# markchil/gptools

Measured on AMD Instinct MI355X. Metric: K-build+Cholesky GFLOP/s (% fp64 MFMA peak) and LML evals/sec, N=8192, higher is better.
Workload: dtype f64

## Files before the change

gptools_amd/_lib.py:

```python
import ctypes as C
import os
import subprocess
import threading

import numpy as np

_HERE = os.path.dirname(os.path.abspath(__file__))
LIB_PATH = os.path.join(_HERE, "libgpt_hip.so")

GPT_OK = 0
GPT_E_ARG, GPT_E_VALUE, GPT_E_NOTIMPL, GPT_E_HIP, GPT_E_NOMEM, GPT_E_STATE = -1, -2, -3, -4, -5, -6
KERNEL_SE, KERNEL_M52, KERNEL_DIAGNOISE, KERNEL_ZERO, KERNEL_RQ, KERNEL_MATERN, KERNEL_PRODUCT = 0, 1, 2, 3, 4, 5, 6
KERNEL_GIBBS_TANH, KERNEL_GIBBS_DTANH = 7, 8
MAX_DIM = 16
WARP_LINEAR, WARP_BETA, WARP_MAX_LAYERS = 1, 2, 4

_dp = C.POINTER(C.c_double)
_ip = C.POINTER(C.c_int32)
_vp = C.c_void_p
_i64 = C.c_int64

SIGNATURES = {
    "gpt_version": (C.c_int, []),
    "gpt_last_error": (C.c_char_p, []),
    "gpt_ctx_create": (C.c_int, [C.c_int, _vp, C.POINTER(_vp)]),
    "gpt_ctx_destroy": (C.c_int, [_vp]),
    "gpt_ctx_set_option": (C.c_int, [_vp, C.c_char_p, _i64]),
    "gpt_ctx_synchronize": (C.c_int, [_vp]),
    "gpt_ctx_stream": (_vp, [_vp]),
    "gpt_ctx_edge_count": (C.c_int64, [_vp]),
    "gpt_concurrency_hint": (C.c_int, [C.c_int]),
    "gpt_kpairs": (C.c_int, [_vp, C.c_int, _dp, C.c_int, _dp, _dp, _ip, _ip, _i64, C.c_int, C.c_int, C.c_int, _ip, _dp]),
    "gpt_kbuild": (C.c_int, [_vp, C.c_int, _dp, C.c_int, _dp, _ip, _i64, _dp, _ip, _i64, C.c_int, C.c_int, _ip, _dp]),
    "gpt_kpairs2": (C.c_int, [_vp, C.c_int, _dp, C.c_int, C.c_int, _dp, C.c_int, _dp, _dp, _ip, _ip, _i64, C.c_int, _dp]),
    "gpt_kbuild2": (C.c_int, [_vp, C.c_int, _dp, C.c_int, C.c_int, _dp, C.c_int, _dp, _ip, _i64, _dp, _ip, _i64, C.c_int, _dp]),
    "gpt_fit_terms": (C.c_int, [_vp, C.c_int, _ip, _ip, _dp, _ip, _ip, C.c_double, _dp, _dp, C.c_double, _dp, _dp]),
    "gpt_set_data": (C.c_int, [_vp, _dp, _ip, _i64, C.c_int]),
    "gpt_set_T": (C.c_int, [_vp, _dp, _i64]),
    "gpt_set_warp": (C.c_int, [_vp, C.c_int, _ip, _dp]),
    "gpt_set_warp_batch": (C.c_int, [_vp, C.c_int, C.c_int, _ip, _dp]),
    "gpt_fit": (C.c_int, [_vp, C.c_int, _dp, C.c_int, C.c_double, _dp, _dp, C.c_double, _dp, _dp]),
    "gpt_fit_sum": (C.c_int, [_vp, C.c_int, _ip, _dp, _ip, C.c_double, _dp, _dp, C.c_double, _dp, _dp]),
    "gpt_fit_batch": (C.c_int, [_vp, C.c_int, C.c_int, _dp, C.c_int, _dp, _dp, _dp, C.c_double, _dp, _dp, _ip]),
    "gpt_fit_batch_sum": (C.c_int, [_vp, C.c_int, C.c_int, _ip, _dp, _ip, _dp, _dp, _dp, C.c_double, _dp, _dp, _ip]),
    "gpt_mem_info": (C.c_int, [_vp, C.POINTER(_i64), C.POINTER(_i64)]),
    "gpt_release_batch_scratch": (C.c_int, [_vp]),
    "gpt_fit_batch_terms": (C.c_int, [_vp, C.c_int, C.c_int, _ip, _ip, _dp, _ip, _ip, _dp, _dp, _dp, C.c_double, _dp, _dp, _ip]),
    "gpt_predict_batch": (C.c_int, [_vp, _dp, _ip, _i64, _ip, _ip, _dp, _dp, _dp, _dp]),
    "gpt_fit_matrix": (C.c_int, [_vp, _dp, _i64, _dp, _dp, _dp]),
    "gpt_get_L": (C.c_int, [_vp, _dp]),
    "gpt_get_alpha": (C.c_int, [_vp, _dp]),
    "gpt_ll_grad": (C.c_int, [_vp, C.c_int, _ip, _ip, _dp]),
    "gpt_predict": (C.c_int, [_vp, _dp, _ip, _i64, C.c_int, _dp, _ip, _dp, _dp, _dp]),
    "gpt_host_alloc": (C.c_int, [_i64, C.POINTER(_vp)]),
    "gpt_host_free": (C.c_int, [_vp]),
    "gpt_cov_sample": (C.c_int, [_vp, _i64, C.c_double, _dp, _i64, _dp]),
    "gpt_solve_L": (C.c_int, [_vp, _dp, _i64]),
    "gpt_cho_solve": (C.c_int, [_vp, _dp, _i64]),
    "gpt_last_timings": (C.c_int, [_vp, _dp, C.c_int]),
    "gpt_gemm_profile_read": (C.c_int, [_vp, _dp]),
    "gpt_gemm_profile_read4": (C.c_int, [_vp, _dp]),
    "gpt_plan_unique_id": (C.c_int, [_vp]),
    "gpt_plan_create": (C.c_int, [C.c_int, C.POINTER(_vp), C.POINTER(_i64), _i64, C.c_int, _vp, _vp, C.c_int, _vp, C.POINTER(_vp)]),
    "gpt_plan_set_comm": (C.c_int, [_vp, C.c_int, C.c_int, _vp]),
    "gpt_plan_set_channel": (C.c_int, [_vp, C.c_int, C.c_int, C.c_int, _vp]),
    "gpt_plan_run": (C.c_int, [_vp, C.c_int, _dp, C.c_int, C.c_double, C.c_double]),
    "gpt_plan_last_enqueue_ms": (C.c_double, [_vp]),
    "gpt_plan_destroy": (C.c_int, [_vp]),
    "gpt_potrf_host": (C.c_int, [_vp, _dp, _i64]),
    "gpt_gemm_nt_host": (C.c_int, [_vp, _i64, _i64, _i64, C.c_double, _dp, _dp, C.c_double, _dp]),
    "gpt_dev_kbuild": (C.c_int, [_vp, C.c_int, _dp, C.c_int, _vp, _vp, _i64, _vp, _vp, _i64, C.c_int, C.c_int, C.c_int,
                                 _ip, C.c_int, _i64, _i64, _vp, C.c_double, C.c_double, _vp, _i64]),
    "gpt_dev_gemm_nt": (C.c_int, [_vp, _i64, _i64, _i64, C.c_double, _vp, _i64, _vp, _i64, C.c_double, _vp, _i64, C.c_int]),
    "gpt_dev_gemm_nt_stair": (C.c_int, [_vp, _i64, _i64, _i64, _i64, C.c_double, _vp, _i64, _vp, _i64, _i64, _i64, C.c_double, _vp, _i64]),
    "gpt_dev_gemm_nt_gridstair": (C.c_int, [_vp, _i64, _i64, _i64, _i64, C.c_double, _vp, _i64, _vp, _i64, _i64, _i64, _i64, _i64,
                                           C.c_double, _vp, _i64]),
    "gpt_dev_row_sumsq": (C.c_int, [_vp, _vp, _i64, _vp]),
    "gpt_dev_potrf_panel": (C.c_int, [_vp, _i64, _i64, _vp, _i64, _vp, _vp, _i64]),
    "gpt_dev_potrf": (C.c_int, [_vp, _i64, _vp, _i64, _vp, _vp]),
    "gpt_dev_trsm_rlt": (C.c_int, [_vp, _i64, _i64, _vp, _i64, _vp, _vp, _i64]),
    "gpt_dev_trinv": (C.c_int, [_vp, _i64, _vp, _i64, _vp, _vp, _i64]),
    "gpt_dev_copy2d": (C.c_int, [_vp, _i64, _i64, _vp, _i64, _vp, _i64]),
    "gpt_dev_copy2d_on": (C.c_int, [_vp, _vp, _i64, _i64, _vp, _i64, _vp, _i64]),
    "gpt_dev_pad_block": (C.c_int, [_vp, _vp, _i64, _i64, _i64, _i64, _i64, _vp, C.c_double]),
    "gpt_dev_panel_scalars": (C.c_int, [_vp, _vp, _i64, _i64, _i64, _vp]),
}

_lib = None
_lock = threading.Lock()


class GPTBackendError(RuntimeError):
    """The HIP backend is missing or failed; there is deliberately no CPU fallback."""


def build(verbose=False):
    cmd = ["make", "-C", os.path.join(_HERE, "csrc"), "-j4"]
    res = subprocess.run(cmd, stdout=subprocess.PIPE, stderr=subprocess.STDOUT, text=True)
    if verbose or res.returncode != 0:
        print(res.stdout)
    if res.returncode != 0:
        raise GPTBackendError("building libgpt_hip.so failed")
    return LIB_PATH


def load():
    global _lib
    with _lock:
        if _lib is None:
            if not os.path.exists(LIB_PATH):
                raise GPTBackendError(
                    "%s not found: run `python -c 'import __graft_entry__ as g; g.build()'` "
                    "(gptools_amd has no CPU fallback)" % LIB_PATH)
            try:
                import torch
            except ImportError:
                pass
            lib = C.CDLL(LIB_PATH)
            for name, (res, args) in SIGNATURES.items():
                fn = getattr(lib, name)
                fn.restype = res
                fn.argtypes = args
            _lib = lib
    return _lib


def last_error():
    return load().gpt_last_error().decode("utf-8", "replace")


def check(rc):
    if rc == GPT_OK:
        return
    msg = last_error()
    if rc > 0:
        raise np.linalg.LinAlgError(msg or "%d-th leading minor of the array is not positive definite" % rc)
    if rc in (GPT_E_ARG, GPT_E_VALUE):
        raise ValueError(msg)
    if rc == GPT_E_NOTIMPL:
        raise NotImplementedError(msg)
    if rc == GPT_E_NOMEM:
        raise MemoryError(msg)
    raise GPTBackendError("libgpt_hip: %s (code %d)" % (msg, rc))


def f64(a):
    return np.ascontiguousarray(a, dtype=np.float64)


def i32(a):
    return np.ascontiguousarray(a, dtype=np.int32)


def dptr(a):
    return None if a is None else a.ctypes.data_as(_dp)


def iptr(a):
    return None if a is None else a.ctypes.data_as(_ip)


class _PinnedOwner(object):

    def __init__(self, lib, ptr, nbytes):
        self._lib, self._ptr, self._nbytes = lib, ptr, nbytes

    def __del__(self):
        try:
            if self._ptr:
                _pinned_release(self._lib, self._ptr, self._nbytes)
                self._ptr = None
        except Exception:
            pass


PINNED_POOL_BYTES = 2 << 30
_pinned_free = {}
_pinned_held = [0]


def _pinned_release(lib, ptr, nbytes):
    with _lock:
        if _pinned_held[0] + nbytes <= PINNED_POOL_BYTES:
            _pinned_free.setdefault(nbytes, []).append(ptr)
            _pinned_held[0] += nbytes
            return
    lib.gpt_host_free(ptr)


def pinned_empty(shape, min_bytes=1 << 20):
    n = int(np.prod(shape))
    if n * 8 < min_bytes:
        return np.empty(shape, dtype=np.float64)
    lib = load()
    p = None
    with _lock:
        blocks = _pinned_free.get(n * 8)
        if blocks:
            p = blocks.pop()
            _pinned_held[0] -= n * 8
    if p is None:
        p = _vp()
        check(lib.gpt_host_alloc(n * 8, C.byref(p)))
    buf = (C.c_double * n).from_address(p.value)
    buf._owner = _PinnedOwner(lib, p, n * 8)
    return np.ctypeslib.as_array(buf).reshape(shape)


class concurrent_evaluations(object):

    def __enter__(self):
        load().gpt_concurrency_hint(1)
        return self

    def __exit__(self, *exc):
        load().gpt_concurrency_hint(-1)
        return False


class Context(object):

    def __init__(self, device=0, stream=None):
        lib = load()
        h = _vp()
        check(lib.gpt_ctx_create(int(device), _vp(stream) if stream else None, C.byref(h)))
        self._h = h
        self._lib = lib
        self.device = int(device)
        self._warp_key = None

    def close(self):
        if getattr(self, "_h", None):
            self._lib.gpt_ctx_destroy(self._h)
            self._h = None

    def __del__(self):
        try:
            self.close()
        except Exception:
            pass

    @property
    def handle(self):
        if not self._h:
            raise GPTBackendError("context already destroyed")
        return self._h

    def set_option(self, key, value):
        check(self._lib.gpt_ctx_set_option(self.handle, key.encode(), int(value)))

    def synchronize(self):
        check(self._lib.gpt_ctx_synchronize(self.handle))

    @property
    def stream(self):
        return self._lib.gpt_ctx_stream(self.handle)

    @property
    def edge_count(self):
        return int(self._lib.gpt_ctx_edge_count(self.handle))

    @staticmethod
    def _pair_args(Xi, Xj, ni, nj):
        Xi, Xj, ni, nj = f64(Xi), f64(Xj), i32(ni), i32(nj)
        if Xi.ndim != 2 or Xi.shape != Xj.shape or ni.shape != Xi.shape or nj.shape != Xi.shape:
            raise ValueError("Lengths/widths of Xi, Xj, ni, nj don't match")
        M, D = Xi.shape
        return (dptr(Xi), dptr(Xj), iptr(ni), iptr(nj), M), D, np.empty(M, dtype=np.float64), (Xi, Xj, ni, nj)

    @staticmethod
    def _block_args(Xi, ni, Xj, nj):
        Xi, ni = f64(Xi), i32(ni)
        M, D = Xi.shape
        if Xj is None:
            Xj_, nj_, P = None, None, M
        else:
            Xj_, nj_ = f64(Xj), i32(nj)
            P = Xj_.shape[0]
        return (dptr(Xi), iptr(ni), M, dptr(Xj_), iptr(nj_), P), D, np.empty((M, P), dtype=np.float64), (Xi, ni, Xj_, nj_)

    def kpairs(self, kernel_id, params, Xi, Xj, ni, nj, hyper_deriv=None, symmetric=False, noise_n=None):
        params = f64(params)
        pts, D, out, keep = self._pair_args(Xi, Xj, ni, nj)
        nn = None if noise_n is None else i32(noise_n)
        check(self._lib.gpt_kpairs(self.handle, kernel_id, dptr(params), len(params), *pts, D,
                                   -1 if hyper_deriv is None else int(hyper_deriv), int(bool(symmetric)), iptr(nn), dptr(out)))
        return out

    def kbuild(self, kernel_id, params, Xi, ni, Xj=None, nj=None, hyper_deriv=None, noise_n=None):
        params = f64(params)
        pts, D, out, keep = self._block_args(Xi, ni, Xj, nj)
        nn = None if noise_n is None else i32(noise_n)
        check(self._lib.gpt_kbuild(self.handle, kernel_id, dptr(params), len(params), *pts, D,
                                   -1 if hyper_deriv is None else int(hyper_deriv), iptr(nn), dptr(out)))
        return out

    def kpairs2(self, kid1, params1, kid2, params2, Xi, Xj, ni, nj):
        p1, p2 = f64(params1), f64(params2)
        pts, D, out, keep = self._pair_args(Xi, Xj, ni, nj)
        check(self._lib.gpt_kpairs2(self.handle, kid1, dptr(p1), len(p1), kid2, dptr(p2), len(p2), *pts, D, dptr(out)))
        return out

    def kbuild2(self, kid1, params1, kid2, params2, Xi, ni, Xj=None, nj=None):
        p1, p2 = f64(params1), f64(params2)
        pts, D, out, keep = self._block_args(Xi, ni, Xj, nj)
        check(self._lib.gpt_kbuild2(self.handle, kid1, dptr(p1), len(p1), kid2, dptr(p2), len(p2), *pts, D, dptr(out)))
        return out

    @staticmethod
    def _flat_params(terms):
        return np.concatenate([np.asarray(p, dtype=float) for t in terms for p in t[1::2]])

    @staticmethod
    def _pack_terms(terms):
        ids = i32(np.asarray([t[0] for t in terms]))
        ids2 = i32(np.asarray([t[2] if len(t) == 4 else -1 for t in terms]))
        npar1 = i32(np.asarray([len(t[1]) for t in terms]))
        npar = i32(np.asarray([len(t[1]) + (len(t[3]) if len(t) == 4 else 0) for t in terms]))
        return ids, ids2, npar, npar1, f64(Context._flat_params(terms))

    def fit_terms(self, terms, noise_var, y, err_y, diag_add):
        ids, ids2, npar, npar1, flat = self._pack_terms(terms)
        y, err_y = f64(y), f64(err_y)
        ll = C.c_double()
        ld = C.c_double()
        check(self._lib.gpt_fit_terms(self.handle, len(ids), iptr(ids), iptr(ids2), dptr(flat), iptr(npar), iptr(npar1),
                                      float(noise_var), dptr(y), dptr(err_y), float(diag_add), C.byref(ll), C.byref(ld)))
        return ll.value, ld.value

    def set_data(self, X, n):
        X, n = f64(X), i32(n)
        self._warp_key = None
        self._num_dim = X.shape[1]
        check(self._lib.gpt_set_data(self.handle, dptr(X), iptr(n), X.shape[0], X.shape[1]))

    def set_warp(self, layers):
        layers = [(int(t), f64(p).ravel()) for t, p in (layers or [])]
        key = tuple((t, p.tobytes()) for t, p in layers) or None
        if key == self._warp_key:
            return
        self._warp_key = None
        if not layers:
            check(self._lib.gpt_set_warp(self.handle, 0, None, None))
            return
        types = i32(np.asarray([t for t, _ in layers]))
        flat = f64(np.concatenate([p for _, p in layers]))
        if any(p.size != 2 * getattr(self, "_num_dim", -1) for _, p in layers):
            raise ValueError("set_warp needs set_data first, and every layer takes 2 * num_dim parameters")
        check(self._lib.gpt_set_warp(self.handle, len(layers), iptr(types), dptr(flat)))
        self._warp_key = key

    def set_warp_batch(self, layers_list):
        types = [int(t) for t, _ in layers_list[0]]
        D = getattr(self, "_num_dim", -1)
        rows = []
        for layers in layers_list:
            if [int(t) for t, _ in layers] != types:
                raise ValueError("set_warp_batch: every element takes the same layer types")
            ps = [f64(p).ravel() for _, p in layers]
            if any(p.size != 2 * D for p in ps):
                raise ValueError("set_warp_batch needs set_data first, and every layer takes 2 * num_dim parameters")
            rows.append(np.concatenate(ps) if ps else np.zeros(0))
        flat = f64(np.array(rows))
        check(self._lib.gpt_set_warp_batch(self.handle, len(layers_list), len(types), iptr(i32(np.asarray(types))), dptr(flat)))

    def set_T(self, T):
        if T is None:
            check(self._lib.gpt_set_T(self.handle, None, 0))
            return
        T = f64(T)
        if T.ndim != 2:
            raise ValueError("T must be 2-dimensional")
        check(self._lib.gpt_set_T(self.handle, dptr(T), T.shape[0]))

    def fit(self, kernel_id, params, noise_var, y, err_y, diag_add):
        params, y, err_y = f64(params), f64(y), f64(err_y)
        ll = C.c_double()
        ld = C.c_double()
        check(self._lib.gpt_fit(self.handle, kernel_id, dptr(params), len(params), float(noise_var), dptr(y),
                                dptr(err_y), float(diag_add), C.byref(ll), C.byref(ld)))
        return ll.value, ld.value

    def fit_sum(self, kernel_ids, params_list, noise_var, y, err_y, diag_add):
        ids = i32(np.asarray(kernel_ids))
        npar = i32(np.asarray([len(p) for p in params_list]))
        flat = f64(np.concatenate([np.asarray(p, dtype=float) for p in params_list]))
        y, err_y = f64(y), f64(err_y)
        ll = C.c_double()
        ld = C.c_double()
        check(self._lib.gpt_fit_sum(self.handle, len(ids), iptr(ids), dptr(flat), iptr(npar), float(noise_var), dptr(y),
                                    dptr(err_y), float(diag_add), C.byref(ll), C.byref(ld)))
        return ll.value, ld.value

    def fit_batch(self, kernel_id, params, noise_var, y, err_y, diag_add):
        params, noise_var, y, err_y = f64(np.atleast_2d(params)), f64(noise_var), f64(np.atleast_2d(y)), f64(err_y)
        B = params.shape[0]
        if noise_var.shape != (B,) or y.shape[0] != B or y.shape[1] != err_y.shape[0]:
            raise ValueError("fit_batch: params (B, p), noise_var (B,), y (B, N), err_y (N,) expected")
        ll, ld, info = np.empty(B), np.empty(B), np.zeros(B, dtype=np.int32)
        check(self._lib.gpt_fit_batch(self.handle, B, kernel_id, dptr(params), params.shape[1], dptr(noise_var), dptr(y),
                                      dptr(err_y), float(diag_add), dptr(ll), dptr(ld), iptr(info)))
        return ll, ld, info

    def fit_batch_sum(self, kernel_ids, params, nparams, noise_var, y, err_y, diag_add):
        ids, npar = i32(kernel_ids), i32(nparams)
        params, noise_var, y, err_y = f64(np.atleast_2d(params)), f64(noise_var), f64(np.atleast_2d(y)), f64(err_y)
        B = params.shape[0]
        if (noise_var.shape != (B,) or y.shape[0] != B or y.shape[1] != err_y.shape[0] or len(ids) != len(npar)
                or params.shape[1] != int(npar.sum())):
            raise ValueError("fit_batch_sum: params (B, sum(nparams)), noise_var (B,), y (B, N), err_y (N,) expected")
        ll, ld, info = np.empty(B), np.empty(B), np.zeros(B, dtype=np.int32)
        check(self._lib.gpt_fit_batch_sum(self.handle, B, len(ids), iptr(ids), dptr(params), iptr(npar), dptr(noise_var),
                                          dptr(y), dptr(err_y), float(diag_add), dptr(ll), dptr(ld), iptr(info)))
        return ll, ld, info

    def fit_batch_terms(self, terms_list, noise_var, y, err_y, diag_add):
        ids, ids2, npar, npar1, _ = self._pack_terms(terms_list[0])
        params = f64(np.array([self._flat_params(terms) for terms in terms_list]))
        noise_var, y, err_y = f64(noise_var), f64(np.atleast_2d(y)), f64(err_y)
        B = params.shape[0]
        if noise_var.shape != (B,) or y.shape[0] != B or y.shape[1] != err_y.shape[0] or params.shape[1] != int(npar.sum()):
            raise ValueError("fit_batch_terms: one parameter set per element, noise_var (B,), y (B, N), err_y (N,) expected")
        ll, ld, info = np.empty(B), np.empty(B), np.zeros(B, dtype=np.int32)
        check(self._lib.gpt_fit_batch_terms(self.handle, B, len(ids), iptr(ids), iptr(ids2), dptr(params), iptr(npar), iptr(npar1),
                                            dptr(noise_var), dptr(y), dptr(err_y), float(diag_add), dptr(ll), dptr(ld), iptr(info)))
        return ll, ld, info

    def predict_batch(self, Xstar, nstar, keep, noise_n=None, want_var=True, want_cov=False, want_cov_sum=False):
        Xstar, nstar, keep = f64(Xstar), i32(nstar), i32(np.asarray(keep) != 0)
        B, M = keep.shape[0], Xstar.shape[0]
        mean = np.full((B, M), np.nan)
        var = np.full((B, M), np.nan) if want_var else None
        cov = np.full((B, M, M), np.nan) if want_cov else None
        cov_sum = np.empty((M, M)) if want_cov_sum else None
        nn = None if noise_n is None else i32(np.asarray(noise_n).reshape(-1))
        check(self._lib.gpt_predict_batch(self.handle, dptr(Xstar), iptr(nstar), M, iptr(nn), iptr(keep), dptr(mean), dptr(var),
                                          dptr(cov), dptr(cov_sum)))
        return mean, var, cov, cov_sum

    def mem_info(self):
        f, t = _i64(), _i64()
        check(self._lib.gpt_mem_info(self.handle, C.byref(f), C.byref(t)))
        return int(f.value), int(t.value)

    def release_batch_scratch(self):
        check(self._lib.gpt_release_batch_scratch(self.handle))

    def ll_grad(self, term_idx, local_idx):
        ti, li = i32(np.asarray(term_idx)), i32(np.asarray(local_idx))
        out = np.empty(len(ti) + 1)
        check(self._lib.gpt_ll_grad(self.handle, len(ti), iptr(ti), iptr(li), dptr(out)))
        return out

    def fit_matrix(self, K_tot, y):
        K_tot, y = f64(K_tot), f64(y)
        ll = C.c_double()
        ld = C.c_double()
        check(self._lib.gpt_fit_matrix(self.handle, dptr(K_tot), K_tot.shape[0], dptr(y), C.byref(ll), C.byref(ld)))
        return ll.value, ld.value

    def get_L(self, N):
        L = np.empty((N, N), dtype=np.float64)
        check(self._lib.gpt_get_L(self.handle, dptr(L)))
        return L

    def get_alpha(self, N):
        a = np.empty(N, dtype=np.float64)
        check(self._lib.gpt_get_alpha(self.handle, dptr(a)))
        return a

    def predict(self, Xstar, nstar, want, noise_params=None, noise_n=None, device_cov=False):
        Xstar, nstar = f64(Xstar), i32(nstar)
        M = Xstar.shape[0]
        mean = np.empty(M)
        std = np.empty(M) if want >= 1 else None
        cov = pinned_empty((M, M)) if (want == 2 and not device_cov) else None
        npar = None if noise_params is None else f64(noise_params)
        nn = None if noise_n is None else i32(noise_n)
        check(self._lib.gpt_predict(self.handle, dptr(Xstar), iptr(nstar), M, int(want), dptr(npar), iptr(nn),
                                    dptr(mean), dptr(std), dptr(cov)))
        return mean, std, cov

    def cov_sample(self, diag_add, rand_vars):
        R = f64(np.atleast_2d(rand_vars))
        out = np.empty(R.shape)
        check(self._lib.gpt_cov_sample(self.handle, R.shape[0], float(diag_add), dptr(R), R.shape[1], dptr(out)))
        return out

    def solve_L(self, B):
        B2 = np.array(B, dtype=np.float64, order="C")
        shp = B2.shape
        B2 = np.ascontiguousarray(B2.reshape(shp[0], -1))
        check(self._lib.gpt_solve_L(self.handle, dptr(B2), B2.shape[1]))
        return B2.reshape(shp)

    def cho_solve(self, B):
        B2 = np.array(B, dtype=np.float64, order="C")
        shp = B2.shape
        B2 = np.ascontiguousarray(B2.reshape(shp[0], -1))
        check(self._lib.gpt_cho_solve(self.handle, dptr(B2), B2.shape[1]))
        return B2.reshape(shp)

    def last_timings(self):
        out = np.zeros(5)
        self._lib.gpt_last_timings(self.handle, dptr(out), 5)
        return dict(upload=out[0], kbuild=out[1], potrf=out[2], tail=out[3], total=out[4])

    def gemm_profile_read(self, with_bytes=False):
        out = np.zeros(4)
        check(self._lib.gpt_gemm_profile_read4(self.handle, dptr(out)))
        if with_bytes:
            return float(out[0]), float(out[1]), int(out[2]), float(out[3])
        return float(out[0]), float(out[1]), int(out[2])

    def potrf_host(self, A):
        L = np.array(A, dtype=np.float64, order="C")
        check(self._lib.gpt_potrf_host(self.handle, dptr(L), L.shape[0]))
        return L

    def gemm_nt_host(self, alpha, A, B, beta, Cm):
        A, B = f64(A), f64(B)
        Cm = np.array(Cm, dtype=np.float64, order="C")
        check(self._lib.gpt_gemm_nt_host(self.handle, A.shape[0], B.shape[0], A.shape[1], float(alpha), dptr(A),
                                         dptr(B), float(beta), dptr(Cm)))
        return Cm


_default_ctx = {}


def default_context(device=0):
    key = (os.getpid(), int(device))
    ctx = _default_ctx.get(key)
    if ctx is None:
        ctx = Context(device)
        _default_ctx[key] = ctx
    return ctx
```

gptools_amd/csrc/api.hip:

```cpp
#include <math.h>
#include <stdarg.h>
#include <stdlib.h>
#include <string.h>
#include <new>
#include <chrono>
#include <mutex>
#include <vector>
#include "common.hpp"
#include "warp.hpp"

static thread_local char g_err[512] = "";

void gpt_set_error(const char *fmt, ...)
{
    va_list ap;
    va_start(ap, fmt);
    vsnprintf(g_err, sizeof(g_err), fmt, ap);
    va_end(ap);
}

extern "C" const char *gpt_last_error(void) { return g_err; }
extern "C" int gpt_version(void) { return 100; }

#define GPT_TRY(expr)          \
    do {                       \
        int rc_ = (expr);      \
        if (rc_ != GPT_OK) return rc_; \
    } while (0)

static inline int64_t round_up(int64_t x, int64_t m) { return (x + m - 1) / m * m; }

#include "api_kparams.inc"

struct DevBuf {
    void *p = nullptr;
    size_t cap = 0;
};

enum { SLOT_XI = 0, SLOT_XJ, SLOT_NI, SLOT_NJ, SLOT_OUT, SLOT_KST, SLOT_KSS, SLOT_XS, SLOT_NS, SLOT_VEC, SLOT_VEC2,
       SLOT_RHS, SLOT_LOW, SLOT_KFULL, SLOT_TK, SLOT_ZERO, SLOT_UINV, SLOT_WINV, SLOT_GPART, SLOT_BINV, SLOT_BTMP,
       SLOT_BINV2, SLOT_BINV3, SLOT_BINV3U, SLOT_BINVU, SLOT_BATCH_A, SLOT_BATCH_WS, SLOT_BATCH_MISC, SLOT_SPLITK,
       SLOT_PB_V, SLOT_PB_COV, SLOT_PB_MISC, SLOT_XSW, SLOT_SS, SLOT_SI, SLOT_SJ, SLOT_WB_X, SLOT_WB_S, SLOT_WB_P, SLOT_COUNT };

struct gpt_ctx {
    int device = 0;
    hipStream_t stream = nullptr;
    bool own_stream = false;
    hipStream_t panel_stream = nullptr;
    hipStream_t helper_stream = nullptr;
    int64_t nb_early = 0, nb_switch_rows = 4608;
    unsigned *d_edge = nullptr;
    unsigned edge_seq = 0;
    int64_t tail_wait = 1;
    int64_t merge_urgent = 1;
    int64_t edge_flags = 1;
    bool flags_now = false;
    int reserve_cus = 0;
    int64_t gemm_prio = -1;
    int64_t purg_rows = 6144;
    int64_t defer_rows = 0;
    int helper_cus = 0;
    std::vector<hipEvent_t> events;
    hipEvent_t tev[5] = {nullptr, nullptr, nullptr, nullptr, nullptr};
    int64_t nb_outer = 0;
    int lookahead = 1;
    int use_graph = 0;
    long n_maxsum = 0;
    long n_maxord = 0;
    int timing = 0;
    int tile = 0;
    int gemm_pad = 1024;
    int64_t fuse_trsm = 8192;
    unsigned *d_flag = nullptr;
    unsigned flag_epoch = 0;
    int64_t binv_launches = 0;
    int64_t splitk = 512;
    int64_t fuse_rows32 = 2048, fuse_rows16 = 0;
    int64_t fuse_rows64 = 2048;
    int64_t helper_min_n = 12288;
    int helper_tf = 45;
    int ramp = 0;
    int inner = 0;
    int64_t N = 0;
    int64_t Nx = 0;
    int D = 0;
    double *dT = nullptr;
    int64_t Ny = 0, NxP = 0;
    double *dX = nullptr;
    int32_t *dn = nullptr;
    WarpLayers warp = WarpLayers();
    double *dXw = nullptr, *dS = nullptr;
    int warpb_nbatch = 0;
    bool rb_warped = false;
    int64_t NP = 0;
    double *dA = nullptr;
    double *d_invd = nullptr;
    int32_t *d_info = nullptr;
    double *d_y = nullptr, *d_erry = nullptr, *d_scal = nullptr, *d_alpha = nullptr;
    double *h_scal = nullptr;
    double *h_yerr = nullptr;
    double *h_alpha = nullptr;
    bool h_alpha_valid = false;
    int32_t *h_info = nullptr;
    bool factored = false, alpha_valid = false, have_kernel = false;
    bool binv_valid = false;
    bool binv2_valid = false;
    bool binv3_valid = false;
    int64_t dev_gemm_pad = 0;
    int64_t eager_alpha = 0;
    int64_t binv_early = 0;
    hipEvent_t e_binv_early = nullptr;
    int64_t defer_pad = 1;
    unsigned alpha_counter = 0;
    int64_t debug_poison = 0;
    int64_t edge_test_stall = 0;
    double *h_stage = nullptr;
    hipStream_t copy_stream = nullptr;
    hipEvent_t cev[4] = {nullptr, nullptr, nullptr, nullptr};
    double *h_batch = nullptr;
    size_t h_batch_cap = 0;
    uint64_t batch_gen = 1, rb_gen = 0;
    int rb_nbatch = 0;
    int64_t rb_N = 0;
    ModelKernel rb_model;
    std::vector<KParams> rb_kp, rb_kp2;
    std::vector<double> rb_nv;
    int64_t cov_M = 0;
    ModelKernel model;
    double timings[5] = {0, 0, 0, 0, 0};
    int prof_gemm = 0;
    struct GemmProf { hipEvent_t e0, e1, stop; double flops, bytes; };
    std::vector<GemmProf> gprof;
    size_t gprof_used = 0;
    double prof_flops = 0, prof_ms = 0, prof_count = 0, prof_bytes = 0;
    hipGraphExec_t gexec = nullptr;
    int64_t g_n = 0, g_nb = 0;
    int g_la = 0;
    double *g_A = nullptr;
    DevBuf slots[SLOT_COUNT];
};

static int strip_rows_code(const gpt_ctx *c, int64_t m) { return m <= c->fuse_rows16 ? 3 : m <= c->fuse_rows32 ? 2 : m <= c->fuse_rows64 ? 1 : 0; }

static int ensure(gpt_ctx *c, int slot, size_t bytes, void **out)
{
    DevBuf &b = c->slots[slot];
    if (b.cap < bytes) {
        if (b.p) GPT_HIP_CHECK(hipFree(b.p));
        b.p = nullptr;
        b.cap = 0;
        const size_t want = bytes + bytes / 8 + 256;
        GPT_HIP_CHECK(hipMalloc(&b.p, want));
        b.cap = want;
    }
    *out = b.p;
    return GPT_OK;
}

static hipEvent_t get_event(gpt_ctx *c, size_t idx)
{
    while (c->events.size() <= idx) {
        hipEvent_t e = nullptr;
        if (hipEventCreate(&e) != hipSuccess) return nullptr;
        c->events.push_back(e);
    }
    return c->events[idx];
}

static void invalidate_factor(gpt_ctx *c)
{
    c->factored = false;
    c->h_alpha_valid = c->alpha_valid = c->binv_valid = c->binv2_valid = c->binv3_valid = false;
}

static int stream_follows(gpt_ctx *c, hipStream_t from, hipStream_t to, size_t idx)
{
    hipEvent_t e = get_event(c, idx);
    if (!e) return GPT_E_HIP;
    GPT_HIP_CHECK(hipEventRecord(e, from));
    GPT_HIP_CHECK(hipStreamWaitEvent(to, e, 0));
    return GPT_OK;
}

#include "api_schedule.inc"
#include "api_context.inc"
#include "api_kernels.inc"
#include "api_fit.inc"
#include "api_batch.inc"
#include "api_grad.inc"
#include "api_solve.inc"
#include "api_predict.inc"
#include "api_dev.inc"
#include "api_plan.inc"
```

gptools_amd/csrc/api_batch.inc:

```
#define GPT_BATCH_MAX_N 8192
static int fit_batch_impl(gpt_ctx *c, int nbatch, int nterms, const int *kernel_ids, const int *kernel_ids2, const double *params,
                          const int *nparams_t, const int *nparams1_t, const double *noise_var, const double *y, const double *err_y,
                          double diag_add, double *ll_data_out, double *logdet_half_out, int32_t *info_out);

extern "C" int gpt_fit_batch(gpt_ctx *c, int nbatch, int kernel_id, const double *params, int nparams,
                             const double *noise_var, const double *y, const double *err_y, double diag_add,
                             double *ll_data_out, double *logdet_half_out, int32_t *info_out)
{
    return fit_batch_impl(c, nbatch, 1, &kernel_id, nullptr, params, &nparams, nullptr, noise_var, y, err_y, diag_add, ll_data_out,
                          logdet_half_out, info_out);
}

extern "C" int gpt_fit_batch_sum(gpt_ctx *c, int nbatch, int nterms, const int *kernel_ids, const double *params,
                                 const int *nparams_t, const double *noise_var, const double *y, const double *err_y,
                                 double diag_add, double *ll_data_out, double *logdet_half_out, int32_t *info_out)
{
    return fit_batch_impl(c, nbatch, nterms, kernel_ids, nullptr, params, nparams_t, nullptr, noise_var, y, err_y, diag_add, ll_data_out,
                          logdet_half_out, info_out);
}

extern "C" int gpt_fit_batch_terms(gpt_ctx *c, int nbatch, int nterms, const int *kernel_ids, const int *kernel_ids2,
                                   const double *params, const int *nparams_t, const int *nparams1_t, const double *noise_var,
                                   const double *y, const double *err_y, double diag_add, double *ll_data_out,
                                   double *logdet_half_out, int32_t *info_out)
// ... 34 lines not shown
    const size_t off_err = (size_t)nbatch * N, off_nv = off_err + (size_t)N, off_kp = off_nv + (size_t)nbatch, off_res = off_kp + nkp;
    const size_t need = (off_res + 4 * (size_t)nbatch) * sizeof(double);
    if (c->h_batch_cap < need) {
        if (c->h_batch) GPT_HIP_CHECK(hipHostFree(c->h_batch));
        c->h_batch = nullptr;
        c->h_batch_cap = 0;
        GPT_HIP_CHECK(hipHostMalloc((void **)&c->h_batch, need + need / 4, hipHostMallocDefault));
        c->h_batch_cap = need + need / 4;
    }
    double *h = c->h_batch;
    memcpy(h, y, (size_t)nbatch * N * sizeof(double));
    memcpy(h + off_err, err_y, (size_t)N * sizeof(double));
    memcpy(h + off_nv, noise_var, (size_t)nbatch * sizeof(double));
    char *hkp = reinterpret_cast<char *>(h + off_kp), *hkp2 = hkp + (size_t)nterms * nbatch * kp_doubles * 8;
    for (int b = 0; b < nbatch; b++) {
        if (b > 0) GPT_TRY(parse_model(c->D, c->n_maxsum, nterms, kernel_ids, kernel_ids2, params + (size_t)b * m0.nparams, nparams_t, nparams1_t, &mb));
        const ModelKernel &m = b > 0 ? mb : m0;
        for (int t = 0; t < nterms; t++) {
            memcpy(hkp + ((size_t)t * nbatch + (size_t)b) * kp_doubles * 8, &m.f1[t], sizeof(KParams));
            if (any_prod) memcpy(hkp2 + ((size_t)t * nbatch + (size_t)b) * kp_doubles * 8, &m.f2[t], sizeof(KParams));
        }
    }
    c->batch_gen++;
    const int64_t NxP = c->dT ? c->NxP : 0, NyP = c->dT ? round_up(N, 64) : 0;
    const size_t kfull = (size_t)NxP * NxP, tk = (size_t)NyP * NxP;
    double *dA, *dws, *dmisc;
    GPT_TRY(ensure(c, SLOT_BATCH_A, ((size_t)nbatch * bs + (size_t)nbatch * (kfull + tk)) * sizeof(double), (void **)&dA));
    double *dKf = dA + (size_t)nbatch * bs, *dTK = dKf + (size_t)nbatch * kfull;
    GPT_TRY(ensure(c, SLOT_BATCH_WS, (size_t)nbatch * bws * sizeof(double), (void **)&dws));
    const size_t d_off_nv = (size_t)N, d_off_kp = d_off_nv + (size_t)nbatch, d_off_info = d_off_kp + nkp,
                 d_off_zero = d_off_info + (size_t)nbatch;
    GPT_TRY(ensure(c, SLOT_BATCH_MISC, (d_off_zero + (size_t)(c->dT ? Nx : 0)) * sizeof(double), (void **)&dmisc));
    int32_t *dinfo = reinterpret_cast<int32_t *>(dmisc + d_off_info);
    const KParams *dkp = reinterpret_cast<const KParams *>(dmisc + d_off_kp);
    const KParams *dkp2 = any_prod ? dkp + (size_t)nterms * nbatch : nullptr;
    const double *bX = c->dX, *bS = nullptr;
    int64_t xstr = 0, sstr = 0;
    if (wb) {
        bX = (const double *)c->slots[SLOT_WB_X].p;
        bS = (const double *)c->slots[SLOT_WB_S].p;
        xstr = Nx * c->D;
        sstr = Nx;
    }
    EvalScope scope(c, true);
    hipStream_t st = c->panel_stream;
    GPT_TRY(stream_follows(c, c->stream, st, 0));
    GPT_HIP_CHECK(hipMemcpyAsync(dmisc, h + off_err, ((size_t)N + (size_t)nbatch + nkp) * sizeof(double), hipMemcpyHostToDevice, st));
    auto term_kp2 = [&](int t) -> const KParams * { return m0.second(t) ? dkp2 + (size_t)t * nbatch : nullptr; };
    if (c->dT) {
        double *dzero = dmisc + d_off_zero;
        GPT_HIP_CHECK(hipMemsetAsync(dzero, 0, (size_t)Nx * sizeof(double), st));
        if (NxP > Nx) GPT_HIP_CHECK(hipMemsetAsync(dKf, 0, (size_t)nbatch * kfull * sizeof(double), st));
        for (int t = 0; t < nterms; t++)
            GPT_TRY(launch_kbuild_batch(st, m0.f1[t].kernel_id, c->D, dkp + (size_t)t * nbatch, dmisc + d_off_nv, nbatch, bX, c->dn, Nx,
                                        t + 1 == nterms ? dzero : nullptr, 0.0, dKf, NxP, (int64_t)kfull, t > 0 ? 1 : 0, 1, term_kp2(t),
                                        xstr, bS, sstr));
        GPT_TRY(launch_gemm_nt(st, NyP, NxP, NxP, 1.0, c->dT, NxP, dKf, NxP, 0.0, dTK, NxP, 0, 0, 0, nullptr, nullptr, 0, EdgeSig(),
                               EdgeSig(), 0, nbatch, 0, EdgeSig(), (int64_t)kfull, (int64_t)tk));
        GPT_TRY(launch_gemm_nt(st, NyP, NyP, NxP, 1.0, dTK, NxP, c->dT, NxP, 0.0, dA, NP, 1, 0, 0, nullptr, nullptr, 0, EdgeSig(),
                               EdgeSig(), 0, nbatch, (int64_t)tk, EdgeSig(), 0, bs));
        GPT_TRY(launch_add_diag(st, dA, NP, N, dmisc, diag_add, nbatch, bs));
        GPT_TRY(launch_batch_pad(st, h, nbatch, dA, NP, bs, N, NP, 1e300, dinfo));
    } else {
        GPT_TRY(launch_batch_pad(st, h, nbatch, dA, NP, bs, N, NP, 1e300, dinfo));
        for (int t = 0; t < nterms; t++)
            GPT_TRY(launch_kbuild_batch(st, m0.f1[t].kernel_id, c->D, dkp + (size_t)t * nbatch, dmisc + d_off_nv, nbatch,
                                        bX, c->dn, N, t + 1 == nterms ? dmisc : nullptr, diag_add, dA, NP, bs,
                                        t > 0 ? 1 : 0, 0, term_kp2(t), xstr, bS, sstr));
    }
    static const bool force_right = getenv("GPT_BATCH_RIGHT") != nullptr;
    const bool right_looking = force_right || NP <= 512;
    for (int64_t lc = 0; lc < NP; lc += 128) {
        if (!right_looking && lc > 0)
            GPT_TRY(launch_gemm_nt(st, NP - lc, 128, lc, -1.0, dA + lc * NP, NP, dA + lc * NP, NP, 1.0, dA + lc * NP + lc, NP, 1, 0, 0,
                                   nullptr, nullptr, 0, EdgeSig(), EdgeSig(), 0, nbatch, bs));
        GPT_TRY(launch_potf2_diag(st, dA + lc * NP + lc, NP, dws + (lc / 128) * GPT_WS_BLOCK, dinfo, lc, EdgeSig(), nbatch, bs, bws));
        const int64_t r1 = lc + 128, m = NP - r1;
        if (m <= 0) break;
        GPT_TRY(launch_trsm_panel(st, m, dA + lc * NP + lc, NP, dws + (lc / 128) * GPT_WS_BLOCK, dA + r1 * NP + lc, NP, nullptr,
                                  EdgeSig(), nbatch, bs, bws));
        if (right_looking)
            GPT_TRY(launch_gemm_nt(st, m, m, 128, -1.0, dA + r1 * NP + lc, NP, dA + r1 * NP + lc, NP, 1.0, dA + r1 * NP + r1, NP, 1, 0, 0,
                                   nullptr, nullptr, 0, EdgeSig(), EdgeSig(), 0, nbatch, bs));
    }
    GPT_TRY(launch_batch_logdet_dot(st, dA, NP, bs, N, nbatch, dinfo, h + off_res));
    GPT_HIP_CHECK(hipStreamSynchronize(st));
    for (int b = 0; b < nbatch; b++) {
        const double logdet_half = h[off_res + 4 * b], zz = h[off_res + 4 * b + 1];
        int32_t info = (int32_t)h[off_res + 4 * b + 2];
        if (info > N) info = (int32_t)N;
        const double ll = -0.5 * zz - logdet_half - 0.5 * (double)N * log(2.0 * M_PI);
        if (info == 0 && !(ll == ll)) info = (int32_t)N;
        info_out[b] = info;
        ll_data_out[b] = ll;
        if (logdet_half_out) logdet_half_out[b] = logdet_half;
    }
    const KParams *hk = reinterpret_cast<const KParams *>(hkp);
    c->rb_kp.assign(hk, hk + (size_t)nterms * nbatch);
    if (any_prod) c->rb_kp2.assign(hk + (size_t)nterms * nbatch, hk + 2 * (size_t)nterms * nbatch);
    else c->rb_kp2.clear();
    c->rb_nv.assign(noise_var, noise_var + nbatch);
    c->rb_nbatch = nbatch;
    c->rb_model = m0;
    c->rb_N = N;
    c->rb_gen = c->batch_gen;
    c->rb_warped = wb != 0;
    return GPT_OK;
}

static int gemm_nt_few(gpt_ctx *c, hipStream_t st, int64_t m, int64_t n, int64_t k, double alpha, const double *A, int64_t lda,
                       const double *B, int64_t ldb, double beta, double *C, int64_t ldc, int tri);
extern "C" int gpt_predict_batch(gpt_ctx *c, const double *Xstar, const int32_t *nstar, int64_t M, const int32_t *noise_n,
                                 const int32_t *keep, double *mean_out, double *var_out, double *cov_out, double *cov_sum_out)
{
    CTX_ENTER(c);
    GPT_TRY(refuse_warp(c, "gpt_predict_batch"));
    if (c->rb_warped && c->rb_nbatch > 0 && c->rb_gen == c->batch_gen) {
        gpt_set_error("gpt_predict_batch is not available for a batch that was fitted with warps (gpt_set_warp_batch)");
        return GPT_E_NOTIMPL;
    }
    if (c->rb_nbatch <= 0 || c->rb_gen != c->batch_gen) {
        gpt_set_error("gpt_predict_batch: no batch resident (call gpt_fit_batch* first; gpt_set_data, gpt_set_T, gpt_cov_sample and "
                      "gpt_release_batch_scratch end its residency)");
        return GPT_E_STATE;
    }
    if (c->dT) {
        gpt_set_error("gpt_predict_batch: not implemented with a linear transform (gpt_set_T)");
        return GPT_E_NOTIMPL;
    }
    if (M <= 0 || M > 65535 * 32 || !Xstar || !nstar || !keep || !mean_out) {
        gpt_set_error("gpt_predict_batch: bad arguments");
        return GPT_E_ARG;
    }
    const ModelKernel &model = c->rb_model;
    const int D = c->D, nbatch = c->rb_nbatch, nterms = model.nterms;
    const int64_t N = c->rb_N, NP = round_up(N + 1, 128), nleaf = NP / 128, bs = NP * NP, bws = nleaf * GPT_WS_BLOCK;
    const int64_t MP = round_up(M, 64), ldv = (int64_t)nbatch * NP;
    GPT_TRY(check_test_orders(model, c->n_maxsum, false, nstar, M, D));
    double noise_sum = 0.0;
    for (int b = 0; b < nbatch; b++)
        if (keep[b]) noise_sum += c->rb_nv[b];
    std::vector<int32_t> hit((size_t)M, 0);
    if (noise_n)
        for (int64_t a = 0; a < M; a++) {
            bool h = true;
            for (int d = 0; d < D; d++) h = h && nstar[a * D + d] == noise_n[d];
            hit[a] = h ? 1 : 0;
        }
    const size_t nkp = (size_t)nterms * nbatch * (model.any_prod ? 2 : 1);
    const size_t b_kp = nkp * sizeof(KParams) + (size_t)nbatch * 8, b_keep = round_up(nbatch, 2) * 4, b_hit = round_up(M, 2) * 4,
                 b_xs = (size_t)M * D * 8, b_ns = round_up(M * D, 2) * 4;
    const size_t o_keep = b_kp, o_hit = o_keep + b_keep, o_xs = o_hit + b_hit, o_ns = o_xs + b_xs, o_mv = o_ns + b_ns;
    const size_t b_mv = 2 * (size_t)nbatch * MP * 8;
    char *dmisc;
    GPT_TRY(ensure(c, SLOT_PB_MISC, o_mv + b_mv, (void **)&dmisc));
    std::vector<char> hin(o_mv);
    memcpy(hin.data(), c->rb_kp.data(), (size_t)nterms * nbatch * sizeof(KParams));
    if (model.any_prod) memcpy(hin.data() + (size_t)nterms * nbatch * sizeof(KParams), c->rb_kp2.data(), (size_t)nterms * nbatch * sizeof(KParams));
    memcpy(hin.data() + nkp * sizeof(KParams), c->rb_nv.data(), (size_t)nbatch * 8);
    memcpy(hin.data() + o_keep, keep, (size_t)nbatch * 4);
    memcpy(hin.data() + o_hit, hit.data(), (size_t)M * 4);
    memcpy(hin.data() + o_xs, Xstar, b_xs);
    memcpy(hin.data() + o_ns, nstar, (size_t)M * D * 4);
    const KParams *dkp = reinterpret_cast<const KParams *>(dmisc);
    const KParams *dkp2 = model.any_prod ? dkp + (size_t)nterms * nbatch : nullptr;
    const double *dnv = reinterpret_cast<const double *>(dmisc + nkp * sizeof(KParams));
    const int32_t *dkeep = reinterpret_cast<const int32_t *>(dmisc + o_keep), *dhit = reinterpret_cast<const int32_t *>(dmisc + o_hit);
    const double *dXs = reinterpret_cast<const double *>(dmisc + o_xs);
    const int32_t *dns = reinterpret_cast<const int32_t *>(dmisc + o_ns);
    double *dmean = reinterpret_cast<double *>(dmisc + o_mv), *dvar = dmean + (size_t)nbatch * MP;
    double *dV, *dC = nullptr;
    GPT_TRY(ensure(c, SLOT_PB_V, (size_t)MP * ldv * sizeof(double), (void **)&dV));
    const bool want_cov = cov_out != nullptr, want_sum = cov_sum_out != nullptr;
    if (want_cov || want_sum)
        GPT_TRY(ensure(c, SLOT_PB_COV, (want_cov ? (size_t)nbatch : 1) * MP * MP * sizeof(double), (void **)&dC));
    const double *dA = (const double *)c->slots[SLOT_BATCH_A].p, *dws = (const double *)c->slots[SLOT_BATCH_WS].p;
    EvalScope scope(c, true);
    hipStream_t st = c->panel_stream;
    GPT_TRY(stream_follows(c, c->stream, st, 0));
    GPT_HIP_CHECK(hipMemcpyAsync(dmisc, hin.data(), o_mv, hipMemcpyHostToDevice, st));
    auto term_kp2 = [&](int t) -> const KParams * { return model.second(t) ? dkp2 + (size_t)t * nbatch : nullptr; };
    GPT_TRY(launch_zero2d(st, MP, ldv, dV, ldv));
    for (int t = 0; t < nterms; t++)
        GPT_TRY(launch_kbuild_batch_cross(st, model.f1[t].kernel_id, D, dkp + (size_t)t * nbatch, dnv, nbatch, dXs, dns,
                                          M, c->dX, c->dn, N, dV, ldv, NP, t > 0 ? 1 : 0, term_kp2(t)));
    for (int64_t lc = 0; lc < NP; lc += 128) {
        if (lc > 0)
            GPT_TRY(launch_gemm_nt(st, MP, 128, lc, -1.0, dV, ldv, dA + lc * NP, NP, 1.0, dV + lc, ldv, 0, 0, 0, nullptr, nullptr, 0,
                                   EdgeSig(), EdgeSig(), 0, nbatch, NP, EdgeSig(), bs, NP));
        GPT_TRY(launch_trsm_panel(st, MP, nullptr, 0, dws + (lc / 128) * GPT_WS_BLOCK, dV + lc, ldv, nullptr, EdgeSig(), nbatch, NP, bws));
    }
    GPT_TRY(launch_kdiag_batch(st, D, nterms, dkp, dkp2, nbatch, dXs, dns, M, dvar, MP));
    GPT_TRY(launch_batch_meanvar(st, M, MP, N, NP, nbatch, dV, ldv, dA, bs, dkeep, dmean, dvar, MP));
    std::vector<double> hmv(2 * (size_t)nbatch * MP);
    GPT_HIP_CHECK(hipMemcpyAsync(hmv.data(), dmean, hmv.size() * sizeof(double), hipMemcpyDeviceToHost, st));
    if (want_sum) {
        GPT_TRY(launch_zero2d(st, MP, MP, dC, MP));
        GPT_TRY(launch_kss_sum(st, D, nterms, dkp, dkp2, nbatch, dkeep, dXs, dns, M, MP, noise_n ? dhit : nullptr, noise_sum, dC, MP));
        GPT_TRY(gemm_nt_few(c, st, MP, MP, ldv, -1.0, dV, ldv, dV, ldv, 1.0, dC, MP, 1));
        GPT_TRY(launch_mirror_rows(st, dC, MP, 0, MP, MP));
        GPT_HIP_CHECK(hipMemcpy2DAsync(cov_sum_out, (size_t)M * sizeof(double), dC, (size_t)MP * sizeof(double), (size_t)M * sizeof(double),
                                       (size_t)M, hipMemcpyDeviceToHost, st));
    }
    GPT_HIP_CHECK(hipStreamSynchronize(st));
    if (want_cov) {
        const int64_t cs = MP * MP;
        GPT_TRY(launch_zero2d(st, (int64_t)nbatch * MP, MP, dC, MP));
        for (int t = 0; t < nterms; t++)
            GPT_TRY(launch_kbuild_batch_cross(st, model.f1[t].kernel_id, D, dkp + (size_t)t * nbatch, dnv, nbatch, dXs,
                                              dns, M, dXs, dns, M, dC, MP, cs, t > 0 ? 1 : 0, term_kp2(t)));
        GPT_TRY(launch_gemm_nt(st, MP, MP, NP, -1.0, dV, ldv, dV, ldv, 1.0, dC, MP, 0, 0, 0, nullptr, nullptr, 0, EdgeSig(), EdgeSig(), 0,
                               nbatch, NP, EdgeSig(), NP, cs));
        for (int b = 0; b < nbatch; b++)
            if (keep[b])
                GPT_HIP_CHECK(hipMemcpy2DAsync(cov_out + (size_t)b * M * M, (size_t)M * sizeof(double), dC + (size_t)b * cs,
                                               (size_t)MP * sizeof(double), (size_t)M * sizeof(double), (size_t)M, hipMemcpyDeviceToHost, st));
        GPT_HIP_CHECK(hipStreamSynchronize(st));
    }
    for (int b = 0; b < nbatch; b++) {
        if (!keep[b]) continue;
        const double *hm = hmv.data() + (size_t)b * MP, *hv = hm + (size_t)nbatch * MP;
        memcpy(mean_out + (size_t)b * M, hm, (size_t)M * sizeof(double));
        const double nv = c->rb_nv[b];
        if (var_out)
            for (int64_t a = 0; a < M; a++) var_out[(size_t)b * M + a] = hv[a] + (hit[a] ? nv : 0.0);
        if (cov_out && noise_n)
            for (int64_t a = 0; a < M; a++)
                if (hit[a]) cov_out[(size_t)b * M * M + (size_t)a * M + a] += nv;
    }
    return GPT_OK;
}

extern "C" int gpt_last_timings(gpt_ctx *c, double *out_ms, int n)
{
    if (!c || !out_ms) return GPT_E_ARG;
    const int cnt = n < 5 ? n : 5;
    for (int i = 0; i < cnt; i++) out_ms[i] = c->timings[i];
    return cnt;
}

static int harvest_gemm_profile(gpt_ctx *c)
{
    for (size_t i = 0; i < c->gprof_used; i++) {
        float t = 0;
        GPT_HIP_CHECK(hipEventElapsedTime(&t, c->gprof[i].e0, c->gprof[i].stop));
        c->prof_ms += t;
        c->prof_flops += c->gprof[i].flops;
        c->prof_bytes += c->gprof[i].bytes;
    }
    c->prof_count += (double)c->gprof_used;
    c->gprof_used = 0;
    return GPT_OK;
}

static int gemm_profile_read(gpt_ctx *c, double *out, int n)
{
    if (!out || n < 3) return GPT_E_ARG;
    GPT_HIP_CHECK(hipStreamSynchronize(c->stream));
    GPT_HIP_CHECK(hipStreamSynchronize(c->panel_stream));
    GPT_TRY(harvest_gemm_profile(c));
    out[0] = c->prof_flops;
    out[1] = c->prof_ms;
    out[2] = c->prof_count;
    if (n > 3) out[3] = c->prof_bytes;
    c->prof_flops = c->prof_ms = c->prof_count = c->prof_bytes = 0.0;
    return GPT_OK;
}

extern "C" int gpt_gemm_profile_read(gpt_ctx *c, double *out3)
{
    CTX_ENTER(c);
    return gemm_profile_read(c, out3, 3);
}

extern "C" int gpt_gemm_profile_read4(gpt_ctx *c, double *out4)
{
    CTX_ENTER(c);
    return gemm_profile_read(c, out4, 4);
}

#define NEED_FACTOR(c)                                                        \
    do {                                                                      \
        if (!(c)->factored) {                                                 \
            gpt_set_error("no valid factorisation resident (call gpt_fit)");  \
            return GPT_E_STATE;                                               \
        }                                                                     \
    } while (0)

extern "C" int gpt_get_L(gpt_ctx *c, double *L_out)
{
    CTX_ENTER(c);
    NEED_FACTOR(c);
    if (!L_out) return GPT_E_ARG;
    const int64_t N = c->N;
    double *dlow;
    GPT_TRY(ensure(c, SLOT_LOW, (size_t)N * N * sizeof(double), (void **)&dlow));
    GPT_TRY(launch_extract_lower(c->stream, c->dA, c->NP, N, dlow, N));
    GPT_HIP_CHECK(hipMemcpyAsync(L_out, dlow, (size_t)N * N * sizeof(double), hipMemcpyDeviceToHost, c->stream));
    GPT_HIP_CHECK(hipStreamSynchronize(c->stream));
    return GPT_OK;
}

static int ensure_block_inverses(gpt_ctx *c, int64_t nb, int64_t nfull, double **out, double **out_u = nullptr, hipStream_t on = nullptr);
static int ensure_alpha(gpt_ctx *c, hipStream_t on = nullptr)
{
    if (c->alpha_valid) return GPT_OK;
    const int64_t N = c->N, NP = c->NP, n128 = round_up(N, 128);
    hipStream_t st = on ? on : c->stream;
    static const bool narrow = getenv("GPT_ALPHA_NARROW") != nullptr;
    const int64_t nwide = (n128 / 512) * 512;
    double *w = c->d_alpha + NP;
    const double *z = c->dA + N * NP;
    if (!narrow && nwide == N && nwide >= 1024) {
        double *W = nullptr, *U = nullptr;
        GPT_TRY(ensure_block_inverses(c, 512, nwide, &W, &U, st));
        GPT_TRY(launch_trsv_lt_wide(st, nwide, c->dA, NP, U, w, c->d_alpha, z));
        c->alpha_valid = true;
        return GPT_OK;
    }
    GPT_TRY(launch_alpha_init(st, N, NP, z, w, c->d_alpha));
    if (narrow || nwide < 1024) {
        GPT_HIP_CHECK(hipMemcpyAsync(c->d_alpha, w, (size_t)N * sizeof(double), hipMemcpyDeviceToDevice, st));
        GPT_TRY(launch_trsv_lt(st, n128, c->dA, NP, c->d_invd, c->d_alpha));
        c->alpha_valid = true;
        return GPT_OK;
    }
    double *W = nullptr, *U = nullptr;
    GPT_TRY(ensure_block_inverses(c, 512, nwide, &W, &U, st));
    if (n128 > nwide) {
        GPT_TRY(launch_trsv_lt(st, n128, c->dA, NP, c->d_invd, w, nwide / 128));
        GPT_HIP_CHECK(hipMemcpyAsync(c->d_alpha + nwide, w + nwide, (size_t)(n128 - nwide) * sizeof(double), hipMemcpyDeviceToDevice, st));
    }
    GPT_TRY(launch_trsv_lt_wide(st, nwide, c->dA, NP, U, w, c->d_alpha));
    c->alpha_valid = true;
    return GPT_OK;
}

static int alpha_to_host(gpt_ctx *c, hipStream_t on)
{
    hipStream_t st = on ? on : c->stream;
    GPT_TRY(ensure_alpha(c, st));
    if (c->h_alpha_valid) return GPT_OK;
    GPT_HIP_CHECK(hipMemcpyAsync(c->h_alpha, c->d_alpha, (size_t)c->N * sizeof(double), hipMemcpyDeviceToHost, st));
    c->h_alpha_valid = true;
    return GPT_OK;
}

extern "C" int gpt_get_alpha(gpt_ctx *c, double *alpha_out)
{
    CTX_ENTER(c);
    NEED_FACTOR(c);
    if (!alpha_out) return GPT_E_ARG;
    const bool landed = c->alpha_valid && c->h_alpha_valid;
    if (!landed) {
        GPT_TRY(alpha_to_host(c));
        GPT_HIP_CHECK(hipStreamSynchronize(c->stream));
    }
    memcpy(alpha_out, c->h_alpha, (size_t)c->N * sizeof(double));
    return GPT_OK;
}
```

gptools_amd/csrc/api_context.inc:

```
extern "C" int gpt_ctx_create(int device_id, void *stream, gpt_ctx **out)
{
    if (!out) return GPT_E_ARG;
    int ndev = 0;
    GPT_HIP_CHECK(hipGetDeviceCount(&ndev));
    if (ndev <= 0 || device_id < 0 || device_id >= ndev) {
        gpt_set_error("no such HIP device %d (count %d)", device_id, ndev);
        return GPT_E_HIP;
    }
    GPT_HIP_CHECK(hipSetDevice(device_id));
    gpt_ctx *c = new (std::nothrow) gpt_ctx();
    if (!c) return GPT_E_NOMEM;
    c->device = device_id;
    int lo = 0, hi = 0;
    GPT_HIP_CHECK(hipDeviceGetStreamPriorityRange(&lo, &hi));
    if (stream) {
        c->stream = (hipStream_t)stream;
    } else {
        int reserve = 32;
        if (const char *e = getenv("GPT_RESERVE_CUS")) reserve = atoi(e);
        hipDeviceProp_t prop;
        GPT_HIP_CHECK(hipGetDeviceProperties(&prop, device_id));
        const int ncu = prop.multiProcessorCount;
        bool masked = false;
        if (reserve > 0 && reserve < ncu) {
            std::vector<uint32_t> mask((ncu + 31) / 32, 0u);
            for (int i = reserve; i < ncu; i++) mask[i / 32] |= (1u << (i % 32));
            masked = hipExtStreamCreateWithCUMask(&c->stream, (uint32_t)mask.size(), mask.data()) == hipSuccess;
            if (!masked) (void)hipGetLastError();
            else c->reserve_cus = reserve;
            if (masked && reserve >= 16) {
                std::vector<uint32_t> hm((ncu + 31) / 32, 0u);
                for (int i = 8; i < reserve; i++) hm[i / 32] |= (1u << (i % 32));
                if (hipExtStreamCreateWithCUMask(&c->helper_stream, (uint32_t)hm.size(), hm.data()) != hipSuccess) {
                    (void)hipGetLastError();
                    c->helper_stream = nullptr;
                }
                c->helper_cus = reserve - 8;
            }
        }
        if (!masked) GPT_HIP_CHECK(hipStreamCreateWithFlags(&c->stream, hipStreamNonBlocking));
        c->own_stream = true;
    }
    GPT_HIP_CHECK(hipStreamCreateWithPriority(&c->panel_stream, hipStreamNonBlocking, hi));
    for (int i = 0; i < 5; i++) GPT_HIP_CHECK(hipEventCreate(&c->tev[i]));
    GPT_HIP_CHECK(hipMalloc(&c->d_info, sizeof(int32_t)));
    GPT_HIP_CHECK(hipMalloc((void **)&c->d_flag, 256));
    GPT_HIP_CHECK(hipMalloc((void **)&c->d_edge, 256));
    GPT_HIP_CHECK(hipMemsetAsync(c->d_flag, 0, 256, c->stream));
    GPT_HIP_CHECK(hipMemsetAsync(c->d_edge, 0, 256, c->stream));
    GPT_HIP_CHECK(hipMalloc(&c->d_scal, 80 * sizeof(double)));
    GPT_HIP_CHECK(hipMemsetAsync(c->d_scal, 0, 80 * sizeof(double), c->stream));
    GPT_HIP_CHECK(hipHostMalloc((void **)&c->h_scal, 4 * sizeof(double), hipHostMallocDefault));
    GPT_HIP_CHECK(hipHostMalloc((void **)&c->h_info, sizeof(int32_t), hipHostMallocDefault));
    *out = c;
    return GPT_OK;
}

static void free_factor(gpt_ctx *c)
{
    if (c->gexec) { hipGraphExecDestroy(c->gexec); c->gexec = nullptr; }
    if (c->dA) hipFree(c->dA);
    if (c->d_invd) hipFree(c->d_invd);
    if (c->d_y) hipFree(c->d_y);
    if (c->h_yerr) hipHostFree(c->h_yerr);
    c->h_yerr = nullptr;
    if (c->h_alpha) hipHostFree(c->h_alpha);
    c->h_alpha = nullptr;
    c->h_alpha_valid = false;
    if (c->d_alpha) hipFree(c->d_alpha);
    c->dA = c->d_invd = c->d_y = c->d_erry = c->d_alpha = nullptr;
    c->NP = 0;
    invalidate_factor(c);
}

extern "C" int gpt_ctx_destroy(gpt_ctx *c)
{
    if (!c) return GPT_OK;
    hipSetDevice(c->device);
    hipStreamSynchronize(c->stream);
    hipStreamSynchronize(c->panel_stream);
    free_factor(c);
    if (c->dX) hipFree(c->dX);
    if (c->dn) hipFree(c->dn);
    if (c->dXw) hipFree(c->dXw);
    if (c->dS) hipFree(c->dS);
    if (c->dT) hipFree(c->dT);
    for (auto &b : c->slots)
        if (b.p) hipFree(b.p);
    for (auto e : c->events) hipEventDestroy(e);
    for (auto &g : c->gprof) { hipEventDestroy(g.e0); hipEventDestroy(g.e1); }
    for (int i = 0; i < 5; i++)
        if (c->tev[i]) hipEventDestroy(c->tev[i]);
    if (c->d_info) hipFree(c->d_info);
    if (c->d_flag) hipFree(c->d_flag);
    if (c->d_edge) hipFree(c->d_edge);
    if (c->d_scal) hipFree(c->d_scal);
    if (c->h_scal) hipHostFree(c->h_scal);
    if (c->h_stage) hipHostFree(c->h_stage);
    if (c->h_batch) hipHostFree(c->h_batch);
    if (c->copy_stream) hipStreamDestroy(c->copy_stream);
    for (auto &e : c->cev)
        if (e) hipEventDestroy(e);
    if (c->h_info) hipHostFree(c->h_info);
    hipStreamDestroy(c->panel_stream);
    if (c->e_binv_early) hipEventDestroy(c->e_binv_early);
    if (c->helper_stream) hipStreamDestroy(c->helper_stream);
    if (c->own_stream) hipStreamDestroy(c->stream);
    delete c;
    return GPT_OK;
}

extern "C" int gpt_ctx_set_option(gpt_ctx *c, const char *key, int64_t value)
{
    if (!c || !key) return GPT_E_ARG;
    if (!strcmp(key, "nb_outer")) {
        if (value < 0 || value % 128) {
            gpt_set_error("nb_outer must be 0 (chosen by size) or a positive multiple of 128");
            return GPT_E_ARG;
        }
        c->nb_outer = value;
    } else if (!strcmp(key, "lookahead")) c->lookahead = value ? 1 : 0;
    else if (!strcmp(key, "graph")) c->use_graph = value ? 1 : 0;
    else if (!strcmp(key, "timing")) c->timing = value ? 1 : 0;
    else if (!strcmp(key, "profile_gemm")) c->prof_gemm = value ? 1 : 0;
    else if (!strcmp(key, "gemm_pad")) c->gemm_pad = (int)value;
    else if (!strcmp(key, "dev_gemm_pad")) c->dev_gemm_pad = value;
    else if (!strcmp(key, "ramp")) c->ramp = value ? 1 : 0;
    else if (!strcmp(key, "defer_rows")) c->defer_rows = value;
    else if (!strcmp(key, "purg_rows")) c->purg_rows = value;
    else if (!strcmp(key, "edge_flags")) c->edge_flags = value;
    else if (!strcmp(key, "merge_urgent")) c->merge_urgent = value;
    else if (!strcmp(key, "tail_wait")) c->tail_wait = value;
    else if (!strcmp(key, "gemm_prio")) c->gemm_prio = value;
    else if (!strcmp(key, "nb_early")) c->nb_early = value;
    else if (!strcmp(key, "nb_switch_rows")) c->nb_switch_rows = value;
    else if (!strcmp(key, "inner")) c->inner = (int)value;
    else if (!strcmp(key, "helper_tf")) c->helper_tf = (int)value;
    else if (!strcmp(key, "helper_min_n")) c->helper_min_n = value;
    else if (!strcmp(key, "fuse_trsm")) c->fuse_trsm = value;
    else if (!strcmp(key, "fuse_rows64")) c->fuse_rows64 = value;
    else if (!strcmp(key, "fuse_rows32")) c->fuse_rows32 = value;
    else if (!strcmp(key, "fuse_rows16")) c->fuse_rows16 = value;
    else if (!strcmp(key, "splitk")) c->splitk = value;
    else if (!strcmp(key, "eager_alpha")) c->eager_alpha = value;
    else if (!strcmp(key, "defer_pad")) c->defer_pad = value;
    else if (!strcmp(key, "binv_launches")) { c->binv_launches = value; c->binv_valid = c->binv2_valid = c->binv3_valid = false; c->h_alpha_valid = c->alpha_valid = false; }
    else if (!strcmp(key, "debug_poison")) c->debug_poison = value;
    else if (!strcmp(key, "alpha_invalidate")) c->h_alpha_valid = c->alpha_valid = false;
    else if (!strcmp(key, "edge_test_stall")) c->edge_test_stall = value;
    else if (!strcmp(key, "tile")) {
        if (value != 0 && value != 32 && value != 64) {
            gpt_set_error("tile must be 0 (by launch size), 32 or 64");
            return GPT_E_ARG;
        }
        c->tile = (int)value;
    } else {
        gpt_set_error("unknown option '%s'", key);
        return GPT_E_ARG;
    }
    return GPT_OK;
}

extern "C" int gpt_ctx_synchronize(gpt_ctx *c)
{
    if (!c) return GPT_E_ARG;
    GPT_HIP_CHECK(hipStreamSynchronize(c->stream));
    return GPT_OK;
}

extern "C" void *gpt_ctx_stream(gpt_ctx *c) { return c ? (void *)c->stream : nullptr; }
extern "C" int64_t gpt_ctx_edge_count(gpt_ctx *c) { return c ? (int64_t)c->edge_seq : -1; }

#define CTX_ENTER(c)                          \
    do {                                      \
        if (!(c)) {                           \
            gpt_set_error("null context");    \
            return GPT_E_ARG;                 \
        }                                     \
        GPT_HIP_CHECK(hipSetDevice((c)->device)); \
    } while (0)
```

gptools_amd/csrc/api_fit.inc:

```
extern "C" int gpt_set_data(gpt_ctx *c, const double *X, const int32_t *n, int64_t N, int D)
{
    CTX_ENTER(c);
    if (N <= 0 || !X || !n || D < 1 || D > GPT_MAX_DIM) {
        gpt_set_error("set_data: bad arguments (N=%lld, D=%d)", (long long)N, D);
        return GPT_E_ARG;
    }
    GPT_HIP_CHECK(hipStreamSynchronize(c->stream));
    if (c->dX) hipFree(c->dX);
    if (c->dn) hipFree(c->dn);
    c->dX = nullptr;
    c->dn = nullptr;
    if (c->dXw) hipFree(c->dXw);
    if (c->dS) hipFree(c->dS);
    c->dXw = c->dS = nullptr;
    c->warp.nlayers = 0;
    c->warpb_nbatch = 0;
    GPT_HIP_CHECK(hipMalloc(&c->dX, (size_t)N * D * sizeof(double)));
    GPT_HIP_CHECK(hipMalloc(&c->dn, (size_t)N * D * sizeof(int32_t)));
    GPT_HIP_CHECK(hipMemcpyAsync(c->dX, X, (size_t)N * D * sizeof(double), hipMemcpyHostToDevice, c->stream));
    GPT_HIP_CHECK(hipMemcpyAsync(c->dn, n, (size_t)N * D * sizeof(int32_t), hipMemcpyHostToDevice, c->stream));
    GPT_HIP_CHECK(hipStreamSynchronize(c->stream));
    c->N = N;
    c->Nx = N;
    c->D = D;
    c->n_maxsum = c->n_maxord = 0;
    for (int64_t i = 0; i < N; i++) {
        long sn = 0;
        for (int d = 0; d < D; d++) {
            sn += n[i * D + d];
            if (n[i * D + d] > c->n_maxord) c->n_maxord = n[i * D + d];
        }
        if (sn > c->n_maxsum) c->n_maxsum = sn;
    }
    invalidate_factor(c);
    c->have_kernel = false;
    c->batch_gen++;
    if (c->dT) hipFree(c->dT);
    c->dT = nullptr;
    c->Ny = 0;
    return GPT_OK;
}

extern "C" int gpt_set_T(gpt_ctx *c, const double *T, int64_t Ny)
{
    CTX_ENTER(c);
    if (!c->dX) {
        gpt_set_error("gpt_set_T: call gpt_set_data first");
        return GPT_E_STATE;
    }
    GPT_HIP_CHECK(hipStreamSynchronize(c->stream));
    if (c->dT) hipFree(c->dT);
    c->dT = nullptr;
    c->Ny = 0;
    invalidate_factor(c);
    c->have_kernel = false;
    c->batch_gen++;
    if (!T || Ny <= 0) return GPT_OK;
    const int64_t NyP = round_up(Ny, 64), NxP = round_up(c->Nx, 16);
    GPT_HIP_CHECK(hipMalloc(&c->dT, (size_t)NyP * NxP * sizeof(double)));
    GPT_HIP_CHECK(hipMemsetAsync(c->dT, 0, (size_t)NyP * NxP * sizeof(double), c->stream));
    GPT_HIP_CHECK(hipMemcpy2DAsync(c->dT, (size_t)NxP * sizeof(double), T, (size_t)c->Nx * sizeof(double),
                                   (size_t)c->Nx * sizeof(double), (size_t)Ny, hipMemcpyHostToDevice, c->stream));
    GPT_HIP_CHECK(hipStreamSynchronize(c->stream));
    c->Ny = Ny;
    c->NxP = NxP;
    return GPT_OK;
}

extern "C" int gpt_set_warp(gpt_ctx *c, int nlayers, const int *types, const double *params)
{
    CTX_ENTER(c);
    if (nlayers == 0 && c->warp.nlayers == 0) return GPT_OK;
    invalidate_factor(c);
    c->have_kernel = false;
    c->cov_M = 0;
    if (nlayers == 0) {
        c->warp.nlayers = 0;
        return GPT_OK;
    }
    if (!c->dX) {
        gpt_set_error("gpt_set_warp: call gpt_set_data first");
        return GPT_E_STATE;
    }
    if (nlayers < 0 || nlayers > GPT_WARP_MAX_LAYERS || !types || !params) {
        gpt_set_error("gpt_set_warp: %d layers (at most %d)", nlayers, GPT_WARP_MAX_LAYERS);
        return GPT_E_ARG;
    }
    WarpLayers wl = WarpLayers();
    wl.nlayers = nlayers;
    wl.D = c->D;
    for (int l = 0; l < nlayers; l++) {
        if (types[l] != GPT_WARP_LINEAR && types[l] != GPT_WARP_BETA) {
            gpt_set_error("gpt_set_warp: unknown warp type %d", types[l]);
            return GPT_E_ARG;
        }
        wl.type[l] = types[l];
        memcpy(wl.p[l], params + (size_t)l * 2 * c->D, (size_t)2 * c->D * sizeof(double));
    }
    c->warp.nlayers = 0;
    if (c->n_maxord > 1) {
        gpt_set_error("%s", WARP_ORDER_MSG);
        return GPT_E_VALUE;
    }
    if (!c->dXw) GPT_HIP_CHECK(hipMalloc(&c->dXw, (size_t)c->Nx * c->D * sizeof(double)));
    if (!c->dS) GPT_HIP_CHECK(hipMalloc(&c->dS, (size_t)c->Nx * sizeof(double)));
    if (c->debug_poison) {
        GPT_HIP_CHECK(hipMemsetAsync(c->dXw, 0xff, (size_t)c->Nx * c->D * sizeof(double), c->stream));
        GPT_HIP_CHECK(hipMemsetAsync(c->dS, 0xff, (size_t)c->Nx * sizeof(double), c->stream));
    }
    GPT_TRY(launch_warp_points(c->stream, wl, c->dX, c->dn, c->Nx, c->dXw, c->dS));
    c->warp = wl;
    return GPT_OK;
}

extern "C" int gpt_set_warp_batch(gpt_ctx *c, int nbatch, int nlayers, const int *types, const double *params)
{
    CTX_ENTER(c);
    c->warpb_nbatch = 0;
    if (nlayers == 0 || nbatch == 0) return GPT_OK;
    if (!c->dX) {
        gpt_set_error("gpt_set_warp_batch: call gpt_set_data first");
        return GPT_E_STATE;
    }
    if (nbatch < 0 || nbatch > 65535 || nlayers < 0 || nlayers > GPT_WARP_MAX_LAYERS || !types || !params) {
        gpt_set_error("gpt_set_warp_batch: %d elements, %d layers (at most %d)", nbatch, nlayers, GPT_WARP_MAX_LAYERS);
        return GPT_E_ARG;
    }
    WarpLayers wl = WarpLayers();
    wl.nlayers = nlayers;
    wl.D = c->D;
    for (int l = 0; l < nlayers; l++) {
        if (types[l] != GPT_WARP_LINEAR && types[l] != GPT_WARP_BETA) {
            gpt_set_error("gpt_set_warp_batch: unknown warp type %d", types[l]);
            return GPT_E_ARG;
        }
        wl.type[l] = types[l];
    }
    if (c->n_maxord > 1) {
        gpt_set_error("%s", WARP_ORDER_MSG);
        return GPT_E_VALUE;
    }
    const size_t np = (size_t)nbatch * nlayers * 2 * c->D, nx = (size_t)nbatch * c->Nx * c->D, ns = (size_t)nbatch * c->Nx;
    double *dP, *dXb, *dSb;
    GPT_TRY(ensure(c, SLOT_WB_P, np * sizeof(double), (void **)&dP));
    GPT_TRY(ensure(c, SLOT_WB_X, nx * sizeof(double), (void **)&dXb));
    GPT_TRY(ensure(c, SLOT_WB_S, ns * sizeof(double), (void **)&dSb));
    hipStream_t st = c->stream;
    GPT_HIP_CHECK(hipMemcpyAsync(dP, params, np * sizeof(double), hipMemcpyHostToDevice, st));
    if (c->debug_poison) {
        GPT_HIP_CHECK(hipMemsetAsync(dXb, 0xff, nx * sizeof(double), st));
        GPT_HIP_CHECK(hipMemsetAsync(dSb, 0xff, ns * sizeof(double), st));
    }
    GPT_TRY(launch_warp_points_batch(st, wl, dP, nbatch, c->dX, c->dn, c->Nx, dXb, dSb));
    GPT_HIP_CHECK(hipStreamSynchronize(st));
    c->warpb_nbatch = nbatch;
    return GPT_OK;
}

static inline const double *model_X(const gpt_ctx *c) { return c->warp.nlayers > 0 ? c->dXw : c->dX; }
static inline const double *model_S(const gpt_ctx *c) { return c->warp.nlayers > 0 ? c->dS : nullptr; }

static int refuse_warp(const gpt_ctx *c, const char *what)
{
    if (c->warp.nlayers > 0) {
        gpt_set_error("%s is not available while warp layers are set (gpt_set_warp)", what);
        return GPT_E_NOTIMPL;
    }
    return GPT_OK;
}

static int ensure_factor_storage(gpt_ctx *c, int64_t N)
{
    const int64_t NP = round_up(N + 1, 128);
    if (c->NP == NP && c->dA) return GPT_OK;
    GPT_HIP_CHECK(hipStreamSynchronize(c->stream));
    free_factor(c);
    GPT_HIP_CHECK(hipMalloc(&c->dA, (size_t)NP * NP * sizeof(double)));
    GPT_HIP_CHECK(hipMalloc(&c->d_invd, (size_t)(NP / 128) * GPT_WS_BLOCK * sizeof(double)));
    GPT_HIP_CHECK(hipMalloc(&c->d_y, (size_t)2 * NP * sizeof(double)));
    c->d_erry = c->d_y + NP;
    GPT_HIP_CHECK(hipHostMalloc((void **)&c->h_yerr, (size_t)2 * NP * sizeof(double), hipHostMallocDefault));
    GPT_HIP_CHECK(hipHostMalloc((void **)&c->h_alpha, (size_t)NP * sizeof(double), hipHostMallocDefault));
    GPT_HIP_CHECK(hipMalloc(&c->d_alpha, (size_t)2 * NP * sizeof(double)));
    c->NP = NP;
    return GPT_OK;
}

static int harvest_gemm_profile(gpt_ctx *c);
static int alpha_to_host(gpt_ctx *c, hipStream_t on = nullptr);

static int factor_and_ll(gpt_ctx *c, int64_t N, double *ll_data_out, double *logdet_half_out, bool padded = false,
                         PotrfRequest req = PotrfRequest())
{
    hipStream_t st = c->stream;
    const int64_t NP = c->NP;
    if (!padded) {
        GPT_HIP_CHECK(hipMemsetAsync(c->d_info, 0, sizeof(int32_t), st));
        GPT_TRY(launch_fill_pad(st, c->dA, NP, N, NP, c->d_y, 1e300));
    }
    if (c->timing) GPT_HIP_CHECK(hipEventRecord(c->tev[2], st));
    req.defer_join = true;
    c->binv_early = 0;
    req.want_early_binv = c->eager_alpha != 0 && !c->use_graph;
    req.defer_pad_leaf = req.want_early_binv && c->defer_pad && N % 512 == 0 && N >= 1024 && NP == N + 128;
    PotrfResult fac;
    GPT_TRY(potrf_run(c, NP, c->dA, NP, c->d_invd, c->d_info, req, &fac));
    const bool pad_on_main = fac.pad_leaf_deferred;
    hipStream_t tl = fac.tail_stream ? fac.tail_stream : st;
    bool joined = false;
    hipStream_t red_st = tl;
    if (pad_on_main && tl != st) {
        red_st = st;
        joined = true;
    } else if (c->eager_alpha && tl != st) {
        GPT_TRY(stream_follows(c, tl, st, 1));
        red_st = st;
        joined = true;
    }
    GPT_TRY(launch_logdet_dot(red_st, c->dA, NP, N, c->d_info, c->d_scal, c->h_scal, nullptr, c->timing ? c->tev[4] : nullptr,
                              c->flags_now ? c->d_edge + 60 : nullptr));
    invalidate_factor(c);
    int rc_alpha = c->eager_alpha ? alpha_to_host(c, tl) : GPT_OK;
    c->binv_early = 0;
    if (tl != st && !joined) GPT_TRY(stream_follows(c, tl, st, 1));
    if (rc_alpha != GPT_OK) {
        invalidate_factor(c);
        if (tl != st) (void)hipStreamSynchronize(tl);
        (void)hipStreamSynchronize(st);
        return rc_alpha;
    }
    if (tl != st) GPT_HIP_CHECK(hipStreamSynchronize(tl));
    GPT_HIP_CHECK(hipStreamSynchronize(st));
    if (c->gprof_used) GPT_TRY(harvest_gemm_profile(c));
    if (c->timing) {
        float ms = 0;
        for (int i = 0; i < 2; i++) {
            hipEventElapsedTime(&ms, c->tev[i], c->tev[i + 1]);
            c->timings[i] = ms;
        }
        hipEventElapsedTime(&ms, c->tev[2], c->tev[4]);
        c->timings[2] = ms;
        c->timings[3] = 0.0;
        hipEventElapsedTime(&ms, c->tev[0], c->tev[4]);
        c->timings[4] = ms;
    }
    if (c->flags_now && c->h_scal[3] != 0.0) {
        invalidate_factor(c);
        return GPT_I_EDGE_TIMEOUT;
    }
    const int32_t info = (int32_t)c->h_scal[2];
    if (info != 0) {
        invalidate_factor(c);
        if (info > N) {
            gpt_set_error("factorisation failed in the augmented row (non-finite data?)");
            return (int)N;
        }
        gpt_set_error("%d-th leading minor of the array is not positive definite", (int)info);
        return (int)info;
    }
    c->factored = true;
    const double logdet_half = c->h_scal[0], zz = c->h_scal[1];
    if (logdet_half_out) *logdet_half_out = logdet_half;
    if (ll_data_out) *ll_data_out = -0.5 * zz - logdet_half - 0.5 * (double)N * log(2.0 * M_PI);
    return GPT_OK;
}

static int kbuild_terms(hipStream_t st, const ModelKernel &m, int symmetric, const double *dXi, const int32_t *dni, int64_t M,
                        const double *dXj, const int32_t *dnj, int64_t P, int lower_only, int64_t i0, int64_t j0,
                        const double *d_err, double noise_var, double diag_add, double *dK, int64_t ldk,
                        const double *dSi = nullptr, const double *dSj = nullptr)
{
    for (int t = 0; t < m.nterms; t++) {
        KParams kp = m.f1[t];
        kp.symmetric = symmetric;
        kp.hyper_deriv = -1;
        const bool last = t + 1 == m.nterms;
        GPT_TRY(launch_kbuild(st, kp, dXi, dni, M, dXj, dnj, P, lower_only, i0, j0, last ? d_err : nullptr, noise_var,
                              diag_add, dK, ldk, t > 0 ? 1 : 0, m.second(t), dSi, dSj));
    }
    return GPT_OK;
}

static int fit_terms(gpt_ctx *c, const ModelKernel &model, double noise_var, const double *y, const double *err_y,
                     double diag_add, double *ll_data_out, double *logdet_half_out);

extern "C" int gpt_fit(gpt_ctx *c, int kernel_id, const double *params, int nparams, double noise_var,
                       const double *y, const double *err_y, double diag_add, double *ll_data_out,
                       double *logdet_half_out)
{
    return gpt_fit_sum(c, 1, &kernel_id, params, &nparams, noise_var, y, err_y, diag_add, ll_data_out, logdet_half_out);
}

static int fit_model(gpt_ctx *c, int nterms, const int *kernel_ids, const int *kernel_ids2, bool need_ids2, const double *params,
                     const int *nparams, const int *nparams1, double noise_var, const double *y, const double *err_y, double diag_add,
                     double *ll_data_out, double *logdet_half_out)
{
    if (!c->dX) {
        gpt_set_error("gpt_fit: call gpt_set_data first");
        return GPT_E_STATE;
    }
    if (!y || !err_y || (need_ids2 && (!kernel_ids2 || !nparams1))) return GPT_E_ARG;
    ModelKernel model;
    GPT_TRY(parse_model(c->D, c->n_maxsum, nterms, kernel_ids, kernel_ids2, params, nparams, nparams1, &model));
    return fit_terms(c, model, noise_var, y, err_y, diag_add, ll_data_out, logdet_half_out);
}

extern "C" int gpt_fit_sum(gpt_ctx *c, int nterms, const int *kernel_ids, const double *params, const int *nparams,
                           double noise_var, const double *y, const double *err_y, double diag_add,
                           double *ll_data_out, double *logdet_half_out)
{
    CTX_ENTER(c);
    return fit_model(c, nterms, kernel_ids, nullptr, false, params, nparams, nullptr, noise_var, y, err_y, diag_add, ll_data_out,
                     logdet_half_out);
}

extern "C" int gpt_fit_terms(gpt_ctx *c, int nterms, const int *kernel_ids, const int *kernel_ids2, const double *params,
                             const int *nparams, const int *nparams1, double noise_var, const double *y, const double *err_y,
                             double diag_add, double *ll_data_out, double *logdet_half_out)
{
    CTX_ENTER(c);
    return fit_model(c, nterms, kernel_ids, kernel_ids2, true, params, nparams, nparams1, noise_var, y, err_y, diag_add, ll_data_out,
                     logdet_half_out);
}

static int fit_terms_once(gpt_ctx *c, const ModelKernel &model, double noise_var, const double *y,
                          const double *err_y, double diag_add, double *ll_data_out, double *logdet_half_out);

static int edge_timeout_fallback(gpt_ctx *c)
{
    g_flags_tripped.store(true);
    hipStreamSynchronize(c->stream);
    hipStreamSynchronize(c->panel_stream);
    static bool told = false;
    if (!told) {
        told = true;
        fprintf(stderr, "libgpt_hip: a flag-edge wait timed out (GPU shared with other work, or kernels serialised by a tool); "
                        "this process uses event edges from now on (GPT_EDGE_FLAGS=0 avoids the attempt)\n");
    }
    return GPT_OK;
}

static int fit_terms(gpt_ctx *c, const ModelKernel &model, double noise_var, const double *y, const double *err_y,
                     double diag_add, double *ll_data_out, double *logdet_half_out)
{
    int rc;
    {
        EvalScope scope(c);
        rc = fit_terms_once(c, model, noise_var, y, err_y, diag_add, ll_data_out, logdet_half_out);
    }
    if (rc == GPT_I_EDGE_TIMEOUT) {
        edge_timeout_fallback(c);
        EvalScope scope(c);
        rc = fit_terms_once(c, model, noise_var, y, err_y, diag_add, ll_data_out, logdet_half_out);
    }
    return rc;
}

static int fit_terms_once(gpt_ctx *c, const ModelKernel &model, double noise_var, const double *y,
                          const double *err_y, double diag_add, double *ll_data_out, double *logdet_half_out)
{
    const int64_t Nx = c->Nx;
    const int64_t N = c->dT ? c->Ny : Nx;
    const double *mX = model_X(c), *mS = model_S(c);
    c->N = N;
    GPT_TRY(ensure_factor_storage(c, N));
    hipStream_t st = c->stream;
    c->factored = false;
    if (c->timing) GPT_HIP_CHECK(hipEventRecord(c->tev[0], st));
    memcpy(c->h_yerr, y, (size_t)N * sizeof(double));
    memcpy(c->h_yerr + c->NP, err_y, (size_t)N * sizeof(double));
    const int64_t NP = c->NP;
    const bool one_launch = (c->dT == nullptr) && NP > N;
    if (!one_launch) {
        GPT_HIP_CHECK(hipMemcpyAsync(c->d_y, c->h_yerr, (size_t)(c->NP + N) * sizeof(double), hipMemcpyHostToDevice, st));
        if (c->timing) GPT_HIP_CHECK(hipEventRecord(c->tev[1], st));
        GPT_HIP_CHECK(hipMemsetAsync(c->d_info, 0, sizeof(int32_t), st));
    }
    c->model = model;
    if (c->dT) {
        const int64_t NxP = c->NxP, NyP = round_up(N, 64);
        double *dK, *dTK, *dzero;
        GPT_TRY(ensure(c, SLOT_KFULL, (size_t)NxP * NxP * sizeof(double), (void **)&dK));
        GPT_TRY(ensure(c, SLOT_TK, (size_t)NyP * NxP * sizeof(double), (void **)&dTK));
        GPT_TRY(ensure(c, SLOT_ZERO, (size_t)Nx * sizeof(double), (void **)&dzero));
        GPT_HIP_CHECK(hipMemsetAsync(dzero, 0, (size_t)Nx * sizeof(double), st));
        if (NxP > Nx) GPT_HIP_CHECK(hipMemsetAsync(dK, 0, (size_t)NxP * NxP * sizeof(double), st));
        GPT_TRY(kbuild_terms(st, c->model, 1, mX, c->dn, Nx, mX, c->dn, Nx, 0, 0, 0, dzero, noise_var, 0.0, dK, NxP, mS, mS));
        GPT_TRY(gemm_nt(c, st, NyP, NxP, NxP, 1.0, c->dT, NxP, dK, NxP, 0.0, dTK, NxP, 0));
        GPT_TRY(gemm_nt(c, st, NyP, NyP, NxP, 1.0, dTK, NxP, c->dT, NxP, 0.0, c->dA, NP, 1));
        GPT_TRY(launch_add_diag(st, c->dA, NP, N, c->d_erry, diag_add));
        GPT_TRY(launch_fill_pad(st, c->dA, NP, N, NP, c->d_y, 1e300));
        c->have_kernel = true;
        return factor_and_ll(c, N, ll_data_out, logdet_half_out, true);
    }
    if (one_launch) {
        GPT_TRY(launch_upload_pad(st, c->h_yerr, c->d_y, NP + N, c->d_info, c->dA, NP, N, NP, 1e300));
        if (c->timing) GPT_HIP_CHECK(hipEventRecord(c->tev[1], st));
    } else {
        GPT_TRY(launch_fill_pad(st, c->dA, NP, N, NP, c->d_y, 1e300));
    }
    const int64_t w0 = (c->nb_early > outer_width(c, NP)) ? c->nb_early : outer_width(c, NP);
    int64_t head = round_up((c->ramp ? 128 : w0) + GPT_PANEL_EXT, 256);
    PotrfRequest req;
    hipEvent_t e_head = nullptr;
    const bool head_flag = c->flags_now && c->edge_seq < 0xf0000000u;
    if (c->lookahead && !c->use_graph && head < N && (head_flag || (e_head = get_event(c, 0)) != nullptr)) {
        GPT_TRY(kbuild_terms(st, c->model, 1, mX, c->dn, N, mX, c->dn, head, 1, 0, 0, c->d_erry, noise_var, diag_add,
                             c->dA, NP, mS, mS));
        if (head_flag) {
            req.head_wait = new_edge(c, 48);
            if (c->edge_test_stall) c->edge_test_stall = 0;
            else GPT_TRY(launch_set_flag(st, req.head_wait.word, req.head_wait.value));
        } else {
            GPT_HIP_CHECK(hipEventRecord(e_head, st));
        }
        GPT_TRY(kbuild_terms(st, c->model, 1, mX + head * c->D, c->dn + head * c->D, N - head, mX + head * c->D,
                             c->dn + head * c->D, N - head, 1, head, head, c->d_erry, noise_var, diag_add,
                             c->dA + head * NP + head, NP, mS ? mS + head : nullptr, mS ? mS + head : nullptr));
    } else {
        GPT_TRY(kbuild_terms(st, c->model, 1, mX, c->dn, N, mX, c->dn, N, 1, 0, 0, c->d_erry, noise_var, diag_add,
                             c->dA, NP, mS, mS));
    }
    c->have_kernel = true;
    req.head_event = e_head;
    return factor_and_ll(c, N, ll_data_out, logdet_half_out, true, req);
}

static int fit_matrix_once(gpt_ctx *c, const double *K_tot, int64_t N, const double *y, double *ll_data_out,
                           double *logdet_half_out);

extern "C" int gpt_fit_matrix(gpt_ctx *c, const double *K_tot, int64_t N, const double *y, double *ll_data_out,
                              double *logdet_half_out)
{
    CTX_ENTER(c);
    if (!K_tot || !y || N <= 0) return GPT_E_ARG;
    int rc;
    {
        EvalScope scope(c);
        rc = fit_matrix_once(c, K_tot, N, y, ll_data_out, logdet_half_out);
    }
    if (rc == GPT_I_EDGE_TIMEOUT) {
        edge_timeout_fallback(c);
        EvalScope scope(c);
        rc = fit_matrix_once(c, K_tot, N, y, ll_data_out, logdet_half_out);
    }
    return rc;
}

static int fit_matrix_once(gpt_ctx *c, const double *K_tot, int64_t N, const double *y, double *ll_data_out,
                           double *logdet_half_out)
{
    GPT_TRY(ensure_factor_storage(c, N));
    hipStream_t st = c->stream;
    c->factored = false;
    c->have_kernel = false;
    c->N = N;
    if (c->timing) {
        GPT_HIP_CHECK(hipEventRecord(c->tev[0], st));
        GPT_HIP_CHECK(hipEventRecord(c->tev[1], st));
    }
    GPT_HIP_CHECK(hipMemcpyAsync(c->d_y, y, (size_t)N * sizeof(double), hipMemcpyHostToDevice, st));
    GPT_HIP_CHECK(hipMemcpy2DAsync(c->dA, (size_t)c->NP * sizeof(double), K_tot, (size_t)N * sizeof(double),
                                   (size_t)N * sizeof(double), (size_t)N, hipMemcpyHostToDevice, st));
    return factor_and_ll(c, N, ll_data_out, logdet_half_out);
}
```

gptools_amd/csrc/api_schedule.inc:

```
#define GPT_PANEL_PRIO 2
static int gemm_nt(gpt_ctx *c, hipStream_t st, int64_t m, int64_t n, int64_t k, double alpha, const double *A,
                   int64_t lda, const double *B, int64_t ldb, double beta, double *C, int64_t ldc, int tri,
                   hipEvent_t done = nullptr, EdgeSig edge = EdgeSig(), EdgeSig wait = EdgeSig(), int64_t edge_cols = 0,
                   EdgeSig tail = EdgeSig())
{
    const double elems = tri ? 0.5 * (double)n * (double)(n + 1) + (double)(m - n) * (double)n : (double)m * (double)n;
    const double flops = 2.0 * (double)k * elems;
    const bool on_main = st == c->stream;
    const bool prof = c->prof_gemm && flops >= 1.0e9 && on_main;
    gpt_ctx::GemmProf *gp = nullptr;
    if (prof) {
        if (c->gprof_used == c->gprof.size()) {
            gpt_ctx::GemmProf g;
            GPT_HIP_CHECK(hipEventCreate(&g.e0));
            GPT_HIP_CHECK(hipEventCreate(&g.e1));
            g.flops = 0;
            g.stop = g.e1;
            c->gprof.push_back(g);
        }
        gp = &c->gprof[c->gprof_used++];
        gp->flops = flops;
        gp->bytes = 16.0 * elems + 8.0 * (double)k * (double)(m > n ? m : n);
    }
    const int lds_pad = on_main ? (c->lookahead ? c->gemm_pad : (int)c->dev_gemm_pad) : 0;
    const bool ext = !c->use_graph && (c->tile == 0 || c->tile == 64);
    hipEvent_t e0 = nullptr, e1 = nullptr;
    if (ext) {
        e0 = prof ? gp->e0 : nullptr;
        e1 = done ? done : (prof ? gp->e1 : nullptr);
        if (prof) gp->stop = e1;
    } else if (prof) {
        gp->stop = gp->e1;
        GPT_HIP_CHECK(hipEventRecord(gp->e0, st));
    }
    {
        static FILE *glog = getenv("GPT_GEMM_LOG") ? fopen(getenv("GPT_GEMM_LOG"), "a") : nullptr;
        if (glog && flops >= 1.0e9 && on_main) {
            const int64_t nt64 = ((m + 63) / 64) * ((n + 63) / 64);
            const int k64 = (c->tile == 64) || !(c->tile == 0 && nt64 < gemm_small_threshold() && !e0 && edge_cols == 0);
            fprintf(glog, "%lld %lld %lld %d %.6e %d\n", (long long)m, (long long)n, (long long)k, tri, flops, k64);
            fflush(glog);
        }
    }
    const int prio = (c->gemm_prio >= 0) ? (int)c->gemm_prio : (!on_main && c->lookahead) ? GPT_PANEL_PRIO : 0;
    int rc = launch_gemm_nt(st, m, n, k, alpha, A, lda, B, ldb, beta, C, ldc, tri, c->tile, lds_pad, e0, e1, prio, edge, wait, edge_cols, 1, 0, tail);
    if (!ext) {
        if (prof) GPT_HIP_CHECK(hipEventRecord(gp->e1, st));
        if (done) GPT_HIP_CHECK(hipEventRecord(done, st));
    }
    return rc;
}

static inline int64_t outer_width(const gpt_ctx *c, int64_t n)
{
    if (c->nb_outer > 0) return c->nb_outer;
    return (n <= 5120) ? 256 : (n <= 12288) ? 384 : 640;
}

#include <atomic>
#include <chrono>
#include <condition_variable>
#include <mutex>
static std::mutex g_eval_mu;
static std::condition_variable g_eval_cv;
static int g_evals = 0;
static int g_flag_evals = 0;
static int g_announced = 0;
static std::atomic<bool> g_flags_tripped{false};
static std::chrono::steady_clock::time_point g_contention_until;
#define GPT_I_EDGE_TIMEOUT (-100)

static bool edge_flags_env_ok()
{
    static int flags_ok = -1;
    if (flags_ok < 0) {
        const char *e = getenv("GPT_EDGE_FLAGS"), *r = getenv("ROCPROF_COUNTER_COLLECTION");
        flags_ok = !((e && atoi(e) == 0) || (r && r[0] && r[0] != '0' && r[0] != 'F' && r[0] != 'f'));
    }
    return flags_ok != 0;
}

struct EvalScope {
    gpt_ctx *c;
    bool flags;
    explicit EvalScope(gpt_ctx *c_, bool never_flags = false) : c(c_), flags(false)
    {
        std::unique_lock<std::mutex> lk(g_eval_mu);
        const auto now = std::chrono::steady_clock::now();
        if (never_flags) {
            if (g_flag_evals != 0) {
                g_contention_until = now + std::chrono::milliseconds(100);
                g_eval_cv.wait(lk, [] { return g_flag_evals == 0; });
            }
            if (g_evals != 0 && g_announced == 0) g_contention_until = now + std::chrono::milliseconds(100);
            g_evals++;
            c->flags_now = false;
            return;
        }
        if (g_flag_evals != 0) {
            g_contention_until = now + std::chrono::milliseconds(100);
            g_eval_cv.wait(lk, [] { return g_flag_evals == 0; });
        }
        flags = edge_flags_env_ok() && !g_flags_tripped.load() && g_evals == 0 && g_announced == 0 && c->edge_flags &&
                c->own_stream && c->d_edge && !c->use_graph && now >= g_contention_until;
        if (g_evals != 0 && g_announced == 0) g_contention_until = now + std::chrono::milliseconds(100);
        g_evals++;
        if (flags) g_flag_evals++;
        c->flags_now = flags;
    }
    ~EvalScope()
    {
        std::lock_guard<std::mutex> lk(g_eval_mu);
        g_evals--;
        if (flags) g_flag_evals--;
        c->flags_now = false;
        g_eval_cv.notify_all();
    }
};

extern "C" int gpt_concurrency_hint(int delta)
{
    std::lock_guard<std::mutex> lk(g_eval_mu);
    g_announced += delta;
    if (g_announced < 0) g_announced = 0;
    return g_announced;
}

static bool gemm_may_wait_in_kernel(const gpt_ctx *c, int64_t m, int64_t n)
{
    if (!(c->tile == 0 || c->tile == 64)) return false;
    const int64_t nt64 = ((m + 63) / 64) * ((n + 63) / 64);
    return nt64 < gemm_small_threshold() && ((m + 31) / 32) * ((n + 31) / 32) <= 1024;
}
static inline EdgeSig new_edge(gpt_ctx *c, int word)
{
    EdgeSig e;
    e.word = c->d_edge + word;
    e.value = ++c->edge_seq;
    e.err = c->d_edge + 60;
    return e;
}

static bool leaf_is_fused(const gpt_ctx *c, int64_t m) { return c->fuse_trsm > 0 && m >= 128 && m <= c->fuse_trsm && !c->use_graph; }
static int64_t leaf_workgroups(const gpt_ctx *c, int64_t m)
{
    if (!leaf_is_fused(c, m)) return 1;
    const int code = strip_rows_code(c, m);
    return code > 0 ? 1 + m / (128 >> code) : 1 + (m + 127) / 128;
}

static int leaf_factor(gpt_ctx *c, hipStream_t st, double *Ad, int64_t lda, double *ws, int32_t *info, int64_t base, int64_t m,
                       hipEvent_t done_ev = nullptr, EdgeSig done_edge = EdgeSig(), EdgeSig wait = EdgeSig())
{
    if (leaf_is_fused(c, m)) {
        if (c->flag_epoch > 0x3fffff00u) {
            GPT_HIP_CHECK(hipMemsetAsync(c->d_flag, 0, 256, st));
            c->flag_epoch = 0;
        }
        c->flag_epoch += 32;
        return launch_potf2_trsm(st, Ad, lda, ws, info, base, m, c->d_flag, c->flag_epoch, done_ev, done_edge, wait, strip_rows_code(c, m));
    }
    GPT_TRY(launch_potf2_diag(st, Ad, lda, ws, info, base, wait));
    GPT_TRY(launch_trsm_panel(st, m, Ad, lda, ws, Ad + 128 * lda, lda, c->use_graph ? nullptr : done_ev, done_edge));
    if (done_ev && c->use_graph) GPT_HIP_CHECK(hipEventRecord(done_ev, st));
    return GPT_OK;
}

static int panel_rec(gpt_ctx *c, hipStream_t st, double *Ap, int64_t lda, int64_t m, int64_t w, double *invd,
                     int32_t *info, int64_t base)
{
    if (w == 128) return leaf_factor(c, st, Ap, lda, invd, info, base, m - 128);
    const int64_t h = (w / 256) * 128 > 0 ? (w / 256) * 128 : 128;
    GPT_TRY(panel_rec(c, st, Ap, lda, m, h, invd, info, base));
    GPT_TRY(gemm_nt(c, st, m - h, w - h, h, -1.0, Ap + h * lda, lda, Ap + h * lda, lda, 1.0, Ap + h * lda + h, lda, 1));
    return panel_rec(c, st, Ap + h * lda + h, lda, m - h, w - h, invd + (h / 128) * GPT_WS_BLOCK, info, base + h);
}

struct PotrfRequest {
    hipEvent_t head_event = nullptr;
    EdgeSig head_wait;
    bool defer_join = false;
    bool want_early_binv = false;
    bool defer_pad_leaf = false;
};
struct PotrfResult {
    hipStream_t tail_stream = nullptr;
    bool pad_leaf_deferred = false;
};
struct PanelShared {
    EdgeSig first_wait;
    bool defer_pad = false;
    bool pad_leaf_deferred = false;
    std::vector<int64_t> pad_upd_lc;
};

#define GPT_PANEL_EXT 128
static int panel_ext_ll(gpt_ctx *c, hipStream_t st, double *A, int64_t lda, int64_t n, int64_t c0, int64_t w,
                        double *invd, int32_t *info, hipEvent_t wait_ev, hipEvent_t done_ev)
{
    bool waited = (wait_ev == nullptr);
    for (int64_t lc = c0; lc < c0 + w; lc += 128) {
        const int64_t kk = lc - c0;
        if (kk > 0) {
            if (!waited) {
                GPT_HIP_CHECK(hipStreamWaitEvent(st, wait_ev, 0));
                waited = true;
            }
            GPT_TRY(gemm_nt(c, st, n - lc, 128, kk, -1.0, A + lc * lda + c0, lda, A + lc * lda + c0, lda, 1.0,
                            A + lc * lda + lc, lda, 1));
        }
        const bool last = (lc + 128 == c0 + w);
        GPT_TRY(leaf_factor(c, st, A + lc * lda + lc, lda, invd + (lc / 128) * GPT_WS_BLOCK, info, lc, n - (lc + 128),
                            last ? done_ev : nullptr));
    }
    const int64_t e0 = c0 + w;
    if (e0 < n) {
        if (!waited) GPT_HIP_CHECK(hipStreamWaitEvent(st, wait_ev, 0));
        const int64_t ew = (n - e0 < GPT_PANEL_EXT) ? n - e0 : GPT_PANEL_EXT;
        GPT_TRY(gemm_nt(c, st, n - e0, ew, w, -1.0, A + e0 * lda + c0, lda, A + e0 * lda + c0, lda, 1.0,
                        A + e0 * lda + e0, lda, 1));
    }
    return GPT_OK;
}

#define GPT_INNER_ROWS 4608
#define GPT_HEAD_WAIT_WGS 33
static int panel_ext(gpt_ctx *c, PanelShared &ps, hipStream_t st, double *A, int64_t lda, int64_t n, int64_t c0, int64_t w,
                     double *invd, int32_t *info, hipEvent_t wait_ev, hipEvent_t done_ev, hipEvent_t first_ev,
                     EdgeSig wait_edge, EdgeSig done_edge)
{
    if (c->inner == 1 || (c->inner == 2 && n - c0 <= GPT_INNER_ROWS))
        return panel_ext_ll(c, st, A, lda, n, c0, w, invd, info, wait_ev, done_ev);
    const int64_t cend = (c0 + w + GPT_PANEL_EXT < n) ? c0 + w + GPT_PANEL_EXT : n;
    for (int64_t lc = c0; lc < c0 + w; lc += 128) {
        const int64_t r1 = lc + 128;
        const bool last = (r1 == c0 + w);
        const int64_t m = n - r1;
        if (ps.defer_pad && m == 0) {
            ps.pad_leaf_deferred = true;
            if (last && done_ev) GPT_HIP_CHECK(hipEventRecord(done_ev, st));
            if (lc == c0 && wait_ev) GPT_HIP_CHECK(hipStreamWaitEvent(st, wait_ev, 0));
            continue;
        }
        EdgeSig fw;
        if (lc == 0 && ps.first_wait.word) {
            fw = ps.first_wait;
            ps.first_wait = EdgeSig();
            if (leaf_workgroups(c, m) > GPT_HEAD_WAIT_WGS) {
                GPT_TRY(launch_wait_flag(st, fw));
                fw = EdgeSig();
            }
        }
        GPT_TRY(leaf_factor(c, st, A + lc * lda + lc, lda, invd + (lc / 128) * GPT_WS_BLOCK, info, lc, m, last ? done_ev : nullptr,
                            last ? done_edge : EdgeSig(), fw));
        if (lc == c0 && wait_ev) GPT_HIP_CHECK(hipStreamWaitEvent(st, wait_ev, 0));
        int64_t cend_p = cend;
        if (ps.defer_pad && cend == n) {
            ps.pad_upd_lc.push_back(lc);
            cend_p = n - 128;
            if (cend_p <= r1 && first_ev) {
                GPT_HIP_CHECK(hipEventRecord(first_ev, st));
                first_ev = nullptr;
            }
        }
        if (cend_p > r1) {
            EdgeSig inwait;
            if (lc == c0 && wait_edge.word) {
                if (gemm_may_wait_in_kernel(c, n - r1, cend_p - r1)) inwait = wait_edge;
                else GPT_TRY(launch_wait_flag(st, wait_edge));
            }
            GPT_TRY(gemm_nt(c, st, n - r1, cend_p - r1, 128, -1.0, A + r1 * lda + lc, lda, A + r1 * lda + lc, lda, 1.0,
                            A + r1 * lda + r1, lda, 1, first_ev, EdgeSig(), inwait));
            first_ev = nullptr;
        }
    }
    return GPT_OK;
}

static int enqueue_early_block_inverses(gpt_ctx *c, hipStream_t S, int64_t cols, int64_t cols_final);
#define GPT_MERGE_MIN_TILES 512
static int potrf_enqueue(gpt_ctx *c, int64_t n, double *A, int64_t lda, double *invd, int32_t *info, const PotrfRequest &req,
                         PotrfResult *res)
{
    if (n % 128) {
        gpt_set_error("potrf: n must be a multiple of 128 (n=%lld)", (long long)n);
        return GPT_E_ARG;
    }
    const int64_t nbo = outer_width(c, n);
    const int64_t nblk = (n + nbo - 1) / nbo;
    const hipStream_t S = c->stream, P = c->panel_stream;
    const bool la = c->lookahead && nblk > 1;
    auto update = [&](hipStream_t st, int64_t pc0, int64_t pw, int64_t a, int64_t b, hipEvent_t done = nullptr, EdgeSig edge = EdgeSig(),
                      EdgeSig wait = EdgeSig(), int64_t edge_cols = 0, EdgeSig tail = EdgeSig()) -> int {
        return gemm_nt(c, st, n - a, b - a, pw, -1.0, A + a * lda + pc0, lda, A + a * lda + pc0, lda, 1.0, A + a * lda + a, lda, 1,
                       done, edge, wait, edge_cols, tail);
    };
    if (!la) {
        for (int64_t k = 0; k < nblk; k++) {
            const int64_t c0 = k * nbo, w = (n - c0 < nbo) ? n - c0 : nbo, m = n - c0;
            GPT_TRY(panel_rec(c, S, A + c0 * lda + c0, lda, m, w, invd + (c0 / 128) * GPT_WS_BLOCK, info, c0));
            if (c0 + w < n) GPT_TRY(update(S, c0, w, c0 + w, n));
        }
        return GPT_OK;
    }
    const bool graph = c->use_graph != 0;
    const bool tile64 = (c->tile == 0 || c->tile == 64);
    const hipStream_t H = (c->helper_stream && !graph && c->helper_tf > 0 && n > c->helper_min_n) ? c->helper_stream : nullptr;
    const double rate_s = 46e12, rate_h = 1e11 * (double)c->helper_tf * (double)c->helper_cus / 24.0;
    const bool use_flags = c->flags_now && !H && c->inner == 0 && c->defer_rows == 0 && tile64;
    const int64_t purg_eff = (H || graph || (use_flags && c->merge_urgent)) ? 0 : c->purg_rows;
    const bool rest_flag = use_flags && c->edge_flags >= 2;
    const bool tail_here = use_flags && c->tail_wait != 0 && !c->prof_gemm;
    const int64_t defer_rows = (!H && !graph) ? c->defer_rows : 0;
    std::vector<int64_t> widths;
    {
        int64_t c0 = 0, w = c->ramp ? 128 : nbo;
        while (c0 < n) {
            const int64_t cap = (c->nb_early > 0 && n - c0 > c->nb_switch_rows) ? c->nb_early : nbo;
            if (w > cap || (!c->ramp)) w = cap;
            if (w > n - c0) w = n - c0;
            widths.push_back(w);
            c0 += w;
            w += 128;
        }
    }
    const size_t np = widths.size();

    PanelShared ps;
    ps.defer_pad = req.defer_pad_leaf && c->inner == 0 && !graph;
    if (req.head_wait.word && c->inner == 0) {
        ps.first_wait = req.head_wait;
    } else {
        hipEvent_t head = req.head_event;
        if (!head) {
            head = get_event(c, 0);
            if (!head) return GPT_E_HIP;
            GPT_HIP_CHECK(hipEventRecord(head, S));
        }
        GPT_HIP_CHECK(hipStreamWaitEvent(P, head, 0));
    }
    if (use_flags && c->edge_seq > 0xf0000000u && !req.head_wait.word) {
        GPT_HIP_CHECK(hipStreamSynchronize(S));
        GPT_HIP_CHECK(hipStreamSynchronize(P));
        GPT_HIP_CHECK(hipMemsetAsync(c->d_edge, 0, 256, S));
        GPT_HIP_CHECK(hipStreamSynchronize(S));
        c->edge_seq = 0;
        c->alpha_counter = 0;
    }
    hipEvent_t e_cu_prev = nullptr, e_help_prev = nullptr, e_rest_prev = nullptr;
    EdgeSig cu_edge_prev, rest_edge_prev;
    EdgeSig next_panel_edge;
    int64_t c0 = 0, s_prev = 0;
    int64_t awaited = 0;
    struct PendingRest { bool on; int64_t c0, w, u1, split; } pend = {false, 0, 0, 0, 0};
    for (size_t k = 0; k < np; c0 += widths[k], k++) {
        const int64_t w = widths[k];
        const int64_t wn = (k + 1 < np) ? widths[k + 1] : 0;
        hipEvent_t e_panel = get_event(c, 2 + 4 * k), e_cu = get_event(c, 3 + 4 * k), e_help = get_event(c, 4 + 4 * k);
        hipEvent_t e_sdone = get_event(c, 5 + 4 * k);
        if (!e_panel || !e_cu || !e_help || !e_sdone) return GPT_E_HIP;
        hipEvent_t e_first = pend.on ? get_event(c, 8 + 4 * np + k) : nullptr;
        if (pend.on && !e_first) return GPT_E_HIP;
        const int64_t u0 = c0 + w + GPT_PANEL_EXT;
        EdgeSig panel_edge;
        bool panel_awaited = false;
        if (use_flags && u0 < n) {
            panel_awaited = next_panel_edge.word != nullptr;
            panel_edge = panel_awaited ? next_panel_edge : new_edge(c, 0);
        }
        next_panel_edge = EdgeSig();
        GPT_TRY(panel_ext(c, ps, P, A, lda, n, c0, w, invd, info, e_cu_prev, use_flags ? nullptr : e_panel, e_first, cu_edge_prev,
                          panel_edge));
        e_cu_prev = nullptr;
        cu_edge_prev = EdgeSig();
        if (pend.on) {
            GPT_HIP_CHECK(hipStreamWaitEvent(S, e_first, 0));
            GPT_TRY(update(S, pend.c0, pend.w, pend.u1, pend.split));
            pend.on = false;
        }
        if (u0 >= n) continue;
        const int64_t u1 = (u0 + wn < n) ? u0 + wn : n;
        int64_t split = n;
        if (H && u1 < n) {
            const double side0 = (double)(n - u1);
            int64_t side = (int64_t)(sqrt(rate_h / (rate_s + rate_h)) * side0) / 64 * 64;
            if (n - side < s_prev) side = n - s_prev;
            if (side >= 1024 && n - side > u1 && (double)w * side0 * side0 >= 1e10) split = n - side;
        }
        if (split < n && !e_help_prev) {
            GPT_HIP_CHECK(hipEventRecord(e_sdone, S));
            GPT_HIP_CHECK(hipStreamWaitEvent(H, e_sdone, 0));
        }
        if (!use_flags) GPT_HIP_CHECK(hipStreamWaitEvent(S, e_panel, 0));
        else if (!panel_awaited) GPT_TRY(launch_wait_flag(S, panel_edge));
        awaited = c0 + w;
        EdgeSig tail;
        if (tail_here && split == n && k + 1 < np && u0 + wn < n) tail = new_edge(c, 0);
        if (split < n) {
            if (use_flags) GPT_TRY(launch_wait_flag(H, panel_edge));
            else GPT_HIP_CHECK(hipStreamWaitEvent(H, e_panel, 0));
            GPT_TRY(update(H, c0, w, split, n, e_help));
        }
        bool help_waited = false;
        if (e_help_prev && u1 > s_prev) {
            GPT_HIP_CHECK(hipStreamWaitEvent(S, e_help_prev, 0));
            help_waited = true;
        }
        auto wait_help_prev = [&]() -> int {
            if (e_help_prev && !help_waited) GPT_HIP_CHECK(hipStreamWaitEvent(S, e_help_prev, 0));
            e_help_prev = nullptr;
            return GPT_OK;
        };
        if (purg_eff > 0 && n - c0 > purg_eff && u1 < n) {
            if (e_rest_prev) GPT_HIP_CHECK(hipStreamWaitEvent(P, e_rest_prev, 0));
            if (!e_rest_prev && !rest_edge_prev.word) {
                hipEvent_t e_k = get_event(c, 9 + 5 * np);
                if (!e_k) return GPT_E_HIP;
                GPT_HIP_CHECK(hipEventRecord(e_k, S));
                GPT_HIP_CHECK(hipStreamWaitEvent(P, e_k, 0));
            }
            EdgeSig rwait;
            if (rest_edge_prev.word) {
                if (gemm_may_wait_in_kernel(c, n - u0, u1 - u0)) rwait = rest_edge_prev;
                else GPT_TRY(launch_wait_flag(P, rest_edge_prev));
            }
            GPT_TRY(update(P, c0, w, u0, u1, nullptr, EdgeSig(), rwait));
            e_rest_prev = nullptr;
            rest_edge_prev = EdgeSig();
            if (rest_flag) {
                rest_edge_prev = new_edge(c, 32);
                GPT_TRY(update(S, c0, w, u1, n, nullptr, rest_edge_prev));
            } else {
                e_rest_prev = get_event(c, 10 + 5 * np + k);
                if (!e_rest_prev) return GPT_E_HIP;
                GPT_TRY(update(S, c0, w, u1, n, e_rest_prev));
            }
            continue;
        }
        e_rest_prev = nullptr;
        rest_edge_prev = EdgeSig();
        if (use_flags) {
            cu_edge_prev = new_edge(c, 16);
            const int64_t mtn = (split - u0 + 63) / 64, mtm = (n - u0 + 63) / 64;
            const int64_t nt64m = mtn * (mtn + 1) / 2 + (mtm - mtn) * mtn;
            if (c->merge_urgent && u1 < split && nt64m >= GPT_MERGE_MIN_TILES && (u1 - u0) % 64 == 0) {
                GPT_TRY(wait_help_prev());
                GPT_TRY(update(S, c0, w, u0, split, nullptr, cu_edge_prev, EdgeSig(), u1 - u0, tail));
                next_panel_edge = tail;
                if (split < n) {
                    s_prev = split;
                    e_help_prev = e_help;
                }
                continue;
            }
            GPT_TRY(update(S, c0, w, u0, u1, nullptr, cu_edge_prev));
        } else {
            GPT_TRY(update(S, c0, w, u0, u1, e_cu));
            e_cu_prev = e_cu;
        }
        if (u1 < n) {
            GPT_TRY(wait_help_prev());
            if (defer_rows > 0 && n - c0 <= defer_rows && k + 1 < np) {
                pend = PendingRest{true, c0, w, u1, split};
            } else {
                GPT_TRY(update(S, c0, w, u1, split, nullptr, EdgeSig(), EdgeSig(), 0, tail));
                next_panel_edge = tail;
            }
            if (split < n) {
                s_prev = split;
                e_help_prev = e_help;
            }
        }
    }
    if (pend.on) GPT_TRY(update(S, pend.c0, pend.w, pend.u1, pend.split));
    if (req.want_early_binv && A == c->dA && invd == c->d_invd && np >= 2)
        GPT_TRY(enqueue_early_block_inverses(c, S, n - widths.back(), awaited));
    if (ps.pad_leaf_deferred) {
        hipEvent_t e_real = get_event(c, 12 + 6 * np);
        if (!e_real) return GPT_E_HIP;
        GPT_HIP_CHECK(hipEventRecord(e_real, P));
        GPT_HIP_CHECK(hipStreamWaitEvent(S, e_real, 0));
        const int64_t pc = n - 128;
        for (const int64_t lc : ps.pad_upd_lc)
            GPT_TRY(gemm_nt(c, S, 128, 128, 128, -1.0, A + pc * lda + lc, lda, A + pc * lda + lc, lda, 1.0, A + pc * lda + pc, lda, 1));
        GPT_TRY(launch_potf2_diag(S, A + pc * lda + pc, lda, invd + (pc / 128) * GPT_WS_BLOCK, info, pc));
        res->pad_leaf_deferred = true;
    }
    if (e_help_prev) GPT_HIP_CHECK(hipStreamWaitEvent(S, e_help_prev, 0));
    if (req.defer_join && !graph) {
        res->tail_stream = P;
        return GPT_OK;
    }
    hipEvent_t e_end = get_event(c, 1);
    if (!e_end) return GPT_E_HIP;
    GPT_HIP_CHECK(hipEventRecord(e_end, P));
    GPT_HIP_CHECK(hipStreamWaitEvent(S, e_end, 0));
    return GPT_OK;
}

static int potrf_run(gpt_ctx *c, int64_t n, double *A, int64_t lda, double *invd, int32_t *info,
                     const PotrfRequest &req = PotrfRequest(), PotrfResult *res = nullptr)
{
    PotrfResult unused;
    if (!res) res = &unused;
    *res = PotrfResult();
    if (!c->use_graph) return potrf_enqueue(c, n, A, lda, invd, info, req, res);
    if (c->gexec && (c->g_n != n || c->g_nb != c->nb_outer || c->g_la != c->lookahead || c->g_A != A)) {
        hipGraphExecDestroy(c->gexec);
        c->gexec = nullptr;
    }
    if (!c->gexec) {
        hipGraph_t graph = nullptr;
        GPT_HIP_CHECK(hipStreamBeginCapture(c->stream, hipStreamCaptureModeRelaxed));
        int rc = potrf_enqueue(c, n, A, lda, invd, info, req, res);
        hipError_t e = hipStreamEndCapture(c->stream, &graph);
        if (rc != GPT_OK) {
            if (graph) hipGraphDestroy(graph);
            return rc;
        }
        GPT_HIP_CHECK(e);
        GPT_HIP_CHECK(hipGraphInstantiate(&c->gexec, graph, nullptr, nullptr, 0));
        hipGraphDestroy(graph);
        c->g_n = n;
        c->g_nb = c->nb_outer;
        c->g_la = c->lookahead;
        c->g_A = A;
    }
    GPT_HIP_CHECK(hipGraphLaunch(c->gexec, c->stream));
    return GPT_OK;
}

static int trsm_rlt(gpt_ctx *c, hipStream_t st, int64_t m, int64_t n, const double *L, int64_t ldl, const double *invd,
                    double *B, int64_t ldb)
{
    if (n == 128) return launch_trsm_panel(st, m, L, ldl, invd, B, ldb);
    const int64_t h = (n / 256) * 128 > 0 ? (n / 256) * 128 : 128;
    GPT_TRY(trsm_rlt(c, st, m, h, L, ldl, invd, B, ldb));
    GPT_TRY(gemm_nt(c, st, m, n - h, h, -1.0, B, ldb, L + h * ldl, ldl, 1.0, B + h, ldb, 0));
    return trsm_rlt(c, st, m, n - h, L + h * ldl + h, ldl, invd + (h / 128) * GPT_WS_BLOCK, B + h, ldb);
}
```

gptools_amd/csrc/api_solve.inc:

```
#define GPT_FEW_ROWS 128
__global__ void eye_strip_kernel(double *__restrict__ U, int64_t n, int64_t w)
{
    const int64_t i = (int64_t)blockIdx.x * blockDim.x + threadIdx.x;
    if (i < n) U[i * w + i % w] = 1.0;
}

__global__ __launch_bounds__(256) void transpose_strip_kernel(const double *__restrict__ U, double *__restrict__ W, int64_t w)
{
    __shared__ double t[32][33];
    const int tx = threadIdx.x & 31, ty = threadIdx.x >> 5;
    const int64_t r0 = (int64_t)blockIdx.y * 32, c0 = (int64_t)blockIdx.x * 32, o = (int64_t)blockIdx.z * w * w;
    for (int i = ty; i < 32; i += 8) t[i][tx] = U[o + (r0 + i) * w + c0 + tx];
    __syncthreads();
    for (int i = ty; i < 32; i += 8) W[o + (c0 + i) * w + r0 + tx] = t[tx][i];
}

static int build_block_inverses_512(gpt_ctx *c, hipStream_t st, int64_t nblk, double *U, double *W)
{
    const int64_t nb = 512, bs = nb * nb, NP = c->NP, bsl = nb * (NP + 1), WS = GPT_WS_BLOCK;
    GPT_HIP_CHECK(hipMemsetAsync(U, 0, (size_t)nblk * bs * sizeof(double), st));
    hipLaunchKernelGGL(eye_strip_kernel, dim3((unsigned)((nblk * nb + 255) / 256)), dim3(256), 0, st, U, nblk * nb, nb);
    GPT_LAUNCH_CHECK();
    for (int p = 0; p < 4; p++)
        GPT_TRY(launch_trsm_panel(st, 128, nullptr, 0, c->d_invd + p * WS, U + (int64_t)p * 128 * nb + p * 128, nb, nullptr, EdgeSig(),
                                  nblk, bs, 4 * WS));
    for (int q = 0; q < 4; q += 2) {
        const int64_t lo = q * 128, mid = lo + 128;
        GPT_TRY(launch_gemm_nt(st, 128, 128, 128, -1.0, U + lo * nb + lo, nb, c->dA + mid * NP + lo, NP, 0.0, U + lo * nb + mid, nb, 0,
                               0, 0, nullptr, nullptr, 0, EdgeSig(), EdgeSig(), 0, nblk, bs, EdgeSig(), bsl, bs));
        GPT_TRY(launch_trsm_panel(st, 128, nullptr, 0, c->d_invd + (q + 1) * WS, U + lo * nb + mid, nb, nullptr, EdgeSig(), nblk, bs,
                                  4 * WS));
    }
    GPT_TRY(launch_gemm_nt(st, 256, 256, 256, -1.0, U, nb, c->dA + 256 * NP, NP, 0.0, U + 256, nb, 0, 0, 0, nullptr, nullptr, 0, EdgeSig(),
                           EdgeSig(), 0, nblk, bs, EdgeSig(), bsl, bs));
    GPT_TRY(launch_trsm_panel(st, 256, nullptr, 0, c->d_invd + 2 * WS, U + 256, nb, nullptr, EdgeSig(), nblk, bs, 4 * WS));
    GPT_TRY(launch_gemm_nt(st, 256, 128, 128, -1.0, U + 256, nb, c->dA + 384 * NP + 256, NP, 1.0, U + 384, nb, 0, 0, 0, nullptr, nullptr, 0,
                           EdgeSig(), EdgeSig(), 0, nblk, bs, EdgeSig(), bsl, bs));
    GPT_TRY(launch_trsm_panel(st, 256, nullptr, 0, c->d_invd + 3 * WS, U + 384, nb, nullptr, EdgeSig(), nblk, bs, 4 * WS));
    hipLaunchKernelGGL(transpose_strip_kernel, dim3((unsigned)(nb / 32), (unsigned)(nb / 32), (unsigned)nblk), dim3(256), 0, st, U, W, nb);
    GPT_LAUNCH_CHECK();
    return GPT_OK;
}

static int ensure_block_inverses_wide(gpt_ctx *c, int64_t nb, int64_t nfull, double **out);
static int ensure_block_inverses(gpt_ctx *c, int64_t nb, int64_t nfull, double **out, double **out_u, hipStream_t on)
{
    if (nb == GPT_BINV_NB2) return ensure_block_inverses_wide(c, nb, nfull, out);
    const int64_t nall = (c->NP / nb) * nb;
    if (nfull > nall || nall <= 0) {
        gpt_set_error("block inverses: extent %lld exceeds the padded order %lld", (long long)nfull, (long long)c->NP);
        return GPT_E_ARG;
    }
    double *W, *Us = nullptr;
    GPT_TRY(ensure(c, SLOT_BINV, (size_t)nall * nb * sizeof(double), (void **)&W));
    GPT_TRY(ensure(c, SLOT_BINVU, (size_t)nall * nb * sizeof(double), (void **)&Us));
    *out = W;
    if (out_u) *out_u = Us;
    if (c->binv_valid) return GPT_OK;
    hipStream_t st = on ? on : c->stream;
    if (c->binv_launches) {
        GPT_TRY(build_block_inverses_512(c, st, nall / nb, Us, W));
    } else {
        const int64_t b0 = c->binv_early;
        GPT_TRY(launch_trinv512(st, nall / nb - b0, c->dA + b0 * nb * (c->NP + 1), c->NP, c->d_invd + b0 * (nb / 128) * GPT_WS_BLOCK,
                                Us + b0 * nb * nb, W + b0 * nb * nb));
        if (b0 > 0 && c->e_binv_early && st != c->stream) GPT_HIP_CHECK(hipStreamWaitEvent(st, c->e_binv_early, 0));
        c->binv_early = 0;
    }
    c->binv_valid = true;
    return GPT_OK;
}

static int enqueue_early_block_inverses(gpt_ctx *c, hipStream_t S, int64_t cols, int64_t cols_final)
{
    const int64_t nb = GPT_BINV_NB, nall = (c->NP / nb) * nb;
    int64_t b = cols / nb;
    c->binv_early = 0;
    if (c->binv_launches || nall < 2 * nb || b <= 0 || b >= nall / nb) return GPT_OK;
    if (b * nb > cols_final) b = cols_final / nb;
    if (b <= 0) return GPT_OK;
    double *W, *Us = nullptr;
    GPT_TRY(ensure(c, SLOT_BINV, (size_t)nall * nb * sizeof(double), (void **)&W));
    GPT_TRY(ensure(c, SLOT_BINVU, (size_t)nall * nb * sizeof(double), (void **)&Us));
    GPT_TRY(launch_trinv512(S, b, c->dA, c->NP, c->d_invd, Us, W));
    if (!c->e_binv_early) GPT_HIP_CHECK(hipEventCreateWithFlags(&c->e_binv_early, hipEventDisableTiming));
    GPT_HIP_CHECK(hipEventRecord(c->e_binv_early, S));
    c->binv_early = b;
    return GPT_OK;
}

#define GPT_BINV_NB3 2048
static int ensure_block_inverses_wide(gpt_ctx *c, int64_t nb, int64_t nfull, double **out)
{
    const bool w3 = (nb == GPT_BINV_NB3);
    double *W, *U, *T, *Wb;
    if (nfull > (c->NP / nb) * nb) {
        gpt_set_error("block inverses: extent %lld exceeds the padded order %lld", (long long)nfull, (long long)c->NP);
        return GPT_E_ARG;
    }
    nfull = (c->NP / nb) * nb;
    GPT_TRY(ensure(c, w3 ? SLOT_BINV3 : SLOT_BINV2, (size_t)nfull * nb * sizeof(double), (void **)&W));
    *out = W;
    bool &valid = w3 ? c->binv3_valid : c->binv2_valid;
    if (valid) return GPT_OK;
    GPT_TRY(ensure_block_inverses(c, GPT_BINV_NB, nfull, &Wb));
    GPT_TRY(ensure(c, SLOT_BINV3U, (size_t)2 * nfull * nb * sizeof(double), (void **)&U));
    T = U + nfull * nb;
    hipStream_t st = c->stream;
    GPT_HIP_CHECK(hipMemsetAsync(U, 0, (size_t)nfull * nb * sizeof(double), st));
    const WideBatch wb = {nfull / nb, nb * nb, nb * nb, nb * (c->NP + 1), nb * GPT_BINV_NB};
    GPT_TRY(trtri_u_gemm_b(c, st, 0, nb, Wb, U, nb, T, nb, wb));
    hipLaunchKernelGGL(transpose_rect_kernel, dim3((unsigned)(nb / 32), (unsigned)(nb / 32), (unsigned)wb.n), dim3(256), 0, st, U, nb, W, nb, nb,
                       nb, nb * nb, nb * nb);
    GPT_LAUNCH_CHECK();
    valid = true;
    if (c->slots[SLOT_BINV3U].cap > ((size_t)256 << 20)) {
        GPT_HIP_CHECK(hipStreamSynchronize(st));
        DevBuf &b = c->slots[SLOT_BINV3U];
        GPT_HIP_CHECK(hipFree(b.p));
        b.p = nullptr;
        b.cap = 0;
    }
    return GPT_OK;
}

static int trsm_rlt_binv(gpt_ctx *c, hipStream_t st, int64_t m, int64_t nb, int64_t lo, int64_t hi, const double *W, double *B,
                         int64_t ldb, double *V, int64_t ldv)
{
    const int64_t n = hi - lo;
    if (n == nb) return gemm_nt(c, st, m, nb, nb, 1.0, B + lo, ldb, W + lo * nb, nb, 0.0, V + lo, ldv, 0);
    const int64_t h = (n / (2 * nb)) * nb > 0 ? (n / (2 * nb)) * nb : nb;
    const int64_t mid = lo + h;
    GPT_TRY(trsm_rlt_binv(c, st, m, nb, lo, mid, W, B, ldb, V, ldv));
    GPT_TRY(gemm_nt(c, st, m, hi - mid, h, -1.0, V + lo, ldv, c->dA + mid * c->NP + lo, c->NP, 1.0, B + mid, ldb, 0));
    return trsm_rlt_binv(c, st, m, nb, mid, hi, W, B, ldb, V, ldv);
}

__global__ __launch_bounds__(256) void splitk_reduce_kernel(int64_t m, int64_t n2, int S, const double2 *__restrict__ P, int64_t pstride2,
                                                            double beta, double *__restrict__ C, int64_t ldc)
{
    const int64_t i = (int64_t)blockIdx.x * 256 + threadIdx.x;
    if (i >= m * n2) return;
    const int64_t r = i / n2, q = i - r * n2;
    double2 *cp = reinterpret_cast<double2 *>(C + r * ldc) + q;
    double2 acc = make_double2(0.0, 0.0);
    if (beta != 0.0) {
        acc = *cp;
        acc.x *= beta;
        acc.y *= beta;
    }
    if (S % 8 == 0) {
        for (int s = 0; s < S; s += 8) {
            double2 p[8];
#pragma unroll
            for (int q = 0; q < 8; q++) p[q] = P[(int64_t)(s + q) * pstride2 + i];
#pragma unroll
            for (int q = 0; q < 8; q++) {
                acc.x += p[q].x;
                acc.y += p[q].y;
            }
        }
    } else {
        for (int s = 0; s < S; s += 2) {
            const double2 p0 = P[(int64_t)s * pstride2 + i], p1 = P[(int64_t)(s + 1) * pstride2 + i];
            acc.x = (acc.x + p0.x) + p1.x;
            acc.y = (acc.y + p0.y) + p1.y;
        }
    }
    *cp = acc;
}

static int gemm_nt_few(gpt_ctx *c, hipStream_t st, int64_t m, int64_t n, int64_t k, double alpha, const double *A, int64_t lda,
                       const double *B, int64_t ldb, double beta, double *C, int64_t ldc, int tri = 0)
{
    const int64_t tiles = ((m + 31) / 32) * ((n + 31) / 32);
    int64_t S = 1;
    if (c->splitk && !c->use_graph && c->tile == 0 && k >= 1024 && (n % 2) == 0 && (ldc % 2) == 0)
        while (S < 32 && tiles * S < c->splitk && (k / (2 * S)) >= 256 && (k % (2 * S * 16)) == 0) S *= 2;
    if (S == 1) return gemm_nt(c, st, m, n, k, alpha, A, lda, B, ldb, beta, C, ldc, tri);
    double *P;
    const int64_t pstride = ((m + 31) / 32) * 32 * n;
    GPT_TRY(ensure(c, SLOT_SPLITK, (size_t)S * pstride * sizeof(double), (void **)&P));
    const int64_t kc = k / S;
    GPT_TRY(launch_gemm_nt(st, m, n, kc, alpha, A, lda, B, ldb, 0.0, P, n, 0, 0, 0, nullptr, nullptr, 0, EdgeSig(), EdgeSig(), 0, S, kc,
                           EdgeSig(), kc, pstride));
    const int64_t n2 = n / 2, tot = m * n2;
    hipLaunchKernelGGL(splitk_reduce_kernel, dim3((unsigned)((tot + 255) / 256)), dim3(256), 0, st, m, n2, (int)S,
                       reinterpret_cast<const double2 *>(P), pstride / 2, beta, C, ldc);
    GPT_LAUNCH_CHECK();
    return GPT_OK;
}

static int solve_rows_resident(gpt_ctx *c, hipStream_t st, int64_t m, int64_t n128, double *B, int64_t ldb, double *V, int64_t ldv)
{
    const int64_t nfull = (n128 / GPT_BINV_NB) * GPT_BINV_NB;
    if (nfull < 2 * GPT_BINV_NB) {
        GPT_TRY(launch_copy2d(st, m, n128, B, ldb, V, ldv));
        return trsm_rlt(c, st, m, n128, c->dA, c->NP, c->d_invd, V, ldv);
    }
    double *W;
    GPT_TRY(ensure_block_inverses(c, GPT_BINV_NB, nfull, &W));
    const int64_t rem = n128 - nfull;
    if (m <= 256) {
        double *W3 = nullptr, *W2 = nullptr;
        int64_t n3 = 0, n2 = 0;
        if (m <= GPT_FEW_ROWS && n128 >= 4 * GPT_BINV_NB3) {
            n3 = (n128 / GPT_BINV_NB3) * GPT_BINV_NB3;
            GPT_TRY(ensure_block_inverses_wide(c, GPT_BINV_NB3, n3, &W3));
        } else if (m <= GPT_FEW_ROWS && n128 >= 4 * GPT_BINV_NB2) {
            n2 = (n128 / GPT_BINV_NB2) * GPT_BINV_NB2;
            GPT_TRY(ensure_block_inverses(c, GPT_BINV_NB2, n2, &W2));
        }
        int64_t j = 0;
        while (j < nfull) {
            const int64_t nb = (j + GPT_BINV_NB3 <= n3) ? GPT_BINV_NB3 : (j + GPT_BINV_NB2 <= n2) ? GPT_BINV_NB2 : GPT_BINV_NB;
            const double *Wj = (nb == GPT_BINV_NB3) ? W3 + j * nb : (nb == GPT_BINV_NB2) ? W2 + j * nb : W + j * nb;
            GPT_TRY(gemm_nt_few(c, st, m, nb, nb, 1.0, B + j, ldb, Wj, nb, 0.0, V + j, ldv));
            const int64_t r0 = j + nb;
            if (r0 < n128)
                GPT_TRY(gemm_nt_few(c, st, m, n128 - r0, nb, -1.0, V + j, ldv, c->dA + r0 * c->NP + j, c->NP, 1.0, B + r0, ldb));
            j = r0;
        }
    } else {
        GPT_TRY(trsm_rlt_binv(c, st, m, GPT_BINV_NB, 0, nfull, W, B, ldb, V, ldv));
        if (rem > 0) GPT_TRY(gemm_nt(c, st, m, rem, nfull, -1.0, V, ldv, c->dA + nfull * c->NP, c->NP, 1.0, B + nfull, ldb, 0));
    }
    if (rem > 0) {
        GPT_TRY(launch_copy2d(st, m, rem, B + nfull, ldb, V + nfull, ldv));
        GPT_TRY(trsm_rlt(c, st, m, rem, c->dA + nfull * c->NP + nfull, c->NP, c->d_invd + (nfull / 128) * GPT_WS_BLOCK, V + nfull, ldv));
    }
    return GPT_OK;
}

#define GPT_STAGE_BYTES ((size_t)16 << 20)
struct StagePending { double *dst; int64_t ldd, rows, cols; bool on; };
static thread_local StagePending g_stage_pend[2] = {{nullptr, 0, 0, 0, false}, {nullptr, 0, 0, 0, false}};
static thread_local int g_stage_next = 0;

static bool host_ptr_is_pinned(const void *p)
{
    hipPointerAttribute_t at;
    if (hipPointerGetAttributes(&at, p) != hipSuccess) {
        (void)hipGetLastError();
        return false;
    }
    return at.type == hipMemoryTypeHost;
}

static int stage_drain(gpt_ctx *c, int slot)
{
    StagePending &p = g_stage_pend[slot];
    if (!p.on) return GPT_OK;
    GPT_HIP_CHECK(hipEventSynchronize(c->cev[slot]));
    const double *src = c->h_stage + (size_t)slot * (GPT_STAGE_BYTES / sizeof(double));
    for (int64_t r = 0; r < p.rows; r++) memcpy(p.dst + r * p.ldd, src + r * p.cols, (size_t)p.cols * sizeof(double));
    p.on = false;
    return GPT_OK;
}

static int d2h_rows(gpt_ctx *c, double *dst, int64_t ldd, const double *dsrc, int64_t lds, int64_t rows, int64_t cols)
{
    if (host_ptr_is_pinned(dst)) {
        GPT_HIP_CHECK(hipMemcpy2DAsync(dst, (size_t)ldd * sizeof(double), dsrc, (size_t)lds * sizeof(double),
                                       (size_t)cols * sizeof(double), (size_t)rows, hipMemcpyDeviceToHost, c->copy_stream));
        return GPT_OK;
    }
    if (!c->h_stage) GPT_HIP_CHECK(hipHostMalloc((void **)&c->h_stage, 2 * GPT_STAGE_BYTES, hipHostMallocDefault));
    const int64_t per = (int64_t)(GPT_STAGE_BYTES / sizeof(double)) / cols;
    if (per < 1) {
        gpt_set_error("d2h_rows: a row of %lld doubles exceeds the staging slot", (long long)cols);
        return GPT_E_ARG;
    }
    for (int64_t r0 = 0; r0 < rows; r0 += per) {
        const int64_t nr = (rows - r0 < per) ? rows - r0 : per;
        const int slot = g_stage_next;
        g_stage_next ^= 1;
        GPT_TRY(stage_drain(c, slot));
        double *ring = c->h_stage + (size_t)slot * (GPT_STAGE_BYTES / sizeof(double));
        GPT_HIP_CHECK(hipMemcpy2DAsync(ring, (size_t)cols * sizeof(double), dsrc + r0 * lds, (size_t)lds * sizeof(double),
                                       (size_t)cols * sizeof(double), (size_t)nr, hipMemcpyDeviceToHost, c->copy_stream));
        GPT_HIP_CHECK(hipEventRecord(c->cev[slot], c->copy_stream));
        g_stage_pend[slot] = StagePending{dst + r0 * ldd, ldd, nr, cols, true};
    }
    return GPT_OK;
}

static int d2h_finish(gpt_ctx *c)
{
    GPT_TRY(stage_drain(c, g_stage_next));
    GPT_TRY(stage_drain(c, g_stage_next ^ 1));
    GPT_HIP_CHECK(hipStreamSynchronize(c->copy_stream));
    return GPT_OK;
}

extern "C" int gpt_host_alloc(int64_t bytes, void **out)
{
    if (!out || bytes <= 0) return GPT_E_ARG;
    *out = nullptr;
    GPT_HIP_CHECK(hipHostMalloc(out, (size_t)bytes, hipHostMallocDefault));
    return GPT_OK;
}

extern "C" int gpt_mem_info(gpt_ctx *c, int64_t *free_bytes, int64_t *total_bytes)
{
    CTX_ENTER(c);
    size_t f = 0, t = 0;
    GPT_HIP_CHECK(hipMemGetInfo(&f, &t));
    if (free_bytes) *free_bytes = (int64_t)f;
    if (total_bytes) *total_bytes = (int64_t)t;
    return GPT_OK;
}

extern "C" int gpt_release_batch_scratch(gpt_ctx *c)
{
    CTX_ENTER(c);
    GPT_HIP_CHECK(hipStreamSynchronize(c->stream));
    GPT_HIP_CHECK(hipStreamSynchronize(c->panel_stream));
    c->batch_gen++;
    for (int slot : {SLOT_BATCH_A, SLOT_BATCH_WS, SLOT_BATCH_MISC, SLOT_PB_V, SLOT_PB_COV, SLOT_PB_MISC}) {
        DevBuf &b = c->slots[slot];
        if (b.p) GPT_HIP_CHECK(hipFree(b.p));
        b.p = nullptr;
        b.cap = 0;
    }
    return GPT_OK;
}

extern "C" int gpt_host_free(void *p)
{
    if (p) GPT_HIP_CHECK(hipHostFree(p));
    return GPT_OK;
}
```

gptools_amd/csrc/common.hpp:

```cpp
#pragma once
#include <hip/hip_runtime.h>
#include <hip/hip_ext.h>
#include <stdint.h>
#include <stdio.h>
#include "../../include/gpt_hip.h"

typedef double f64x4 __attribute__((ext_vector_type(4)));
typedef double f64x2 __attribute__((ext_vector_type(2)));

#define GPT_WAVE 64
#define GPT_WS_BLOCK 9216
#define GPT_WS_LOFF 2048

void gpt_set_error(const char *fmt, ...);

#define GPT_HIP_CHECK(expr)                                                              \
    do {                                                                                 \
        hipError_t e_ = (expr);                                                          \
        if (e_ != hipSuccess) {                                                          \
            gpt_set_error("%s failed: %s (%s:%d)", #expr, hipGetErrorString(e_), __FILE__, __LINE__); \
            return (e_ == hipErrorOutOfMemory) ? GPT_E_NOMEM : GPT_E_HIP;                \
        }                                                                                \
    } while (0)

#define GPT_LAUNCH_CHECK()                                                               \
    do {                                                                                 \
        hipError_t e_ = hipGetLastError();                                               \
        if (e_ != hipSuccess) {                                                          \
            gpt_set_error("kernel launch failed: %s (%s:%d)", hipGetErrorString(e_), __FILE__, __LINE__); \
            return GPT_E_HIP;                                                            \
        }                                                                                \
    } while (0)

struct KParams {
    int kernel_id;
    int D;
    int hyper_deriv;
    int symmetric;
    double sigma;
    double alpha;
    double l[GPT_MAX_DIM];
    double inv_l[GPT_MAX_DIM];
    double inv_var[GPT_MAX_DIM];
    int noise_n[GPT_MAX_DIM];
    double m_cnu;
    double m_mu;
    int m_nint;
    int m_isint;
    int zero_l;
    int pad_;
    double m_gampl, m_gammi, m_gam1, m_gam2;
    double m_g[2], m_gm[2], m_nus[2];
    double g_amp[2], g_w[2], g_x0[2], g_c;
    int g_nt, g_pad_;
};

struct EdgeSig {
    unsigned *word = nullptr;
    unsigned value = 0;
    unsigned *err = nullptr;
};
#define GPT_EDGE_TIMEOUT_TICKS 25000000ll
#ifdef __HIPCC__
__device__ __forceinline__ void edge_signal(unsigned *word, unsigned value, unsigned total)
{
    asm volatile("s_waitcnt vmcnt(0)" ::: "memory");
    __syncthreads();
    if (threadIdx.x == 0) {
        const unsigned done = __hip_atomic_fetch_add(word + 1, 1u, __ATOMIC_RELAXED, __HIP_MEMORY_SCOPE_AGENT) + 1u;
        if (done == total) {
            __hip_atomic_store(word + 1, 0u, __ATOMIC_RELAXED, __HIP_MEMORY_SCOPE_AGENT);
            __hip_atomic_store(word, value, __ATOMIC_RELAXED, __HIP_MEMORY_SCOPE_SYSTEM);
        }
    }
}
template <int SLEEP, bool ACQUIRE>
__device__ __forceinline__ void edge_poll(const unsigned *word, unsigned value, unsigned *err)
{
    if ((int)(__hip_atomic_load(word, __ATOMIC_RELAXED, __HIP_MEMORY_SCOPE_SYSTEM) - value) < 0) {
        const long long t0 = wall_clock64();
        while ((int)(__hip_atomic_load(word, __ATOMIC_RELAXED, __HIP_MEMORY_SCOPE_SYSTEM) - value) < 0) {
            __builtin_amdgcn_s_sleep(SLEEP);
            if (err && wall_clock64() - t0 > GPT_EDGE_TIMEOUT_TICKS) {
                __hip_atomic_store(err, 1u, __ATOMIC_RELAXED, __HIP_MEMORY_SCOPE_SYSTEM);
                break;
            }
        }
    }
    if (ACQUIRE) __builtin_amdgcn_fence(__ATOMIC_ACQUIRE, "agent");
}
#endif

int launch_kpairs(hipStream_t st, const KParams &kp, const double *dXi, const double *dXj,
                  const int32_t *dni, const int32_t *dnj, int64_t M, double *dout, int accumulate = 0,
                  const KParams *kp2 = nullptr);
int launch_kbuild(hipStream_t st, const KParams &kp, const double *dXi, const int32_t *dni, int64_t M,
                  const double *dXj, const int32_t *dnj, int64_t P, int lower_only, int64_t i0, int64_t j0,
                  const double *d_err_y, double noise_var, double diag_add, double *dK, int64_t ldk,
                  int accumulate = 0, const KParams *kp2 = nullptr, const double *dSi = nullptr, const double *dSj = nullptr);
int launch_kbuild_prod(hipStream_t st, const KParams &kp1, const KParams &kp2, const double *dXi, const int32_t *dni, int64_t M,
                       const double *dXj, const int32_t *dnj, int64_t P, int lower_only, int64_t i0, int64_t j0,
                       const double *d_err_y, double noise_var, double diag_add, double *dK, int64_t ldk, int accumulate,
                       const double *dSi = nullptr, const double *dSj = nullptr);
int launch_kpairs_prod(hipStream_t st, const KParams &kp1, const KParams &kp2, const double *dXi, const double *dXj,
                       const int32_t *dni, const int32_t *dnj, int64_t M, double *dout, int accumulate);
int launch_check_orders(hipStream_t st, const int32_t *dn, int64_t M, int D, int32_t *d_flag);
int launch_gemm_nt(hipStream_t st, int64_t m, int64_t n, int64_t k, double alpha, const double *A, int64_t lda,
                   const double *B, int64_t ldb, double beta, double *C, int64_t ldc, int tri, int force_tile, int lds_pad,
                   hipEvent_t ev0 = nullptr, hipEvent_t ev1 = nullptr, int prio = 0, EdgeSig edge = EdgeSig(),
                   EdgeSig wait = EdgeSig(), int64_t edge_cols = 0, int64_t nbatch = 1, int64_t bstride = 0,
                   EdgeSig tail = EdgeSig(), int64_t bstride_b = -1, int64_t bstride_c = -1);
int launch_potf2_diag(hipStream_t st, double *A, int64_t lda, double *invd, int32_t *info, int64_t info_base,
                      EdgeSig wait = EdgeSig(), int64_t nbatch = 1, int64_t bstride_a = 0, int64_t bstride_ws = 0);
int launch_gemm_nt_stair(hipStream_t st, int64_t m, int64_t nseg, int64_t seg_cols, int64_t k, double alpha,
                         const double *A, int64_t lda, const double *B, int64_t ldb, int64_t b_stride, int64_t row_step,
                         double beta, double *C, int64_t ldc, int lds_pad, hipEvent_t ev0 = nullptr,
                         hipEvent_t ev1 = nullptr);
int launch_gemm_nt_gridstair(hipStream_t st, int64_t m, int64_t nseg, int64_t seg_cols, int64_t k, double alpha, const double *A,
                             int64_t lda, const double *B, int64_t ldb, int64_t off, int64_t num, int64_t den, int64_t base,
                             double beta, double *C, int64_t ldc, int lds_pad, hipEvent_t ev0 = nullptr, hipEvent_t ev1 = nullptr);
int launch_potf2_trsm(hipStream_t st, double *A, int64_t lda, double *invd, int32_t *info, int64_t info_base, int64_t m,
                      unsigned *flag, unsigned flag_base, hipEvent_t done = nullptr, EdgeSig edge = EdgeSig(),
                      EdgeSig wait = EdgeSig(), int rows64 = 0);
int launch_trsm_panel(hipStream_t st, int64_t m, const double *L, int64_t ldl, const double *invd,
                      double *B, int64_t ldb, hipEvent_t done = nullptr, EdgeSig edge = EdgeSig(), int64_t nbatch = 1,
                      int64_t bstride_b = 0, int64_t bstride_ws = 0);
int launch_kbuild_batch(hipStream_t st, int kernel_id, int D, const KParams *d_kps, const double *d_noise_var, int64_t nbatch,
                        const double *dX, const int32_t *dn, int64_t N, const double *d_err_y, double diag_add, double *dK,
                        int64_t ldk, int64_t bstride, int accumulate = 0, int full = 0, const KParams *d_kps2 = nullptr,
                        int64_t xstride = 0, const double *dS = nullptr, int64_t sstride = 0);
int launch_batch_pad(hipStream_t st, const double *h_y, int64_t nbatch, double *A, int64_t lda, int64_t bstride, int64_t n_valid,
                     int64_t n_pad, double big, int32_t *info);
int launch_kbuild_batch_cross(hipStream_t st, int kernel_id, int D, const KParams *d_kps, const double *d_nv, int64_t nbatch,
                              const double *dXi, const int32_t *dni, int64_t M, const double *dXj, const int32_t *dnj, int64_t P, double *dK,
                              int64_t ldk, int64_t bstride, int accumulate = 0, const KParams *d_kps2 = nullptr);
int launch_kdiag_batch(hipStream_t st, int D, int nterms, const KParams *d_kps, const KParams *d_kps2, int64_t nbatch, const double *dX,
                       const int32_t *dn, int64_t M, double *dout, int64_t ldo);
int launch_kss_sum(hipStream_t st, int D, int nterms, const KParams *d_kps, const KParams *d_kps2, int64_t nbatch, const int32_t *d_keep,
                   const double *dX, const int32_t *dn, int64_t M, int64_t MP, const int32_t *d_hit, double noise_sum, double *dC,
                   int64_t ldc);
int launch_batch_meanvar(hipStream_t st, int64_t M, int64_t MP, int64_t N, int64_t NP, int64_t nbatch, double *V, int64_t ldv,
                         const double *A, int64_t bs, const int32_t *keep, double *mean, double *var, int64_t ld);
int launch_batch_logdet_dot(hipStream_t st, const double *A, int64_t lda, int64_t bstride, int64_t n, int64_t nbatch,
                            const int32_t *d_info, double *out3);
#define GPT_GRAD_MAXH 8
int grad_reduce_blocks(int64_t N);
int launch_grad_reduce(hipStream_t st, const KParams &kp, int nh, const int *hl, const double *dX, const int32_t *dn,
                       int64_t N, const double *dalpha, const double *dW, int64_t ldw, double *dpartial);
int launch_add_diag(hipStream_t st, double *A, int64_t lda, int64_t n, const double *err, double diag_add, int64_t nbatch = 1,
                    int64_t bstride = 0);
void gpt_jitter(hipStream_t st);
int launch_set_flag(hipStream_t st, unsigned *word, unsigned value);
int launch_wait_flag(hipStream_t st, EdgeSig w);
int gemm_small_threshold();
int launch_upload_pad(hipStream_t st, const double *h_src, double *d_dst, int64_t ncopy, int32_t *info, double *A,
                      int64_t lda, int64_t n_valid, int64_t n_pad, double big);
int launch_fill_pad(hipStream_t st, double *A, int64_t lda, int64_t n_valid, int64_t n_pad, const double *dy,
                    double big);
int launch_logdet_dot(hipStream_t st, const double *A, int64_t lda, int64_t n, const int32_t *d_info, double *d_part,
                      double *out4, hipEvent_t ev0 = nullptr, hipEvent_t ev1 = nullptr, unsigned *edge_err = nullptr);
int launch_extract_lower(hipStream_t st, const double *A, int64_t lda, int64_t n, double *out, int64_t ldo);
int launch_trsv_lt(hipStream_t st, int64_t n, const double *L, int64_t ldl, const double *invd, double *x, int64_t b_lo = 0);
int launch_trsv_lt_wide(hipStream_t st, int64_t nwide, const double *L, int64_t ldl, const double *U, double *w, double *x,
                        const double *w0 = nullptr);
int launch_alpha_init(hipStream_t st, int64_t n, int64_t np, const double *z, double *w, double *x);
int launch_gemv_n(hipStream_t st, int64_t m, int64_t n, const double *A, int64_t lda, const double *x, double *y);
int launch_trinv512(hipStream_t st, int64_t nblk, const double *L, int64_t ldl, const double *invd, double *U, double *W);
int launch_rowsumsq_sub(hipStream_t st, int64_t m, int64_t n, const double *V, int64_t ldv, const double *kdiag,
                        double *var_out);
int launch_add_noise_sym(hipStream_t st, const KParams &kp, const double *dX, const int32_t *dn, int64_t M,
                         double *C, int64_t ldc);
int launch_mirror_rows(hipStream_t st, double *A, int64_t lda, int64_t c0, int64_t w, int64_t n);
int launch_alpha_trace(hipStream_t st, const double *alpha, const double *W, int64_t ldw, int64_t n, double *out);
int launch_diag_gather(hipStream_t st, const double *A, int64_t lda, int64_t n, double *out);
int launch_copy2d(hipStream_t st, int64_t rows, int64_t cols, const double *src, int64_t lds, double *dst, int64_t ldd);
int launch_zero2d(hipStream_t st, int64_t rows, int64_t cols, double *dst, int64_t ldd);
int launch_pad_block(hipStream_t st, double *A, int64_t lda, int64_t c0, int64_t nb, int64_t n_valid, int64_t n_pad,
                     const double *dy, double big);
int launch_row_sumsq(hipStream_t st, const double *row, int64_t w, double *acc);
int launch_panel_scalars(hipStream_t st, const double *P, int64_t ldp, int64_t w, int64_t zrow, double *acc);
```

gptools_amd/csrc/solve.hip:

```cpp
#include "common.hpp"
#include <type_traits>
#define GPT_TRY_RC_SOLVE(expr) do { int rc_ = (expr); if (rc_ != GPT_OK) return rc_; } while (0)

__global__ void fill_pad_kernel(double *__restrict__ A, int64_t lda, int64_t n_valid, int64_t n_pad,
                                const double *__restrict__ dy, double big)
{
    const int64_t row = n_valid + blockIdx.y;
    const int64_t col = (int64_t)blockIdx.x * blockDim.x + threadIdx.x;
    if (row >= n_pad || col >= n_pad) return;
    double v = 0.0;
    if (row == n_valid && dy != nullptr) {
        if (col < n_valid) v = dy[col];
        else if (col == row) v = big;
    } else if (col == row) {
        v = 1.0;
    }
    A[row * lda + col] = v;
}

__global__ void set_flag_kernel(unsigned *word, unsigned value)
{
    __hip_atomic_store(word, value, __ATOMIC_RELEASE, __HIP_MEMORY_SCOPE_SYSTEM);
}

// ... 233 lines not shown
        }
        for (int off = 32; off > 0; off >>= 1) {
            a += __shfl_down(a, off);
            b += __shfl_down(b, off);
        }
        if (lane == 0) {
            s0[wave] = a;
            s1[wave] = b;
        }
        __syncthreads();
        if (threadIdx.x == 0) {
            p0[vw] = ((s0[0] + s0[1]) + s0[2]) + s0[3];
            p1[vw] = ((s1[0] + s1[1]) + s1[2]) + s1[3];
        }
        __syncthreads();
    }
    if (threadIdx.x < 64) {
        const unsigned w = threadIdx.x;
        double ta = (w < LD_WGS) ? p0[w] : 0.0, tb = (w < LD_WGS) ? p1[w] : 0.0;
        for (int off = 32; off > 0; off >>= 1) {
            ta += __shfl_down(ta, off);
            tb += __shfl_down(tb, off);
        }
        if (w == 0) {
            double *o = out + 4 * (int64_t)blockIdx.x;
            __hip_atomic_store(o + 0, ta, __ATOMIC_RELAXED, __HIP_MEMORY_SCOPE_SYSTEM);
            __hip_atomic_store(o + 1, tb, __ATOMIC_RELAXED, __HIP_MEMORY_SCOPE_SYSTEM);
            __hip_atomic_store(o + 2, (double)info[blockIdx.x], __ATOMIC_RELAXED, __HIP_MEMORY_SCOPE_SYSTEM);
        }
    }
}

int launch_batch_logdet_dot(hipStream_t st, const double *A, int64_t lda, int64_t bstride, int64_t n, int64_t nbatch,
                            const int32_t *d_info, double *out3)
{
    if (nbatch <= 0) return GPT_OK;
    hipLaunchKernelGGL(batch_logdet_dot_kernel, dim3((unsigned)nbatch), dim3(256), 0, st, A, lda, bstride, n, d_info, out3);
    GPT_LAUNCH_CHECK();
    return GPT_OK;
}

__global__ void extract_lower_kernel(const double *__restrict__ A, int64_t lda, int64_t n,
                                     double *__restrict__ out, int64_t ldo)
{
    const int64_t col = (int64_t)blockIdx.x * blockDim.x + threadIdx.x;
    if (col >= n) return;
    for (int64_t row = blockIdx.y; row < n; row += gridDim.y)
        out[row * ldo + col] = (col <= row) ? A[row * lda + col] : 0.0;
}

int launch_extract_lower(hipStream_t st, const double *A, int64_t lda, int64_t n, double *out, int64_t ldo)
{
    if (n <= 0) return GPT_OK;
    dim3 grid((unsigned)((n + 255) / 256), (unsigned)(n < 16384 ? n : 16384));
    hipLaunchKernelGGL(extract_lower_kernel, grid, dim3(256), 0, st, A, lda, n, out, ldo);
    GPT_LAUNCH_CHECK();
    return GPT_OK;
}

__global__ void copy2d_kernel(int64_t rows, int64_t cols, const double *__restrict__ src, int64_t lds,
                              double *__restrict__ dst, int64_t ldd)
{
    const int64_t col = (int64_t)blockIdx.x * blockDim.x + threadIdx.x;
    if (col >= cols) return;
    for (int64_t row = blockIdx.y; row < rows; row += gridDim.y) dst[row * ldd + col] = src[row * lds + col];
}

int launch_copy2d(hipStream_t st, int64_t rows, int64_t cols, const double *src, int64_t lds, double *dst, int64_t ldd)
{
    if (rows <= 0 || cols <= 0) return GPT_OK;
    dim3 grid((unsigned)((cols + 255) / 256), (unsigned)(rows < 16384 ? rows : 16384));
    hipLaunchKernelGGL(copy2d_kernel, grid, dim3(256), 0, st, rows, cols, src, lds, dst, ldd);
    GPT_LAUNCH_CHECK();
    return GPT_OK;
}

__global__ void zero2d_kernel(int64_t rows, int64_t cols, double *__restrict__ dst, int64_t ldd)
{
    const int64_t col = (int64_t)blockIdx.x * blockDim.x + threadIdx.x;
    if (col >= cols) return;
    for (int64_t row = blockIdx.y; row < rows; row += gridDim.y) dst[row * ldd + col] = 0.0;
}

int launch_zero2d(hipStream_t st, int64_t rows, int64_t cols, double *dst, int64_t ldd)
{
    if (rows <= 0 || cols <= 0) return GPT_OK;
    dim3 grid((unsigned)((cols + 255) / 256), (unsigned)(rows < 16384 ? rows : 16384));
    hipLaunchKernelGGL(zero2d_kernel, grid, dim3(256), 0, st, rows, cols, dst, ldd);
    GPT_LAUNCH_CHECK();
    return GPT_OK;
}

__global__ __launch_bounds__(256) void trsv_lt_diag_kernel(const double *__restrict__ Lbb, int64_t ldl,
                                                           const double *__restrict__ invd, double *__restrict__ x)
{
    (void)Lbb;
    (void)ldl;
    __shared__ double ws[GPT_WS_BLOCK];
    __shared__ double w[128], xb[16];
    const int tid = threadIdx.x;
    for (int i = tid; i < GPT_WS_BLOCK; i += 256) ws[i] = invd[i];
    if (tid < 128) w[tid] = x[tid];
    __syncthreads();
    const int j = tid >> 4, i = tid & 15;
    const int col = (i >> 2) * 64 + 16 * (i & 3);
    for (int b = 7; b >= 0; b--) {
        if (tid < 128 && j == b) {
            const double *inv = ws + b * 256 + col;
            double acc = 0.0;
#pragma unroll
            for (int k = 0; k < 16; k++) acc = fma(inv[k], w[b * 16 + k], acc);
            xb[i] = acc;
        }
        __syncthreads();
        if (tid < 128) {
            if (j == b) w[tid] = xb[i];
            else if (j < b) {
                const double *lb = ws + GPT_WS_LOFF + (b * (b - 1) / 2 + j) * 256 + col;
                double acc = w[tid];
#pragma unroll
                for (int k = 0; k < 16; k++) acc = fma(-lb[k], xb[k], acc);
                w[tid] = acc;
            }
        }
        __syncthreads();
    }
    if (tid < 128) x[tid] = w[tid];
}

__global__ __launch_bounds__(256) void trsv_lt_update_kernel(int64_t ncols, const double *__restrict__ Lrow,
                                                             int64_t ldl, const double *__restrict__ xb,
                                                             double *__restrict__ w)
{
    __shared__ double xs[128];
    if (threadIdx.x < 128) xs[threadIdx.x] = xb[threadIdx.x];
    __syncthreads();
    const int64_t col = (int64_t)blockIdx.x * 256 + threadIdx.x;
    if (col >= ncols) return;
    double acc = 0.0;
#pragma unroll 8
    for (int r = 0; r < 128; r++) acc = fma(Lrow[(int64_t)r * ldl + col], xs[r], acc);
    w[col] -= acc;
}

int launch_trsv_lt(hipStream_t st, int64_t n, const double *L, int64_t ldl, const double *invd, double *x, int64_t b_lo)
{
    if (n % 128) {
        gpt_set_error("trsv_lt: n must be a multiple of 128");
        return GPT_E_ARG;
    }
    for (int64_t b = n / 128 - 1; b >= b_lo; b--) {
        const double *Lbb = L + (b * 128) * ldl + b * 128;
        hipLaunchKernelGGL(trsv_lt_diag_kernel, dim3(1), dim3(256), 0, st, Lbb, ldl, invd + b * GPT_WS_BLOCK, x + b * 128);
        if (b > 0) {
            const int64_t ncols = b * 128;
            hipLaunchKernelGGL(trsv_lt_update_kernel, dim3((unsigned)((ncols + 255) / 256)), dim3(256), 0, st, ncols,
                               L + (b * 128) * ldl, ldl, x + b * 128, x);
        }
    }
    GPT_LAUNCH_CHECK();
    return GPT_OK;
}

#define TI_NB 512
#define TI_XS 513
__global__ __launch_bounds__(512, 2) void trinv512_kernel(int nblk, const double *__restrict__ L, int64_t ldl, const double *__restrict__ invd,
                                                          double *__restrict__ U, double *__restrict__ W)
{
    __shared__ double xs[16 * TI_XS];
    __shared__ double xt[2][256];
    __shared__ double dl[32 * 256];
    const int tid = threadIdx.x, lane = tid & 63, fr = lane & 15, fk = lane >> 4;
    const int w = __builtin_amdgcn_readfirstlane(tid >> 6);
    const int s = 31 - (int)blockIdx.x / nblk, b = (int)blockIdx.x % nblk;
    const double *Lb = L + (int64_t)b * TI_NB * (ldl + 1);
    const double *wsb = invd + (int64_t)b * 4 * GPT_WS_BLOCK;

    f64x4 acc[4];
#pragma unroll
    for (int t = 0; t < 4; t++) {
        acc[t] = f64x4{0.0, 0.0, 0.0, 0.0};
        if (8 * t + w == s) {
#pragma unroll
            for (int q = 0; q < 4; q++) acc[t][q] = (fk + 4 * q == fr) ? 1.0 : 0.0;
        }
    }
    f64x4 la[2][4];
    auto request = [&](f64x4 (&dst)[4], int k, auto nl) {
        const int kc = k > 0 ? k : 0;
#pragma unroll
        for (int t = 0; t < decltype(nl)::value; t++) {
            const double *p = Lb + (int64_t)(16 * kc + fk) * ldl + 16 * (8 * t + w) + fr;
#pragma unroll
            for (int u = 0; u < 4; u++) dst[t][u] = p[(int64_t)(4 * u) * ldl];
        }
    };
    auto solve = [&](const f64x4 &r, int k) {
        const double *dk = dl + k * 256 + 64 * (fr >> 2) + 16 * (fr & 3) + fk;
        f64x4 x = f64x4{0.0, 0.0, 0.0, 0.0};
#pragma unroll
        for (int u = 0; u < 4; u++) x = __builtin_amdgcn_mfma_f64_16x16x4f64(dk[4 * u], r[u], x, 0, 0, 0);
        *reinterpret_cast<f64x4 *>(&xt[k & 1][4 * lane]) = x;
#pragma unroll
        for (int q = 0; q < 4; q++) xs[fr * TI_XS + 16 * k + fk + 4 * q] = x[q];
    };
    auto nlive = [&](int k) { const int n = (k - w + 7) >> 3; return n < 0 ? 0 : (n > 4 ? 4 : n); };

    {
        double v[16];
        const int lim = 256 * (s + 1);
#pragma unroll
        for (int i = 0; i < 16; i++) {
            const int e = tid + 512 * i, ec = e < lim ? e : 0;
            v[i] = wsb[(int64_t)(ec >> 11) * GPT_WS_BLOCK + (ec & 2047)];
        }
#pragma unroll
        for (int i = 0; i < 16; i++) {
            const int e = tid + 512 * i;
            if (e < lim) dl[e] = v[i];
        }
    }
    request(la[0], s, std::integral_constant<int, 4>());
    request(la[1], s - 1, std::integral_constant<int, 4>());
    __syncthreads();
#pragma unroll
    for (int t = 0; t < 4; t++)
        if (8 * t + w == s) solve(acc[t], s);
    __syncthreads();
    auto step = [&](f64x4 (&lk)[4], int k, auto nl) {
        constexpr int NL = decltype(nl)::value;
        f64x4 xb = *reinterpret_cast<const f64x4 *>(&xt[k & 1][4 * lane]);
        xb = -xb;
        const int tn = (k - 1) >> 3;
        const bool next_owner = (w == ((k - 1) & 7));
        if (next_owner) {
#pragma unroll
            for (int t = 0; t < NL; t++)
                if (t == tn) {
#pragma unroll
                    for (int u = 0; u < 4; u++) acc[t] = __builtin_amdgcn_mfma_f64_16x16x4f64(lk[t][u], xb[u], acc[t], 0, 0, 0);
                    solve(acc[t], k - 1);
                }
        }
#pragma unroll
        for (int t = 0; t < NL; t++) {
            if (!(next_owner && t == tn)) {
#pragma unroll
                for (int u = 0; u < 4; u++) acc[t] = __builtin_amdgcn_mfma_f64_16x16x4f64(lk[t][u], xb[u], acc[t], 0, 0, 0);
            }
        }
        request(lk, k - 2, nl);
        __syncthreads();
    };
    int k = s;
    auto phase = [&](auto nl) {
        while (k > 0 && nlive(k) == decltype(nl)::value) {
            step(la[0], k, nl);
            if (k - 1 > 0) step(la[1], k - 1, nl);
            k -= 2;
        }
    };
    phase(std::integral_constant<int, 4>());
    phase(std::integral_constant<int, 3>());
    phase(std::integral_constant<int, 2>());
    phase(std::integral_constant<int, 1>());
    phase(std::integral_constant<int, 0>());

    double *Ub = U + (int64_t)b * TI_NB * TI_NB, *Wb = W + (int64_t)b * TI_NB * TI_NB;
    const int nz = 16 * s + 16;
    {
        double v[16];
#pragma unroll
        for (int i = 0; i < 16; i++) {
            const int e = tid + 512 * i, r = e >> 9, c = e & 511;
            v[i] = (c < nz) ? xs[r * TI_XS + c] : 0.0;
        }
#pragma unroll
        for (int i = 0; i < 16; i++) {
            const int e = tid + 512 * i, r = e >> 9, c = e & 511;
            Wb[(int64_t)(16 * s + r) * TI_NB + c] = v[i];
        }
#pragma unroll
        for (int i = 0; i < 16; i++) {
            const int e = tid + 512 * i, c = e >> 4, r = e & 15;
            v[i] = (c < nz) ? xs[r * TI_XS + c] : 0.0;
        }
#pragma unroll
        for (int i = 0; i < 16; i++) {
            const int e = tid + 512 * i, c = e >> 4, r = e & 15;
            Ub[(int64_t)c * TI_NB + 16 * s + r] = v[i];
        }
    }
}

int launch_trinv512(hipStream_t st, int64_t nblk, const double *L, int64_t ldl, const double *invd, double *U, double *W)
{
    if (nblk <= 0) return GPT_OK;
    hipLaunchKernelGGL(trinv512_kernel, dim3((unsigned)(32 * nblk)), dim3(512), 0, st, (int)nblk, L, ldl, invd, U, W);
    GPT_LAUNCH_CHECK();
    return GPT_OK;
}

#define TW_NB 512
__global__ __launch_bounds__(512) void gemv_t_sub_kernel(int64_t ncols, const double *__restrict__ M, int64_t ldm,
                                                         const double *__restrict__ x, double *__restrict__ w, const double *__restrict__ w_in)
{
    __shared__ double xs[TW_NB];
    __shared__ double part[32][17];
    const int tid = threadIdx.x, lane = tid & 63, g = tid >> 6, c = lane & 15, rs = lane >> 4;
    xs[tid] = x[tid];
    __syncthreads();
    const int64_t col = (int64_t)blockIdx.x * 16 + c;
    double a0 = 0.0, a1 = 0.0, a2 = 0.0, a3 = 0.0;
    if (col < ncols) {
        const int r0 = g * (TW_NB / 8) + rs;
        const double *p = M + (int64_t)r0 * ldm + col;
        double v[16];
#pragma unroll
        for (int i = 0; i < 16; i++) v[i] = p[(int64_t)(4 * i) * ldm];
#pragma unroll
        for (int i = 0; i < 16; i += 4) {
            a0 = fma(v[i + 0], xs[r0 + 4 * (i + 0)], a0);
            a1 = fma(v[i + 1], xs[r0 + 4 * (i + 1)], a1);
            a2 = fma(v[i + 2], xs[r0 + 4 * (i + 2)], a2);
            a3 = fma(v[i + 3], xs[r0 + 4 * (i + 3)], a3);
        }
    }
    part[g * 4 + rs][c] = (a0 + a1) + (a2 + a3);
    __syncthreads();
    if (tid < 16 && col < ncols) {
        double t = 0.0;
#pragma unroll
        for (int q = 0; q < 32; q++) t += part[q][tid];
        w[col] = w_in[col] - t;
    }
}

__global__ __launch_bounds__(256) void alpha_init_kernel(int64_t n, int64_t np, const double *__restrict__ z, double *__restrict__ w,
                                                         double *__restrict__ x)
{
    const int64_t i = (int64_t)blockIdx.x * 256 + threadIdx.x;
    if (i < np) {
        w[i] = i < n ? z[i] : 0.0;
        x[i] = 0.0;
    }
}
int launch_alpha_init(hipStream_t st, int64_t n, int64_t np, const double *z, double *w, double *x)
{
    hipLaunchKernelGGL(alpha_init_kernel, dim3((unsigned)((np + 255) / 256)), dim3(256), 0, st, n, np, z, w, x);
    GPT_LAUNCH_CHECK();
    return GPT_OK;
}

int launch_trsv_lt_wide(hipStream_t st, int64_t nwide, const double *L, int64_t ldl, const double *U, double *w, double *x, const double *w0)
{
    if (nwide % TW_NB) {
        gpt_set_error("trsv_lt_wide: the extent must be a multiple of %d", TW_NB);
        return GPT_E_ARG;
    }
    if (w0 && nwide < 2 * TW_NB) {
        gpt_set_error("trsv_lt_wide: w0 needs at least two blocks");
        return GPT_E_ARG;
    }
    const double *wsrc = w0 ? w0 : w;
    for (int64_t j0 = nwide - TW_NB; j0 >= 0; j0 -= TW_NB) {
        GPT_TRY_RC_SOLVE(launch_gemv_n(st, TW_NB, TW_NB, U + j0 * TW_NB, TW_NB, wsrc + j0, x + j0));
        if (j0 > 0)
            hipLaunchKernelGGL(gemv_t_sub_kernel, dim3((unsigned)(j0 / 16)), dim3(512), 0, st, j0, L + j0 * ldl, ldl, x + j0, w, wsrc);
        wsrc = w;
    }
    GPT_LAUNCH_CHECK();
    return GPT_OK;
}

template <int WAVES, bool SQ>
__global__ __launch_bounds__(256) void rowred_kernel(int64_t m, int64_t n, const double *__restrict__ A, int64_t lda,
                                                     const double *__restrict__ x, double *__restrict__ y)
{
    __shared__ double part[4];
    const int lane = threadIdx.x & 63, wave = threadIdx.x >> 6;
    const int64_t row = (WAVES == 4) ? (int64_t)blockIdx.x : (int64_t)blockIdx.x * 4 + wave;
    const bool live = row < m;
    const int t = (WAVES == 4) ? (int)threadIdx.x : lane, T = WAVES * 64;
    double a0 = 0.0, a1 = 0.0, a2 = 0.0, a3 = 0.0;
    if (live) {
        const double *r = A + row * lda;
        int64_t c = t;
        for (; c + 3 * T < n; c += 4 * T) {
            const double v0 = r[c], v1 = r[c + T], v2 = r[c + 2 * T], v3 = r[c + 3 * T];
            a0 = fma(v0, SQ ? v0 : x[c], a0);
            a1 = fma(v1, SQ ? v1 : x[c + T], a1);
            a2 = fma(v2, SQ ? v2 : x[c + 2 * T], a2);
            a3 = fma(v3, SQ ? v3 : x[c + 3 * T], a3);
        }
        for (; c < n; c += T) {
            const double v0 = r[c];
            a0 = fma(v0, SQ ? v0 : x[c], a0);
        }
    }
    double acc = (a0 + a1) + (a2 + a3);
    for (int off = 32; off > 0; off >>= 1) acc += __shfl_down(acc, off);
    if (WAVES == 4) {
        if (lane == 0) part[wave] = acc;
        __syncthreads();
        if (threadIdx.x == 0 && live) {
            const double tot = (part[0] + part[1]) + (part[2] + part[3]);
            y[row] = SQ ? x[row] - tot : tot;
        }
    } else if (lane == 0 && live) {
        y[row] = SQ ? x[row] - acc : acc;
    }
}

int launch_gemv_n(hipStream_t st, int64_t m, int64_t n, const double *A, int64_t lda, const double *x, double *y)
{
    if (m <= 0) return GPT_OK;
    if (m < 2048) hipLaunchKernelGGL((rowred_kernel<4, false>), dim3((unsigned)m), dim3(256), 0, st, m, n, A, lda, x, y);
    else hipLaunchKernelGGL((rowred_kernel<1, false>), dim3((unsigned)((m + 3) / 4)), dim3(256), 0, st, m, n, A, lda, x, y);
    GPT_LAUNCH_CHECK();
    return GPT_OK;
}

int launch_rowsumsq_sub(hipStream_t st, int64_t m, int64_t n, const double *V, int64_t ldv, const double *kdiag,
                        double *var_out)
{
    if (m <= 0) return GPT_OK;
    if (m < 2048) hipLaunchKernelGGL((rowred_kernel<4, true>), dim3((unsigned)m), dim3(256), 0, st, m, n, V, ldv, kdiag, var_out);
    else hipLaunchKernelGGL((rowred_kernel<1, true>), dim3((unsigned)((m + 3) / 4)), dim3(256), 0, st, m, n, V, ldv, kdiag, var_out);
    GPT_LAUNCH_CHECK();
    return GPT_OK;
}

__global__ __launch_bounds__(256) void mirror_rows_kernel(double *__restrict__ A, int64_t lda, int64_t c0, int64_t w, int64_t n)
{
    __shared__ double t[32][33];
    const int tx = threadIdx.x & 31, ty = threadIdx.x >> 5;
    const int64_t a0 = c0 + (int64_t)blockIdx.y * 32;
    const int64_t b0 = a0 + (int64_t)blockIdx.x * 32;
    if (b0 >= n) return;
    for (int i = ty; i < 32; i += 8)
        if (b0 + i < n && a0 + tx < c0 + w) t[i][tx] = A[(b0 + i) * lda + a0 + tx];
    __syncthreads();
    for (int i = ty; i < 32; i += 8) {
        const int64_t a = a0 + i, b = b0 + tx;
        if (a < c0 + w && b < n && b > a) A[a * lda + b] = t[tx][i];
    }
}

int launch_mirror_rows(hipStream_t st, double *A, int64_t lda, int64_t c0, int64_t w, int64_t n)
{
    if (w <= 0 || c0 >= n) return GPT_OK;
    dim3 grid((unsigned)((n - c0 + 31) / 32), (unsigned)((w + 31) / 32));
    hipLaunchKernelGGL(mirror_rows_kernel, grid, dim3(256), 0, st, A, lda, c0, w, n);
    GPT_LAUNCH_CHECK();
    return GPT_OK;
}

__global__ __launch_bounds__(256) void alpha_trace_kernel(const double *__restrict__ alpha, const double *__restrict__ W,
                                                          int64_t ldw, int64_t n, double *__restrict__ out)
{
    __shared__ double s0[4];
    double a = 0.0;
    for (int64_t i = threadIdx.x; i < n; i += 256) a += alpha[i] * alpha[i] - W[i * ldw + i];
    for (int off = 32; off > 0; off >>= 1) a += __shfl_down(a, off);
    if ((threadIdx.x & 63) == 0) s0[threadIdx.x >> 6] = a;
    __syncthreads();
    if (threadIdx.x == 0) out[0] = ((s0[0] + s0[1]) + s0[2]) + s0[3];
}

int launch_alpha_trace(hipStream_t st, const double *alpha, const double *W, int64_t ldw, int64_t n, double *out)
{
    hipLaunchKernelGGL(alpha_trace_kernel, dim3(1), dim3(256), 0, st, alpha, W, ldw, n, out);
    GPT_LAUNCH_CHECK();
    return GPT_OK;
}

__global__ void diag_gather_kernel(const double *__restrict__ A, int64_t lda, int64_t n, double *__restrict__ out)
{
    const int64_t i = (int64_t)blockIdx.x * blockDim.x + threadIdx.x;
    if (i < n) out[i] = A[i * lda + i];
}

int launch_diag_gather(hipStream_t st, const double *A, int64_t lda, int64_t n, double *out)
{
    if (n <= 0) return GPT_OK;
    hipLaunchKernelGGL(diag_gather_kernel, dim3((unsigned)((n + 255) / 256)), dim3(256), 0, st, A, lda, n, out);
    GPT_LAUNCH_CHECK();
    return GPT_OK;
}

__global__ void pad_block_kernel(double *__restrict__ A, int64_t lda, int64_t c0, int64_t nb, int64_t n_valid,
                                 int64_t n_pad, const double *__restrict__ dy, double big)
{
    const int64_t c = (int64_t)blockIdx.x * blockDim.x + threadIdx.x;
    const int64_t row = n_valid + blockIdx.y;
    if (c >= nb || row >= n_pad) return;
    const int64_t gc = c0 + c;
    double v = 0.0;
    if (row == n_valid && gc < n_valid) v = dy[gc];
    else if (gc == row) v = (row == n_valid) ? big : 1.0;
    A[row * lda + c] = v;
}

int launch_pad_block(hipStream_t st, double *A, int64_t lda, int64_t c0, int64_t nb, int64_t n_valid, int64_t n_pad,
                     const double *dy, double big)
{
    if (n_pad <= n_valid || nb <= 0) return GPT_OK;
    dim3 grid((unsigned)((nb + 255) / 256), (unsigned)(n_pad - n_valid));
    hipLaunchKernelGGL(pad_block_kernel, grid, dim3(256), 0, st, A, lda, c0, nb, n_valid, n_pad, dy, big);
    GPT_LAUNCH_CHECK();
    return GPT_OK;
}

__global__ __launch_bounds__(256) void panel_scalars_kernel(const double *__restrict__ P, int64_t ldp, int64_t w,
                                                            int64_t zrow, double *__restrict__ acc)
{
    __shared__ double s0[4], s1[4];
    double a = 0.0, b = 0.0;
    for (int64_t i = threadIdx.x; i < w; i += 256) {
        a += log(P[i * ldp + i]);
        if (zrow >= 0) {
            const double z = P[zrow * ldp + i];
            b = fma(z, z, b);
        }
    }
    for (int off = 32; off > 0; off >>= 1) {
        a += __shfl_down(a, off);
        b += __shfl_down(b, off);
    }
    const int lane = threadIdx.x & 63, wave = threadIdx.x >> 6;
    if (lane == 0) {
        s0[wave] = a;
        s1[wave] = b;
    }
    __syncthreads();
    if (threadIdx.x == 0) {
        acc[0] += ((s0[0] + s0[1]) + s0[2]) + s0[3];
        if (zrow >= 0) acc[1] += ((s1[0] + s1[1]) + s1[2]) + s1[3];
    }
}

int launch_panel_scalars(hipStream_t st, const double *P, int64_t ldp, int64_t w, int64_t zrow, double *acc)
{
    if (w <= 0) return GPT_OK;
    hipLaunchKernelGGL(panel_scalars_kernel, dim3(1), dim3(256), 0, st, P, ldp, w, zrow, acc);
    GPT_LAUNCH_CHECK();
    return GPT_OK;
}

__global__ __launch_bounds__(256) void row_sumsq_kernel(const double *__restrict__ row, int64_t w, double *__restrict__ acc)
{
    __shared__ double s1[4];
    double b = 0.0;
    for (int64_t i = threadIdx.x; i < w; i += 256) b = fma(row[i], row[i], b);
    for (int off = 32; off > 0; off >>= 1) b += __shfl_down(b, off);
    if ((threadIdx.x & 63) == 0) s1[threadIdx.x >> 6] = b;
    __syncthreads();
    if (threadIdx.x == 0) acc[0] += ((s1[0] + s1[1]) + s1[2]) + s1[3];
}

int launch_row_sumsq(hipStream_t st, const double *row, int64_t w, double *acc)
{
    if (w <= 0) return GPT_OK;
    hipLaunchKernelGGL(row_sumsq_kernel, dim3(1), dim3(256), 0, st, row, w, acc);
    GPT_LAUNCH_CHECK();
    return GPT_OK;
}

__global__ __launch_bounds__(256) void batch_meanvar_kernel(int64_t M, int64_t MP, int64_t N, int64_t NP, double *__restrict__ V,
                                                            int64_t ldv, const double *__restrict__ A, int64_t bs,
                                                            const int32_t *__restrict__ keep, double *__restrict__ mean,
                                                            double *__restrict__ var, int64_t ld)
{
    const int lane = threadIdx.x & 63;
    const int64_t a = (int64_t)blockIdx.x * 4 + (threadIdx.x >> 6), b = blockIdx.y;
    if (a >= MP) return;
    double *row = V + a * ldv + b * NP;
    if (!keep[b]) {
        for (int64_t i = lane; i < NP; i += 64) row[i] = 0.0;
        return;
    }
    const double *z = A + b * bs + N * NP;
    double s = 0.0, q = 0.0;
    for (int64_t i = lane; i < N; i += 64) {
        const double v = row[i];
        s = fma(v, z[i], s);
        q = fma(v, v, q);
    }
    for (int64_t i = N + lane; i < NP; i += 64) row[i] = 0.0;
#pragma unroll
    for (int off = 32; off > 0; off >>= 1) {
        s += __shfl_xor(s, off, 64);
        q += __shfl_xor(q, off, 64);
    }
    if (lane == 0 && a < M) {
        mean[b * ld + a] = s;
        var[b * ld + a] -= q;
    }
}

int launch_batch_meanvar(hipStream_t st, int64_t M, int64_t MP, int64_t N, int64_t NP, int64_t nbatch, double *V, int64_t ldv,
                         const double *A, int64_t bs, const int32_t *keep, double *mean, double *var, int64_t ld)
{
    if (MP <= 0 || nbatch <= 0) return GPT_OK;
    hipLaunchKernelGGL(batch_meanvar_kernel, dim3((unsigned)((MP + 3) / 4), (unsigned)nbatch), dim3(256), 0, st, M, MP, N, NP, V, ldv, A,
                       bs, keep, mean, var, ld);
    GPT_LAUNCH_CHECK();
    return GPT_OK;
}
```

include/gpt_hip.h:

```cpp
#ifndef GPT_HIP_H_
#define GPT_HIP_H_

#include <stdint.h>

#ifdef __cplusplus
extern "C" {
#endif

#define GPT_OK 0
#define GPT_E_ARG (-1)
#define GPT_E_VALUE (-2)
#define GPT_E_NOTIMPL (-3)
#define GPT_E_HIP (-4)
#define GPT_E_NOMEM (-5)
#define GPT_E_STATE (-6)

#define GPT_KERNEL_SE 0
#define GPT_KERNEL_M52 1
#define GPT_KERNEL_DIAGNOISE 2
#define GPT_KERNEL_ZERO 3
#define GPT_KERNEL_RQ 4
#define GPT_RQ_MAXORD 16
#define GPT_KERNEL_MATERN 5

#define GPT_KERNEL_PRODUCT 6
#define GPT_KERNEL_GIBBS_TANH 7
#define GPT_KERNEL_GIBBS_DTANH 8

#define GPT_MAX_DIM 16
#define GPT_WARP_LINEAR 1
#define GPT_WARP_BETA 2
#define GPT_WARP_MAX_LAYERS 4
#define GPT_WS_BLOCK 9216

typedef struct gpt_ctx gpt_ctx;

int gpt_version(void);
const char *gpt_last_error(void);

int gpt_ctx_create(int device_id, void *stream, gpt_ctx **out);
int gpt_ctx_destroy(gpt_ctx *ctx);
int gpt_ctx_set_option(gpt_ctx *ctx, const char *key, int64_t value);
int gpt_ctx_synchronize(gpt_ctx *ctx);
void *gpt_ctx_stream(gpt_ctx *ctx);
int64_t gpt_ctx_edge_count(gpt_ctx *ctx);
int gpt_concurrency_hint(int delta);

int gpt_kpairs(gpt_ctx *ctx, int kernel_id, const double *params, int nparams,
               const double *Xi, const double *Xj, const int32_t *ni, const int32_t *nj,
               int64_t M, int D, int hyper_deriv, int symmetric, const int32_t *noise_n,
               double *out);

int gpt_kpairs2(gpt_ctx *ctx, int kernel_id1, const double *params1, int nparams1, int kernel_id2, const double *params2,
                int nparams2, const double *Xi, const double *Xj, const int32_t *ni, const int32_t *nj, int64_t M, int D,
                double *out);

int gpt_kbuild(gpt_ctx *ctx, int kernel_id, const double *params, int nparams,
               const double *Xi, const int32_t *ni, int64_t M,
               const double *Xj, const int32_t *nj, int64_t P, int D,
               int hyper_deriv, const int32_t *noise_n, double *K_out);

int gpt_kbuild2(gpt_ctx *ctx, int kernel_id1, const double *params1, int nparams1, int kernel_id2, const double *params2,
                int nparams2, const double *Xi, const int32_t *ni, int64_t M, const double *Xj, const int32_t *nj, int64_t P,
                int D, double *K_out);

int gpt_set_data(gpt_ctx *ctx, const double *X, const int32_t *n, int64_t N, int D);

int gpt_set_T(gpt_ctx *ctx, const double *T, int64_t Ny);

int gpt_set_warp(gpt_ctx *ctx, int nlayers, const int *types, const double *params);

int gpt_set_warp_batch(gpt_ctx *ctx, int nbatch, int nlayers, const int *types, const double *params);

int gpt_fit(gpt_ctx *ctx, int kernel_id, const double *params, int nparams, double noise_var,
            const double *y, const double *err_y, double diag_add,
            double *ll_data_out, double *logdet_half_out);

int gpt_fit_sum(gpt_ctx *ctx, int nterms, const int *kernel_ids, const double *params, const int *nparams,
                double noise_var, const double *y, const double *err_y, double diag_add, double *ll_data_out,
                double *logdet_half_out);

int gpt_fit_terms(gpt_ctx *ctx, int nterms, const int *kernel_ids, const int *kernel_ids2, const double *params,
                  const int *nparams, const int *nparams1, double noise_var, const double *y, const double *err_y,
                  double diag_add, double *ll_data_out, double *logdet_half_out);

int gpt_fit_batch(gpt_ctx *ctx, int nbatch, int kernel_id, const double *params, int nparams,
                  const double *noise_var, const double *y, const double *err_y, double diag_add,
                  double *ll_data_out, double *logdet_half_out, int32_t *info_out);

int gpt_fit_batch_sum(gpt_ctx *ctx, int nbatch, int nterms, const int *kernel_ids, const double *params,
                      const int *nparams, const double *noise_var, const double *y, const double *err_y,
                      double diag_add, double *ll_data_out, double *logdet_half_out, int32_t *info_out);

int gpt_fit_batch_terms(gpt_ctx *ctx, int nbatch, int nterms, const int *kernel_ids, const int *kernel_ids2, const double *params,
                        const int *nparams, const int *nparams1, const double *noise_var, const double *y, const double *err_y,
                        double diag_add, double *ll_data_out, double *logdet_half_out, int32_t *info_out);

int gpt_mem_info(gpt_ctx *ctx, int64_t *free_bytes, int64_t *total_bytes);
int gpt_release_batch_scratch(gpt_ctx *ctx);

int gpt_predict_batch(gpt_ctx *ctx, const double *Xstar, const int32_t *nstar, int64_t M, const int32_t *noise_n,
                      const int32_t *keep, double *mean_out, double *var_out, double *cov_out, double *cov_sum_out);

int gpt_fit_matrix(gpt_ctx *ctx, const double *K_tot, int64_t N, const double *y,
                   double *ll_data_out, double *logdet_half_out);

int gpt_get_L(gpt_ctx *ctx, double *L_out);
int gpt_get_alpha(gpt_ctx *ctx, double *alpha_out);

int gpt_ll_grad(gpt_ctx *ctx, int nh, const int *term_idx, const int *local_idx, double *out);

int gpt_predict(gpt_ctx *ctx, const double *Xstar, const int32_t *nstar, int64_t M, int want,
                const double *noise_params, const int32_t *noise_n,
                double *mean_out, double *std_out, double *cov_out);

int gpt_cov_sample(gpt_ctx *ctx, int64_t M, double diag_add, const double *rand, int64_t S, double *out);

int gpt_host_alloc(int64_t bytes, void **out);
int gpt_host_free(void *p);

int gpt_solve_L(gpt_ctx *ctx, double *B, int64_t nrhs);
int gpt_cho_solve(gpt_ctx *ctx, double *B, int64_t nrhs);

int gpt_last_timings(gpt_ctx *ctx, double *out_ms, int n);

int gpt_gemm_profile_read(gpt_ctx *ctx, double *out3);
int gpt_gemm_profile_read4(gpt_ctx *ctx, double *out4);

int gpt_potrf_host(gpt_ctx *ctx, double *A, int64_t N);
int gpt_gemm_nt_host(gpt_ctx *ctx, int64_t m, int64_t n, int64_t k, double alpha, const double *A,
                     const double *B, double beta, double *C);


int gpt_dev_kbuild(gpt_ctx *ctx, int kernel_id, const double *params_host, int nparams,
                   const double *dXi, const int32_t *dni, int64_t M,
                   const double *dXj, const int32_t *dnj, int64_t P, int D,
                   int hyper_deriv, int symmetric, const int32_t *noise_n_host,
                   int lower_only, int64_t i0, int64_t j0,
                   const double *d_err_y, double noise_var, double diag_add,
                   double *dK, int64_t ldk);

int gpt_dev_gemm_nt(gpt_ctx *ctx, int64_t m, int64_t n, int64_t k, double alpha,
                    const double *dA, int64_t lda, const double *dB, int64_t ldb,
                    double beta, double *dC, int64_t ldc, int tri);
int gpt_dev_gemm_nt_stair(gpt_ctx *ctx, int64_t m, int64_t nseg, int64_t seg_cols, int64_t k, double alpha,
                          const double *dA, int64_t lda, const double *dB, int64_t ldb, int64_t b_stride,
                          int64_t row_step, double beta, double *dC, int64_t ldc);

int gpt_dev_gemm_nt_gridstair(gpt_ctx *ctx, int64_t m, int64_t nseg, int64_t seg_cols, int64_t k, double alpha,
                              const double *dA, int64_t lda, const double *dB, int64_t ldb, int64_t off, int64_t num,
                              int64_t den, int64_t base, double beta, double *dC, int64_t ldc);
int gpt_dev_row_sumsq(gpt_ctx *ctx, const double *d_row, int64_t w, double *d_acc);

int gpt_dev_potrf_panel(gpt_ctx *ctx, int64_t m, int64_t nb, double *dA, int64_t lda,
                        double *d_invd, int32_t *d_info, int64_t info_base);

int gpt_dev_potrf(gpt_ctx *ctx, int64_t n, double *dA, int64_t lda, double *d_invd, int32_t *d_info);

int gpt_dev_trsm_rlt(gpt_ctx *ctx, int64_t m, int64_t n, const double *dL, int64_t ldl,
                     const double *d_invd, double *dB, int64_t ldb);

int gpt_dev_trinv(gpt_ctx *ctx, int64_t n, const double *dL, int64_t ldl, const double *d_invd,
                  double *dW, int64_t ldw);

int gpt_dev_copy2d(gpt_ctx *ctx, int64_t rows, int64_t cols, const double *d_src, int64_t lds, double *d_dst, int64_t ldd);
int gpt_dev_copy2d_on(gpt_ctx *ctx, void *stream, int64_t rows, int64_t cols, const double *d_src, int64_t lds, double *d_dst,
                      int64_t ldd);
int gpt_dev_pad_block(gpt_ctx *ctx, double *dA, int64_t lda, int64_t c0, int64_t nb, int64_t n_valid, int64_t n_pad,
                      const double *d_y, double big);
int gpt_dev_panel_scalars(gpt_ctx *ctx, const double *dP, int64_t ldp, int64_t w, int64_t zrow, double *d_acc);

#define GPT_PLAN_W 20
#define GPT_PLAN_CHANNELS 8
typedef struct gpt_plan gpt_plan;
int gpt_plan_unique_id(void *out128);
int gpt_plan_create(int nctx, gpt_ctx **ctxs, const int64_t *ops, int64_t nops, int nevents, const void *dX, const void *dn, int D,
                    const void *d_err, gpt_plan **out);
int gpt_plan_set_comm(gpt_plan *plan, int nranks, int rank, const void *unique_id128);
int gpt_plan_set_channel(gpt_plan *plan, int channel, int nranks, int rank, const void *unique_id128);
int gpt_plan_run(gpt_plan *plan, int kernel_id, const double *params, int nparams, double noise_var, double diag_add);
double gpt_plan_last_enqueue_ms(gpt_plan *plan);
int gpt_plan_destroy(gpt_plan *plan);

#ifdef __cplusplus
}
#endif
#endif
```

Baseline: 39730.

## Merge pairs of 512-blocks in back-substitution via precomputed off-diagonal inverse quadrants

The blocked L^T back-substitution for alpha now handles pairs of 512-row blocks in one step. It precomputes the off-diagonal quadrant of each 1024x1024 block inverse with two batched GEMMs, then uses a fused pair-solve kernel and a wider gemv_t_sub pass. This roughly halves the number of serial solve steps and kernel launches. Quadrant construction is staged across the last Cholesky panels so it can overlap the factorization, at the cost of extra GEMM work, a new scratch slot and a new debug accessor.

After: 38960. 1.9% lower.

```diff
diff --git a/gptools_amd/_lib.py b/gptools_amd/_lib.py
--- a/gptools_amd/_lib.py
+++ b/gptools_amd/_lib.py
@@ -49,6 +49,7 @@
     "gpt_predict_batch": (C.c_int, [_vp, _dp, _ip, _i64, _ip, _ip, _dp, _dp, _dp, _dp]),
     "gpt_fit_matrix": (C.c_int, [_vp, _dp, _i64, _dp, _dp, _dp]),
     "gpt_get_L": (C.c_int, [_vp, _dp]),
+    "gpt_get_alpha_pair": (C.c_int, [_vp, C.c_int64, _dp, _dp, _dp]),
     "gpt_get_alpha": (C.c_int, [_vp, _dp]),
     "gpt_ll_grad": (C.c_int, [_vp, C.c_int, _ip, _ip, _dp]),
     "gpt_predict": (C.c_int, [_vp, _dp, _ip, _i64, C.c_int, _dp, _ip, _dp, _dp, _dp]),
@@ -464,6 +465,11 @@
         check(self._lib.gpt_get_L(self.handle, dptr(L)))
         return L
 
+    def get_alpha_pair(self, pair):
+        Ua, Ub, Q = (np.empty((512, 512), dtype=np.float64) for _ in range(3))
+        check(self._lib.gpt_get_alpha_pair(self.handle, pair, dptr(Ua), dptr(Ub), dptr(Q)))
+        return Ua, Ub, Q
+
     def get_alpha(self, N):
         a = np.empty(N, dtype=np.float64)
         check(self._lib.gpt_get_alpha(self.handle, dptr(a)))
diff --git a/gptools_amd/csrc/api.hip b/gptools_amd/csrc/api.hip
--- a/gptools_amd/csrc/api.hip
+++ b/gptools_amd/csrc/api.hip
@@ -40,7 +40,7 @@
 enum { SLOT_XI = 0, SLOT_XJ, SLOT_NI, SLOT_NJ, SLOT_OUT, SLOT_KST, SLOT_KSS, SLOT_XS, SLOT_NS, SLOT_VEC, SLOT_VEC2,
        SLOT_RHS, SLOT_LOW, SLOT_KFULL, SLOT_TK, SLOT_ZERO, SLOT_UINV, SLOT_WINV, SLOT_GPART, SLOT_BINV, SLOT_BTMP,
        SLOT_BINV2, SLOT_BINV3, SLOT_BINV3U, SLOT_BINVU, SLOT_BATCH_A, SLOT_BATCH_WS, SLOT_BATCH_MISC, SLOT_SPLITK,
-       SLOT_PB_V, SLOT_PB_COV, SLOT_PB_MISC, SLOT_XSW, SLOT_SS, SLOT_SI, SLOT_SJ, SLOT_WB_X, SLOT_WB_S, SLOT_WB_P, SLOT_COUNT };
+       SLOT_PB_V, SLOT_PB_COV, SLOT_PB_MISC, SLOT_XSW, SLOT_SS, SLOT_SI, SLOT_SJ, SLOT_WB_X, SLOT_WB_S, SLOT_WB_P, SLOT_BQUAD, SLOT_COUNT };
 
 struct gpt_ctx {
     int device = 0;
@@ -104,12 +104,14 @@
     int32_t *h_info = nullptr;
     bool factored = false, alpha_valid = false, have_kernel = false;
     bool binv_valid = false;
+    bool quad_valid = false;
     bool binv2_valid = false;
     bool binv3_valid = false;
     int64_t dev_gemm_pad = 0;
     int64_t eager_alpha = 0;
     int64_t binv_early = 0;
     hipEvent_t e_binv_early = nullptr;
+    int64_t quad_t_early = 0, quad_early = 0;
     int64_t defer_pad = 1;
     unsigned alpha_counter = 0;
     int64_t debug_poison = 0;
@@ -170,7 +172,7 @@
 static void invalidate_factor(gpt_ctx *c)
 {
     c->factored = false;
-    c->h_alpha_valid = c->alpha_valid = c->binv_valid = c->binv2_valid = c->binv3_valid = false;
+    c->h_alpha_valid = c->alpha_valid = c->binv_valid = c->quad_valid = c->binv2_valid = c->binv3_valid = false;
 }
 
 static int stream_follows(gpt_ctx *c, hipStream_t from, hipStream_t to, size_t idx)
diff --git a/gptools_amd/csrc/api_batch.inc b/gptools_amd/csrc/api_batch.inc
--- a/gptools_amd/csrc/api_batch.inc
+++ b/gptools_amd/csrc/api_batch.inc
@@ -360,19 +360,23 @@
 }
 
 static int ensure_block_inverses(gpt_ctx *c, int64_t nb, int64_t nfull, double **out, double **out_u = nullptr, hipStream_t on = nullptr);
+static bool alpha_narrow();
+static int64_t alpha_pairs(const gpt_ctx *c, int64_t nblk);
+static int ensure_quadrants(gpt_ctx *c, hipStream_t st, int64_t npairs, double **out);
 static int ensure_alpha(gpt_ctx *c, hipStream_t on = nullptr)
 {
     if (c->alpha_valid) return GPT_OK;
     const int64_t N = c->N, NP = c->NP, n128 = round_up(N, 128);
     hipStream_t st = on ? on : c->stream;
-    static const bool narrow = getenv("GPT_ALPHA_NARROW") != nullptr;
-    const int64_t nwide = (n128 / 512) * 512;
+    const bool narrow = alpha_narrow();
+    const int64_t nwide = (n128 / 512) * 512, npairs = alpha_pairs(c, nwide / 512);
     double *w = c->d_alpha + NP;
     const double *z = c->dA + N * NP;
     if (!narrow && nwide == N && nwide >= 1024) {
-        double *W = nullptr, *U = nullptr;
+        double *W = nullptr, *U = nullptr, *Q = nullptr;
         GPT_TRY(ensure_block_inverses(c, 512, nwide, &W, &U, st));
-        GPT_TRY(launch_trsv_lt_wide(st, nwide, c->dA, NP, U, w, c->d_alpha, z));
+        GPT_TRY(ensure_quadrants(c, st, npairs, &Q));
+        GPT_TRY(launch_trsv_lt_wide(st, nwide, c->dA, NP, U, w, c->d_alpha, z, Q, npairs));
         c->alpha_valid = true;
         return GPT_OK;
     }
@@ -383,13 +387,14 @@
         c->alpha_valid = true;
         return GPT_OK;
     }
-    double *W = nullptr, *U = nullptr;
+    double *W = nullptr, *U = nullptr, *Q = nullptr;
     GPT_TRY(ensure_block_inverses(c, 512, nwide, &W, &U, st));
+    GPT_TRY(ensure_quadrants(c, st, npairs, &Q));
     if (n128 > nwide) {
         GPT_TRY(launch_trsv_lt(st, n128, c->dA, NP, c->d_invd, w, nwide / 128));
         GPT_HIP_CHECK(hipMemcpyAsync(c->d_alpha + nwide, w + nwide, (size_t)(n128 - nwide) * sizeof(double), hipMemcpyDeviceToDevice, st));
     }
-    GPT_TRY(launch_trsv_lt_wide(st, nwide, c->dA, NP, U, w, c->d_alpha));
+    GPT_TRY(launch_trsv_lt_wide(st, nwide, c->dA, NP, U, w, c->d_alpha, nullptr, Q, npairs));
     c->alpha_valid = true;
     return GPT_OK;
 }
@@ -401,6 +406,25 @@
     if (c->h_alpha_valid) return GPT_OK;
     GPT_HIP_CHECK(hipMemcpyAsync(c->h_alpha, c->d_alpha, (size_t)c->N * sizeof(double), hipMemcpyDeviceToHost, st));
     c->h_alpha_valid = true;
+    return GPT_OK;
+}
+
+extern "C" int gpt_get_alpha_pair(gpt_ctx *c, int64_t pair, double *Ua_out, double *Ub_out, double *Q_out)
+{
+    CTX_ENTER(c);
+    NEED_FACTOR(c);
+    const int64_t nwide = (round_up(c->N, 128) / 512) * 512, npairs = alpha_pairs(c, nwide / 512), bs = 512 * 512;
+    if (!Ua_out || !Ub_out || !Q_out || pair < 0 || pair >= npairs) {
+        gpt_set_error("get_alpha_pair: pair %lld has no quadrant (%lld pairs)", (long long)pair, (long long)npairs);
+        return GPT_E_ARG;
+    }
+    double *W = nullptr, *U = nullptr, *Q = nullptr;
+    GPT_TRY(ensure_block_inverses(c, 512, nwide, &W, &U, c->stream));
+    GPT_TRY(ensure_quadrants(c, c->stream, npairs, &Q));
+    GPT_HIP_CHECK(hipMemcpyAsync(Ua_out, U + 2 * pair * bs, bs * sizeof(double), hipMemcpyDeviceToHost, c->stream));
+    GPT_HIP_CHECK(hipMemcpyAsync(Ub_out, U + (2 * pair + 1) * bs, bs * sizeof(double), hipMemcpyDeviceToHost, c->stream));
+    GPT_HIP_CHECK(hipMemcpyAsync(Q_out, Q + pair * bs, bs * sizeof(double), hipMemcpyDeviceToHost, c->stream));
+    GPT_HIP_CHECK(hipStreamSynchronize(c->stream));
     return GPT_OK;
 }
 
diff --git a/gptools_amd/csrc/api_context.inc b/gptools_amd/csrc/api_context.inc
--- a/gptools_amd/csrc/api_context.inc
+++ b/gptools_amd/csrc/api_context.inc
@@ -144,7 +144,7 @@
     else if (!strcmp(key, "splitk")) c->splitk = value;
     else if (!strcmp(key, "eager_alpha")) c->eager_alpha = value;
     else if (!strcmp(key, "defer_pad")) c->defer_pad = value;
-    else if (!strcmp(key, "binv_launches")) { c->binv_launches = value; c->binv_valid = c->binv2_valid = c->binv3_valid = false; c->h_alpha_valid = c->alpha_valid = false; }
+    else if (!strcmp(key, "binv_launches")) { c->binv_launches = value; c->binv_valid = c->quad_valid = c->binv2_valid = c->binv3_valid = false; c->h_alpha_valid = c->alpha_valid = false; }
     else if (!strcmp(key, "debug_poison")) c->debug_poison = value;
     else if (!strcmp(key, "alpha_invalidate")) c->h_alpha_valid = c->alpha_valid = false;
     else if (!strcmp(key, "edge_test_stall")) c->edge_test_stall = value;
diff --git a/gptools_amd/csrc/api_fit.inc b/gptools_amd/csrc/api_fit.inc
--- a/gptools_amd/csrc/api_fit.inc
+++ b/gptools_amd/csrc/api_fit.inc
@@ -200,7 +200,7 @@
     }
     if (c->timing) GPT_HIP_CHECK(hipEventRecord(c->tev[2], st));
     req.defer_join = true;
-    c->binv_early = 0;
+    c->binv_early = c->quad_t_early = c->quad_early = 0;
     req.want_early_binv = c->eager_alpha != 0 && !c->use_graph;
     req.defer_pad_leaf = req.want_early_binv && c->defer_pad && N % 512 == 0 && N >= 1024 && NP == N + 128;
     PotrfResult fac;
@@ -221,7 +221,7 @@
                               c->flags_now ? c->d_edge + 60 : nullptr));
     invalidate_factor(c);
     int rc_alpha = c->eager_alpha ? alpha_to_host(c, tl) : GPT_OK;
-    c->binv_early = 0;
+    c->binv_early = c->quad_t_early = c->quad_early = 0;
     if (tl != st && !joined) GPT_TRY(stream_follows(c, tl, st, 1));
     if (rc_alpha != GPT_OK) {
         invalidate_factor(c);
diff --git a/gptools_amd/csrc/api_schedule.inc b/gptools_amd/csrc/api_schedule.inc
--- a/gptools_amd/csrc/api_schedule.inc
+++ b/gptools_amd/csrc/api_schedule.inc
@@ -277,7 +277,7 @@
     return GPT_OK;
 }
 
-static int enqueue_early_block_inverses(gpt_ctx *c, hipStream_t S, int64_t cols, int64_t cols_final);
+static int enqueue_early_alpha_work(gpt_ctx *c, hipStream_t S, int64_t cols, int64_t cols_final, int left);
 #define GPT_MERGE_MIN_TILES 512
 static int potrf_enqueue(gpt_ctx *c, int64_t n, double *A, int64_t lda, double *invd, int32_t *info, const PotrfRequest &req,
                          PotrfResult *res)
@@ -353,6 +353,12 @@
     int64_t c0 = 0, s_prev = 0;
     int64_t awaited = 0;
     struct PendingRest { bool on; int64_t c0, w, u1, split; } pend = {false, 0, 0, 0, 0};
+    const bool early_alpha = req.want_early_binv && A == c->dA && invd == c->d_invd && np >= 2;
+    auto early_piece = [&](size_t k) -> int {
+        const size_t left = np - 1 - k;
+        if (!early_alpha || left < 1 || left > 3) return GPT_OK;
+        return enqueue_early_alpha_work(c, S, n - widths.back(), awaited, (int)left);
+    };
     for (size_t k = 0; k < np; c0 += widths[k], k++) {
         const int64_t w = widths[k];
         const int64_t wn = (k + 1 < np) ? widths[k + 1] : 0;
@@ -435,6 +441,7 @@
                 if (!e_rest_prev) return GPT_E_HIP;
                 GPT_TRY(update(S, c0, w, u1, n, e_rest_prev));
             }
+            GPT_TRY(early_piece(k));
             continue;
         }
         e_rest_prev = nullptr;
@@ -451,6 +458,7 @@
                     s_prev = split;
                     e_help_prev = e_help;
                 }
+                GPT_TRY(early_piece(k));
                 continue;
             }
             GPT_TRY(update(S, c0, w, u0, u1, nullptr, cu_edge_prev));
@@ -458,6 +466,7 @@
             GPT_TRY(update(S, c0, w, u0, u1, e_cu));
             e_cu_prev = e_cu;
         }
+        GPT_TRY(early_piece(k));
         if (u1 < n) {
             GPT_TRY(wait_help_prev());
             if (defer_rows > 0 && n - c0 <= defer_rows && k + 1 < np) {
@@ -473,8 +482,7 @@
         }
     }
     if (pend.on) GPT_TRY(update(S, pend.c0, pend.w, pend.u1, pend.split));
-    if (req.want_early_binv && A == c->dA && invd == c->d_invd && np >= 2)
-        GPT_TRY(enqueue_early_block_inverses(c, S, n - widths.back(), awaited));
+    if (early_alpha) GPT_TRY(enqueue_early_alpha_work(c, S, n - widths.back(), awaited, 0));
     if (ps.pad_leaf_deferred) {
         hipEvent_t e_real = get_event(c, 12 + 6 * np);
         if (!e_real) return GPT_E_HIP;
diff --git a/gptools_amd/csrc/api_solve.inc b/gptools_amd/csrc/api_solve.inc
--- a/gptools_amd/csrc/api_solve.inc
+++ b/gptools_amd/csrc/api_solve.inc
@@ -71,21 +71,92 @@
     return GPT_OK;
 }
 
-static int enqueue_early_block_inverses(gpt_ctx *c, hipStream_t S, int64_t cols, int64_t cols_final)
+static bool alpha_narrow()
+{
+    static const bool narrow = getenv("GPT_ALPHA_NARROW") != nullptr;
+    return narrow;
+}
+static int64_t alpha_pairs(const gpt_ctx *c, int64_t nblk) { return (c->binv_launches || alpha_narrow() || nblk < 3) ? 0 : (nblk - 1) / 2; }
+
+static int quadrant_strip(gpt_ctx *c, double **Q, double **T)
+{
+    const int64_t nb = GPT_BINV_NB, cap = (c->NP / (2 * nb)) > 0 ? c->NP / (2 * nb) : 1;
+    double *q;
+    GPT_TRY(ensure(c, SLOT_BQUAD, (size_t)2 * cap * nb * nb * sizeof(double), (void **)&q));
+    *Q = q;
+    *T = q + cap * nb * nb;
+    return GPT_OK;
+}
+static int build_quadrants(gpt_ctx *c, hipStream_t st, int64_t p0, int64_t p1, int which)
+{
+    if (p1 <= p0) return GPT_OK;
+    const int64_t nb = GPT_BINV_NB, bs = nb * nb, NP = c->NP, nall = (NP / nb) * nb;
+    double *W, *Us, *Q, *T;
+    GPT_TRY(ensure(c, SLOT_BINV, (size_t)nall * nb * sizeof(double), (void **)&W));
+    GPT_TRY(ensure(c, SLOT_BINVU, (size_t)nall * nb * sizeof(double), (void **)&Us));
+    GPT_TRY(quadrant_strip(c, &Q, &T));
+    if (2 * p1 * nb > nall) {
+        gpt_set_error("quadrants: pair %lld exceeds the padded order %lld", (long long)p1, (long long)NP);
+        return GPT_E_ARG;
+    }
+    const int64_t np = p1 - p0, a0 = 2 * p0;
+    if (which & 1)
+        GPT_TRY(launch_gemm_nt(st, nb, nb, nb, -1.0, Us + a0 * bs, nb, c->dA + (a0 + 1) * nb * NP + a0 * nb, NP, 0.0, T + p0 * bs, nb, 0, 0, 0,
+                               nullptr, nullptr, 0, EdgeSig(), EdgeSig(), 0, np, 2 * bs, EdgeSig(), 2 * nb * (NP + 1), bs));
+    if (which & 2)
+        GPT_TRY(launch_gemm_nt(st, nb, nb, nb, 1.0, T + p0 * bs, nb, W + (a0 + 1) * bs, nb, 0.0, Q + p0 * bs, nb, 0, 0, 0, nullptr, nullptr, 0,
+                               EdgeSig(), EdgeSig(), 0, np, bs, EdgeSig(), 2 * bs, bs));
+    return GPT_OK;
+}
+
+static int ensure_quadrants(gpt_ctx *c, hipStream_t st, int64_t npairs, double **out)
+{
+    double *Q, *T;
+    GPT_TRY(quadrant_strip(c, &Q, &T));
+    *out = Q;
+    if (c->quad_valid || npairs <= 0) return GPT_OK;
+    const int64_t t0 = c->quad_t_early < npairs ? c->quad_t_early : npairs, q0 = c->quad_early < npairs ? c->quad_early : npairs;
+    GPT_TRY(build_quadrants(c, st, t0, npairs, 1));
+    GPT_TRY(build_quadrants(c, st, q0, npairs, 2));
+    c->quad_t_early = c->quad_early = 0;
+    c->quad_valid = true;
+    return GPT_OK;
+}
+
+static int enqueue_early_alpha_work(gpt_ctx *c, hipStream_t S, int64_t cols, int64_t cols_final, int left)
 {
     const int64_t nb = GPT_BINV_NB, nall = (c->NP / nb) * nb;
     int64_t b = cols / nb;
-    c->binv_early = 0;
     if (c->binv_launches || nall < 2 * nb || b <= 0 || b >= nall / nb) return GPT_OK;
     if (b * nb > cols_final) b = cols_final / nb;
     if (b <= 0) return GPT_OK;
-    double *W, *Us = nullptr;
-    GPT_TRY(ensure(c, SLOT_BINV, (size_t)nall * nb * sizeof(double), (void **)&W));
-    GPT_TRY(ensure(c, SLOT_BINVU, (size_t)nall * nb * sizeof(double), (void **)&Us));
-    GPT_TRY(launch_trinv512(S, b, c->dA, c->NP, c->d_invd, Us, W));
-    if (!c->e_binv_early) GPT_HIP_CHECK(hipEventCreateWithFlags(&c->e_binv_early, hipEventDisableTiming));
-    GPT_HIP_CHECK(hipEventRecord(c->e_binv_early, S));
-    c->binv_early = b;
+    const int64_t nblk = (round_up(c->N, 128) / nb), rule = alpha_pairs(c, nblk);
+    bool did = false;
+    if ((left == 3 || left == 0) && b > c->binv_early) {
+        double *W, *Us = nullptr;
+        const int64_t b0 = c->binv_early;
+        GPT_TRY(ensure(c, SLOT_BINV, (size_t)nall * nb * sizeof(double), (void **)&W));
+        GPT_TRY(ensure(c, SLOT_BINVU, (size_t)nall * nb * sizeof(double), (void **)&Us));
+        GPT_TRY(launch_trinv512(S, b - b0, c->dA + b0 * nb * (c->NP + 1), c->NP, c->d_invd + b0 * (nb / 128) * GPT_WS_BLOCK, Us + b0 * nb * nb,
+                                W + b0 * nb * nb));
+        c->binv_early = b;
+        did = true;
+    }
+    const int64_t pairs = (c->binv_early / 2 < rule) ? c->binv_early / 2 : rule;
+    if ((left == 2 || left == 0) && pairs > c->quad_t_early) {
+        GPT_TRY(build_quadrants(c, S, c->quad_t_early, pairs, 1));
+        c->quad_t_early = pairs;
+        did = true;
+    }
+    if ((left == 1 || left == 0) && c->quad_t_early > c->quad_early) {
+        GPT_TRY(build_quadrants(c, S, c->quad_early, c->quad_t_early, 2));
+        c->quad_early = c->quad_t_early;
+        did = true;
+    }
+    if (did) {
+        if (!c->e_binv_early) GPT_HIP_CHECK(hipEventCreateWithFlags(&c->e_binv_early, hipEventDisableTiming));
+        GPT_HIP_CHECK(hipEventRecord(c->e_binv_early, S));
+    }
     return GPT_OK;
 }
 
diff --git a/gptools_amd/csrc/common.hpp b/gptools_amd/csrc/common.hpp
--- a/gptools_amd/csrc/common.hpp
+++ b/gptools_amd/csrc/common.hpp
@@ -162,7 +162,7 @@
 int launch_extract_lower(hipStream_t st, const double *A, int64_t lda, int64_t n, double *out, int64_t ldo);
 int launch_trsv_lt(hipStream_t st, int64_t n, const double *L, int64_t ldl, const double *invd, double *x, int64_t b_lo = 0);
 int launch_trsv_lt_wide(hipStream_t st, int64_t nwide, const double *L, int64_t ldl, const double *U, double *w, double *x,
-                        const double *w0 = nullptr);
+                        const double *w0 = nullptr, const double *Q = nullptr, int64_t npairs = 0);
 int launch_alpha_init(hipStream_t st, int64_t n, int64_t np, const double *z, double *w, double *x);
 int launch_gemv_n(hipStream_t st, int64_t m, int64_t n, const double *A, int64_t lda, const double *x, double *y);
 int launch_trinv512(hipStream_t st, int64_t nblk, const double *L, int64_t ldl, const double *invd, double *U, double *W);
diff --git a/gptools_amd/csrc/solve.hip b/gptools_amd/csrc/solve.hip
--- a/gptools_amd/csrc/solve.hip
+++ b/gptools_amd/csrc/solve.hip
@@ -559,24 +559,27 @@
 }
 
 #define TW_NB 512
+template <int NB>
 __global__ __launch_bounds__(512) void gemv_t_sub_kernel(int64_t ncols, const double *__restrict__ M, int64_t ldm,
                                                          const double *__restrict__ x, double *__restrict__ w, const double *__restrict__ w_in)
 {
-    __shared__ double xs[TW_NB];
+    __shared__ double xs[NB];
     __shared__ double part[32][17];
     const int tid = threadIdx.x, lane = tid & 63, g = tid >> 6, c = lane & 15, rs = lane >> 4;
-    xs[tid] = x[tid];
+#pragma unroll
+    for (int i = 0; i < NB; i += 512) xs[tid + i] = x[tid + i];
     __syncthreads();
     const int64_t col = (int64_t)blockIdx.x * 16 + c;
     double a0 = 0.0, a1 = 0.0, a2 = 0.0, a3 = 0.0;
     if (col < ncols) {
-        const int r0 = g * (TW_NB / 8) + rs;
+        constexpr int NL = NB / 32;
+        const int r0 = g * (NB / 8) + rs;
         const double *p = M + (int64_t)r0 * ldm + col;
-        double v[16];
-#pragma unroll
-        for (int i = 0; i < 16; i++) v[i] = p[(int64_t)(4 * i) * ldm];
-#pragma unroll
-        for (int i = 0; i < 16; i += 4) {
+        double v[NL];
+#pragma unroll
+        for (int i = 0; i < NL; i++) v[i] = p[(int64_t)(4 * i) * ldm];
+#pragma unroll
+        for (int i = 0; i < NL; i += 4) {
             a0 = fma(v[i + 0], xs[r0 + 4 * (i + 0)], a0);
             a1 = fma(v[i + 1], xs[r0 + 4 * (i + 1)], a1);
             a2 = fma(v[i + 2], xs[r0 + 4 * (i + 2)], a2);
@@ -593,6 +596,26 @@
     }
 }
 
+__global__ __launch_bounds__(256) void pair_solve_kernel(const double *__restrict__ Ua, const double *__restrict__ Q,
+                                                         const double *__restrict__ wv, double *__restrict__ xv)
+{
+    __shared__ double part[4];
+    const int row = (int)blockIdx.x, t = (int)threadIdx.x, lane = t & 63, wave = t >> 6;
+    const double *u = Ua + (int64_t)row * TW_NB;
+    const double *ws = wv + (row < TW_NB ? 0 : TW_NB);
+    double a0 = u[t] * ws[t], a1 = u[t + 256] * ws[t + 256];
+    if (row < TW_NB) {
+        const double *q = Q + (int64_t)row * TW_NB;
+        a0 = fma(q[t], wv[TW_NB + t], a0);
+        a1 = fma(q[t + 256], wv[TW_NB + t + 256], a1);
+    }
+    double acc = a0 + a1;
+    for (int off = 32; off > 0; off >>= 1) acc += __shfl_down(acc, off);
+    if (lane == 0) part[wave] = acc;
+    __syncthreads();
+    if (t == 0) xv[row] = (part[0] + part[1]) + (part[2] + part[3]);
+}
+
 __global__ __launch_bounds__(256) void alpha_init_kernel(int64_t n, int64_t np, const double *__restrict__ z, double *__restrict__ w,
                                                          double *__restrict__ x)
 {
@@ -609,7 +632,8 @@
     return GPT_OK;
 }
 
-int launch_trsv_lt_wide(hipStream_t st, int64_t nwide, const double *L, int64_t ldl, const double *U, double *w, double *x, const double *w0)
+int launch_trsv_lt_wide(hipStream_t st, int64_t nwide, const double *L, int64_t ldl, const double *U, double *w, double *x, const double *w0,
+                        const double *Q, int64_t npairs)
 {
     if (nwide % TW_NB) {
         gpt_set_error("trsv_lt_wide: the extent must be a multiple of %d", TW_NB);
@@ -619,11 +643,25 @@
         gpt_set_error("trsv_lt_wide: w0 needs at least two blocks");
         return GPT_E_ARG;
     }
+    if (npairs < 0 || 2 * npairs * TW_NB > nwide || (npairs > 0 && !Q) || (w0 && 2 * npairs * TW_NB >= nwide)) {
+        gpt_set_error("trsv_lt_wide: %lld block pairs do not fit the extent %lld", (long long)npairs, (long long)nwide);
+        return GPT_E_ARG;
+    }
     const double *wsrc = w0 ? w0 : w;
     for (int64_t j0 = nwide - TW_NB; j0 >= 0; j0 -= TW_NB) {
-        GPT_TRY_RC_SOLVE(launch_gemv_n(st, TW_NB, TW_NB, U + j0 * TW_NB, TW_NB, wsrc + j0, x + j0));
-        if (j0 > 0)
-            hipLaunchKernelGGL(gemv_t_sub_kernel, dim3((unsigned)(j0 / 16)), dim3(512), 0, st, j0, L + j0 * ldl, ldl, x + j0, w, wsrc);
+        const int64_t blk = j0 / TW_NB;
+        if ((blk & 1) && blk / 2 < npairs) {
+            j0 -= TW_NB;
+            hipLaunchKernelGGL(pair_solve_kernel, dim3(2 * TW_NB), dim3(256), 0, st, U + j0 * TW_NB, Q + (blk / 2) * TW_NB * TW_NB, wsrc + j0,
+                               x + j0);
+            if (j0 > 0)
+                hipLaunchKernelGGL(gemv_t_sub_kernel<2 * TW_NB>, dim3((unsigned)(j0 / 16)), dim3(512), 0, st, j0, L + j0 * ldl, ldl, x + j0, w,
+                                   wsrc);
+        } else {
+            GPT_TRY_RC_SOLVE(launch_gemv_n(st, TW_NB, TW_NB, U + j0 * TW_NB, TW_NB, wsrc + j0, x + j0));
+            if (j0 > 0)
+                hipLaunchKernelGGL(gemv_t_sub_kernel<TW_NB>, dim3((unsigned)(j0 / 16)), dim3(512), 0, st, j0, L + j0 * ldl, ldl, x + j0, w, wsrc);
+        }
         wsrc = w;
     }
     GPT_LAUNCH_CHECK();
diff --git a/include/gpt_hip.h b/include/gpt_hip.h
--- a/include/gpt_hip.h
+++ b/include/gpt_hip.h
@@ -107,6 +107,7 @@
 
 int gpt_get_L(gpt_ctx *ctx, double *L_out);
 int gpt_get_alpha(gpt_ctx *ctx, double *alpha_out);
+int gpt_get_alpha_pair(gpt_ctx *ctx, int64_t pair, double *Ua_out, double *Ub_out, double *Q_out);
 
 int gpt_ll_grad(gpt_ctx *ctx, int nh, const int *term_idx, const int *local_idx, double *out);
 
```
